# AlessioSam/LADiff

Measured on AMD Instinct MI355X. Metric: motions/sec (196-frame, 50-step DDIM, bs128), higher is better.
Workload: dtype f16x3+f32; 1 GPU; headline:ddim50_cfg7.5_b128_f196_c263_humanml3d; prompts_per_gpu=128, global_batch=128, frames=196, scheduler=ddim, denoising_steps=50, parallelism=dp1, loop=persistent pipeline kernel (16-row blocks x 86)

## Files before the change

### ladiff_amd/csrc/api.hip

```cpp
#include <algorithm>
#include <cstdlib>
#include <cstring>
#include <vector>

#include "model.h"
#include "sampler.h"
#include "../../include/ladiff_hip_debug.h"

using namespace ladiff;

namespace {

inline hipStream_t S(ladiff_stream_t s) { return reinterpret_cast<hipStream_t>(s); }

bool all_set(const float* const* w, size_t n) {
    if (w == nullptr) return false;
    for (size_t i = 0; i < n; ++i)
        if (w[i] == nullptr) return false;
    return true;
}
template <class W>
bool load_weights(W& dst, const float* const* ptrs) {
    if (!all_set(ptrs, sizeof(W) / sizeof(const float*))) return false;
    std::memcpy(&dst, ptrs, sizeof(W));
    return true;
}
const char* name_at(const std::vector<std::string>& n, int i) { return (i >= 0 && i < (int)n.size()) ? n[i].c_str() : nullptr; }

}

#ifdef LADIFF_STAMPS
static unsigned long long* g_stamps = nullptr;
#endif

extern "C" {

int ladiff_version(void) { return LADIFF_ABI_VERSION; }
int ladiff_split_format(void) {
#ifndef LADIFF_SPLIT_BF16
    return 1;
#else
    return 0;
#endif
}

const char* ladiff_error_string(int code) {
    switch (code) {
        case LADIFF_OK: return "ok";
        case LADIFF_ERR_ARG: return "invalid argument (null pointer or negative size)";
        case LADIFF_ERR_SHAPE: return "shape not supported by the gfx950 kernels";
        case LADIFF_ERR_WORKSPACE: return "workspace too small";
        case LADIFF_ERR_UNSUPPORTED: return "configuration branch not built";
        default: return code > 0 ? hipGetErrorString((hipError_t)code) : "unknown ladiff error";
    }
}

int ladiff_denoiser_num_params(void) { return DEN_NPARAMS; }
const char* ladiff_denoiser_param_name(int i) { return name_at(denoiser_param_names(), i); }
int ladiff_decoder_num_params(void) { return DEC_NPARAMS; }
const char* ladiff_decoder_param_name(int i) { return name_at(decoder_param_names(), i); }

int ladiff_gemm(const float* A, int lda, const float* A2, int lda2, int K1, const float* W, int ldw, const float* bias,
                const float* res, int ldres, const float* ln_gamma, const float* ln_beta, float* Y, int ldy, int M,
                int N, int K, int act, ladiff_stream_t stream) {
    LADIFF_CHECK_ARG(A && W && Y && M >= 0 && N > 0 && K > 0);
    GemmArgs g;
    g.A = A; g.lda = lda; g.A2 = A2; g.lda2 = lda2; g.K1 = A2 ? K1 : K; g.W = W; g.ldw = ldw; g.bias = bias;
    g.res = res; g.ldres = ldres; g.ln_g = ln_gamma; g.ln_b = ln_beta; g.Y = Y; g.ldy = ldy; g.M = M; g.N = N; g.K = K;
    g.act = act;
    return launch_gemm(g, S(stream));
}

int ladiff_gemm_resident(const float* A, int lda, const float* A2, int lda2, int K1, const float* W, int ldw,
                         const float* bias, const float* res, int ldres, float* Y, int ldy, int M, int N, int K, int act,
                         int split, float* Ys, ladiff_stream_t stream) {
    LADIFF_CHECK_ARG(A && W && (Y || Ys) && M >= 0 && N > 0 && K > 0);
    if (M == 0) return 0;
    KrArgs g;
    g.A = A; g.lda = lda; g.A2 = A2; g.lda2 = lda2; g.K1 = A2 ? K1 : K; g.W = W; g.ldw = ldw; g.bias = bias;
    g.res = res; g.ldres = ldres; g.Y = Y; g.ldy = ldy; g.M = M; g.N = N; g.K = K; g.act = act;
    g.split = split; g.Ys = Ys;
#ifdef LADIFF_STAMPS
    g.stamps = g_stamps;
#endif
    return launch_gemm_kr(g, S(stream));
}

int ladiff_gemm_split(const float* A, int lda, const float* A2, int lda2, int K1, const float* W, int ldw, const float* bias,
                      const float* res, int ldres, float* Y, float* Ys, int ldy, int M, int N, int K, int act,
                      ladiff_stream_t stream) {
    LADIFF_CHECK_ARG(A && W && (Y || Ys) && M >= 0 && N > 0 && K > 0);
    if (M == 0) return 0;
    GemmArgs g;
    g.A = A; g.lda = lda; g.A2 = A2; g.lda2 = lda2; g.K1 = A2 ? K1 : K; g.W = W; g.ldw = ldw; g.bias = bias;
    g.res = res; g.ldres = ldres; g.Y = Y; g.Ys = Ys; g.ldy = ldy; g.M = M; g.N = N; g.K = K; g.act = act; g.split = 1;
    return launch_gemm(g, S(stream));
}

#ifdef LADIFF_STAMPS
void ladiff_debug_set_stamps(unsigned long long* p) { g_stamps = p; }
void ladiff_debug_set_sys_stamps(unsigned long long* p) { ladiff::g_sys_stamps = p; }
void ladiff_debug_set_probe(int v) { ladiff::g_sys_probe = v; }
#endif

int ladiff_combine_rows(const float* partials, int n_planes, int M, const float* bias, const float* res, int mode,
                        const float* ln_gamma, const float* ln_beta, const float* table, const int32_t* counts, int Bs,
                        int T, int pad_row, float* out, ladiff_stream_t stream) {
    LADIFF_CHECK_ARG(partials && out && n_planes > 0 && M >= 0 && Bs > 0 && T > 0);
    if (mode != RED_PLAIN && mode != RED_LN && mode != RED_LN_ADD && mode != RED_LN_MOD) return LADIFF_ERR_ARG;
    if (mode != RED_PLAIN && !(ln_gamma && ln_beta)) return LADIFF_ERR_ARG;
    if ((mode == RED_LN_ADD || mode == RED_LN_MOD) && !table) return LADIFF_ERR_ARG;
    if (M == 0) return 0;
    RedArgs r;
    r.P = partials; r.S = n_planes; r.M = M; r.bias = bias; r.res = res; r.mode = mode; r.g = ln_gamma; r.b = ln_beta; r.tab = table;
    r.counts = counts; r.Bs = Bs; r.T = T; r.pad_row = pad_row; r.out = out;
    return launch_reduce_rows(r, S(stream));
}

int ladiff_layernorm(const float* x, const float* gamma, const float* beta, float* y, int M, ladiff_stream_t stream) {
    LADIFF_CHECK_ARG(x && gamma && beta && y && M >= 0);
    return launch_layernorm(x, gamma, beta, y, M, S(stream));
}

int ladiff_timestep_sinusoid(const int64_t* timesteps, int n, float* out, ladiff_stream_t stream) {
    LADIFF_CHECK_ARG(timesteps && out && n >= 0);
    if (n == 0) return 0;
    return launch_sinusoid(timesteps, n, out, S(stream));
}

int ladiff_decoder_self_attention(const float* qkv, const int32_t* lengths, const uint32_t* keybits, float* out, int B,
                                  int F, ladiff_stream_t stream) {
    LADIFF_CHECK_ARG(qkv && (lengths || keybits) && out && B >= 0);
    return launch_decoder_self_attention(qkv, lengths, keybits, out, B, F, 0, S(stream));
}

int ladiff_self_attention_split(const float* qkv, const int32_t* lengths, const uint32_t* keybits, float* out, int B, int F,
                                 int nheads, int causal, ladiff_stream_t stream) {
    LADIFF_CHECK_ARG(qkv && out && B >= 0);
    return launch_self_attention_split(qkv, lengths, keybits, out, B, F, nheads, causal, 0, S(stream));
}

int ladiff_decoder_cross_attention(const float* q, const float* kv, const int32_t* counts, float* out, int B, int F,
                                   int T, ladiff_stream_t stream) {
    LADIFF_CHECK_ARG(q && kv && out && B >= 0 && F >= 0);
    return launch_decoder_cross_attention(q, kv, counts, out, B, F, T, 0, S(stream));
}

size_t ladiff_denoiser_tables_floats(int n_steps) { return den_tables_floats(n_steps); }
size_t ladiff_denoiser_text_cache_floats(int B2, int n_steps, int n_text) { return den_text_cache_floats(B2, n_steps, n_text); }
size_t ladiff_denoiser_workspace_bytes(int B2, int T, int n_steps, int n_text) {
    return sizeof(float) * std::max({den_forward_ws_floats(B2, T), den_time_layout(nullptr, n_steps).total,
                                     den_text_ws_floats(B2, n_steps, n_text), den_text_ws_floats(B2, n_steps, 1)});
}

int ladiff_denoiser_time_tables(const float* const* w, const float* sinusoid, int n_steps, float* tables, void* ws,
                                size_t ws_bytes, ladiff_stream_t stream) {
    DenoiserW W;
    LADIFF_CHECK_ARG(load_weights(W, w) && sinusoid && tables && ws && n_steps > 0);
    if (ws_bytes < ladiff_denoiser_workspace_bytes(1, 1, n_steps, 1)) return LADIFF_ERR_WORKSPACE;
    return denoiser_time_tables(W, sinusoid, n_steps, tables, (float*)ws, ws_bytes / sizeof(float), S(stream));
}

int ladiff_denoiser_text_cache(const float* const* w, const float* text_emb, int B2, int n_text, const float* tables, int n_steps,
                               float* cache, void* ws, size_t ws_bytes, ladiff_stream_t stream) {
    DenoiserW W;
    LADIFF_CHECK_ARG(load_weights(W, w) && text_emb && tables && cache && ws && B2 > 0 && n_steps > 0 && n_text >= 1);
    if (ws_bytes < ladiff_denoiser_workspace_bytes(B2, 1, n_steps, n_text)) return LADIFF_ERR_WORKSPACE;
    return denoiser_text_cache(W, text_emb, B2, tables, n_steps, cache, (float*)ws, ws_bytes / sizeof(float), S(stream), n_text);
}

int ladiff_denoiser_forward(const float* const* w, const float* const* w_split, const float* tables, const int32_t* d_step,
                            const float* text_cache, int n_text, int n_steps, const float* sample, int Bs, int dup, int T,
                            const int32_t* counts, float* eps, void* ws, size_t ws_bytes, ladiff_stream_t stream) {
    DenoiserW W, WS;
    LADIFF_CHECK_ARG(load_weights(W, w) && tables && d_step && text_cache && sample && eps && ws && Bs > 0 && dup > 0 && n_steps > 0 &&
                     n_text >= 1);
    if (w_split != nullptr) LADIFF_CHECK_ARG(load_weights(WS, w_split));
    if (T < 1 || T > LADIFF_MAX_LATENTS) return LADIFF_ERR_SHAPE;
    if (ws_bytes < ladiff_denoiser_workspace_bytes(Bs * dup, T, n_steps, n_text)) return LADIFF_ERR_WORKSPACE;
    return denoiser_forward(W, w_split ? &WS : nullptr, tables, d_step, text_cache, n_steps, sample, Bs, dup, T, counts, eps, (float*)ws,
                            ws_bytes / sizeof(float), S(stream), 0, -1, 0, n_text);
}

size_t ladiff_linear_cross_attention_workspace_bytes(int B, int T, int n_text) {
    return linear_cross_attention_ws_floats(B, T, n_text) * sizeof(float);
}
int ladiff_linear_cross_attention(const float* const* w, int layer, const float* x, const float* xf, const float* emb,
                                  const int32_t* counts, int B, int T, int n_text, float* out, void* ws, size_t ws_bytes,
                                  ladiff_stream_t stream) {
    DenoiserW W;
    LADIFF_CHECK_ARG(load_weights(W, w) && x && xf && emb && out && ws && B > 0);
    return linear_cross_attention(W, layer, x, xf, emb, counts, B, T, n_text, out, (float*)ws, ws_bytes / sizeof(float), S(stream));
}

int ladiff_cfg_scheduler_step(const float* eps, float* latents, const float* coef, const int32_t* d_step,
                              const float* step_noise, float guidance_scale, int cfg, int B, int T,
                              ladiff_stream_t stream) {
    LADIFF_CHECK_ARG(eps && latents && coef && d_step && B > 0 && T > 0);
    return launch_cfg_step(eps, latents, coef, d_step, step_noise, guidance_scale, cfg, B, T, S(stream));
}
int ladiff_cfg_scheduler_step_multistep(const float* eps, float* latents, float* x0_prev, const float* coef, const int32_t* d_step,
                                        const float* step_noise, float guidance_scale, int cfg, int B, int T, ladiff_stream_t stream) {
    LADIFF_CHECK_ARG(eps && latents && x0_prev && coef && d_step && B > 0 && T > 0);
    if (reinterpret_cast<uintptr_t>(x0_prev) & 15) return LADIFF_ERR_SHAPE;
    return launch_cfg_step(eps, latents, coef, d_step, step_noise, guidance_scale, cfg, B, T, S(stream), nullptr, NoiseGen{0u, 0u, 0u, 0},
                           x0_prev);
}
int ladiff_advance_step(int32_t* d_step, ladiff_stream_t stream) {
    LADIFF_CHECK_ARG(d_step);
    return launch_advance(d_step, S(stream));
}
int ladiff_init_latents(const float* noise, const int32_t* counts, float sigma, float* latents, int B, int T,
                        ladiff_stream_t stream) {
    LADIFF_CHECK_ARG(noise && latents && B > 0 && T > 0);
    return launch_init_latents(noise, counts, sigma, latents, B, T, S(stream));
}
int ladiff_finalize_latents(const float* latents, const int32_t* counts, float* z, int B, int T, ladiff_stream_t stream) {
    LADIFF_CHECK_ARG(latents && z && B > 0 && T > 0);
    return launch_finalize_latents(latents, counts, z, B, T, S(stream));
}

int ladiff_sampler_create(void** sampler) {
    LADIFF_CHECK_ARG(sampler);
    *sampler = new Sampler();
    return 0;
}
int ladiff_sampler_destroy(void* sampler) {
    Sampler* sp = reinterpret_cast<Sampler*>(sampler);
    if (sp == nullptr) return 0;
    (void)hipDeviceSynchronize();
    sp->drain_retired();
    if (sp->exec) (void)hipGraphExecDestroy(sp->exec);
    if (sp->setup) (void)hipGraphExecDestroy(sp->setup);
    if (sp->ev0) (void)hipEventDestroy(sp->ev0);
    if (sp->ev1) (void)hipEventDestroy(sp->ev1);
    for (hipEvent_t e : sp->wev) (void)hipEventDestroy(e);
    sp->cap.destroy();
    delete sp;
    return 0;
}

int ladiff_reverse_plan(int B, int T, const int32_t* h_counts, int masked, int loop_mode, int f16x3, int cfg, int* rows_per_block, int* n_blocks) {
    LADIFF_CHECK_ARG(B >= 1 && T >= 1 && T <= LADIFF_MAX_LATENTS && loop_mode >= 1 && loop_mode <= 3 && rows_per_block && n_blocks);
    if (!cfg && masked && h_counts == nullptr) return LADIFF_ERR_UNSUPPORTED;
    std::vector<unsigned char> plan;
    int mr = 2, nb = 0;
    choose_plan(B, T, h_counts, masked != 0, loop_mode, f16x3 != 0, plan, &mr, &nb, cfg != 0);
    *rows_per_block = 16 * mr; *n_blocks = nb;
    return 0;
}

int ladiff_debug_set_stage_waves(int waves_per_simd) {
    LADIFF_CHECK_ARG(waves_per_simd == 1 || waves_per_simd == 2);
    g_waves16 = waves_per_simd;
    return 0;
}

int ladiff_debug_set_handoff(int tagged) {
    LADIFF_CHECK_ARG(tagged == 0 || tagged == 1);
    g_handoff = tagged;
    return 0;
}

int ladiff_debug_set_mlp_variant(int v) {
#ifdef LADIFF_STAMPS
    LADIFF_CHECK_ARG((v >= 0 && v <= 3) || (v >= 11 && v <= 17) || (v >= 21 && v <= 26));
#else
    LADIFF_CHECK_ARG(v >= 0 && v <= 3);
#endif
    g_mlp_variant = v;
    return 0;
}

int ladiff_debug_set_decoder_fusion(int on) {
    LADIFF_CHECK_ARG(on >= 0 && on <= 126 && (on & 3) != 3 && (on & 48) != 48);
    g_dec_out_cross = (on & 64) ? 0 : 1;
    g_dec_fused_mlp = on & 3;
    g_dec_small_rows_path = (on & 4) ? 0 : 1;
    g_dec_final_split = (on & 8) ? 0 : 1;
    g_dec_fused_attn = (on & 16) ? 0 : (on & 32) ? 2 : 1;
    return 0;
}

int ladiff_debug_set_stage_plan(int v) {
    LADIFF_CHECK_ARG(v >= 0 && v <= 1);
    g_stage_plan = v;
    return 0;
}

int ladiff_debug_set_poll_pause(int mask, int len) {
    LADIFF_CHECK_ARG(mask >= 0 && mask <= 255 && len >= 0 && len <= 64);
    g_poll_pause = mask | (len << 8);
    return 0;
}

int ladiff_debug_set_pacing(int eighths, int mask) {
    if (eighths == -1) { g_pace = -1; return 0; }
    LADIFF_CHECK_ARG(eighths >= 0 && eighths <= 8 && mask >= 0 && mask <= 255);
    g_pace = eighths | (mask << 8);
    return 0;
}

int ladiff_debug_set_stage_delay(int mask, int len) {
    LADIFF_CHECK_ARG(mask >= -1 && mask <= 255 && len >= 0 && len <= 64);
    g_stage_delay = mask < 0 ? -1 : (mask | (len << 8));
    return 0;
}

int ladiff_debug_set_loop_thresholds(int look_ahead_from, int small_upto) {
    LADIFF_CHECK_ARG(look_ahead_from >= -1 && small_upto >= -1);
    g_look_ahead_from = look_ahead_from;
    g_small_upto = small_upto;
    return 0;
}

int ladiff_debug_set_graph_epoch_rule(int on) {
    LADIFF_CHECK_ARG(on == 0 || on == 1);
    g_graph_epoch_rule = on;
    return 0;
}

int ladiff_debug_graph_instantiations(void) { return g_graph_instantiations.load(); }

int ladiff_debug_set_xcd_local(int on) {
    LADIFF_CHECK_ARG(on >= 0 && on <= 2);
    g_xcd_local = on;
    return 0;
}

int ladiff_sampler_set_loop(void* sampler, int mode) {
    Sampler* sp = reinterpret_cast<Sampler*>(sampler);
    LADIFF_CHECK_ARG(sp != nullptr && mode >= 0 && mode <= 3);
    sp->loop = mode != 0;
    sp->loop_mode = mode;
    return 0;
}

int ladiff_sampler_loop_ms(void* sampler, float* ms) {
    Sampler* sp = reinterpret_cast<Sampler*>(sampler);
    LADIFF_CHECK_ARG(sp != nullptr && ms != nullptr && sp->ev1 != nullptr);
    LADIFF_HIP(hipEventSynchronize(sp->ev1));
    LADIFF_HIP(hipEventElapsedTime(ms, sp->ev0, sp->ev1));
    return 0;
}

int ladiff_sampler_set_window_timing(void* sampler, int on) {
    Sampler* sp = reinterpret_cast<Sampler*>(sampler);
    LADIFF_CHECK_ARG(sp != nullptr);
    sp->time_windows = on != 0;
    return 0;
}

int ladiff_sampler_window_ms(void* sampler, float* loop_ms_sum, int* n_windows) {
    Sampler* sp = reinterpret_cast<Sampler*>(sampler);
    LADIFF_CHECK_ARG(sp != nullptr && loop_ms_sum != nullptr && n_windows != nullptr);
    float sum = 0.f;
    for (int i = 0; i < sp->n_windows; ++i) {
        float ms = 0.f;
        LADIFF_HIP(hipEventSynchronize(sp->wev[2 * i + 1]));
        LADIFF_HIP(hipEventElapsedTime(&ms, sp->wev[2 * i], sp->wev[2 * i + 1]));
        sum += ms;
    }
    *loop_ms_sum = sum; *n_windows = sp->n_windows;
    return 0;
}

int ladiff_sampler_last_loop(void* sampler, int* pipeline, int* rows_per_block, int* n_blocks) {
    Sampler* sp = reinterpret_cast<Sampler*>(sampler);
    LADIFF_CHECK_ARG(sp != nullptr && pipeline != nullptr);
    *pipeline = sp->last_pipeline;
    if (rows_per_block) *rows_per_block = sp->last_pipeline ? 16 * sp->plan_mr : 0;
    if (n_blocks) *n_blocks = sp->last_pipeline ? sp->plan_nb : 0;
    return 0;
}

int ladiff_sampler_set_noise_generator(void* sampler, uint64_t seed, uint32_t first_prompt, int enable) {
    Sampler* sp = reinterpret_cast<Sampler*>(sampler);
    LADIFF_CHECK_ARG(sp != nullptr);
    sp->gen = NoiseGen{(unsigned)(seed & 0xffffffffull), (unsigned)(seed >> 32), first_prompt, enable ? 1 : 0};
    return 0;
}

int ladiff_noise_fill(uint64_t seed, uint32_t first_prompt, int first_step, int n_steps, int B, int T, float* out, ladiff_stream_t stream) {
    LADIFF_CHECK_ARG(out != nullptr && first_step >= 0 && n_steps >= 0 && B >= 0);
    if (T < 1 || T > LADIFF_MAX_LATENTS) return LADIFF_ERR_SHAPE;
    return launch_noise_fill(NoiseGen{(unsigned)(seed & 0xffffffffull), (unsigned)(seed >> 32), first_prompt, 1}, first_step, n_steps, B, T, out,
                             S(stream));
}

int ladiff_noise_fill_prompts(const uint64_t* seeds, const uint32_t* prompt_index, int first_step, int n_steps, int B, int T, float* out,
                              ladiff_stream_t stream) {
    LADIFF_CHECK_ARG(out != nullptr && first_step >= -1 && n_steps >= 0 && B >= 0 && (seeds != nullptr || B == 0));
    if (T < 1 || T > LADIFF_MAX_LATENTS) return LADIFF_ERR_SHAPE;
    if ((reinterpret_cast<uintptr_t>(seeds) & 7) || (reinterpret_cast<uintptr_t>(prompt_index) & 3)) return LADIFF_ERR_SHAPE;
    return launch_noise_fill(NoiseGen{0u, 0u, 0u, 1, reinterpret_cast<const unsigned long long*>(seeds), prompt_index}, first_step, n_steps, B, T,
                             out, S(stream));
}

int ladiff_sampler_set_fault(void* sampler, int workgroup, int timeout_ms) {
    Sampler* sp = reinterpret_cast<Sampler*>(sampler);
    LADIFF_CHECK_ARG(sp != nullptr && workgroup >= -1 && workgroup < 256 && timeout_ms >= 0);
    sp->fault_wg = workgroup;
    sp->timeout_ticks = (unsigned long long)timeout_ms * 100000ull;
    return 0;
}

size_t ladiff_reverse_status_offset_bytes(int B, int T, int n_steps, int n_text) {
    if (B < 1 || T < 1 || T > LADIFF_MAX_LATENTS || n_steps < 1 || n_text < 1) return 0;
    const ReverseWs r = carve_reverse(nullptr, B, T, n_steps, n_text);
    return (r.sys_off + sys_status_offset_floats(B, T)) * sizeof(float);
}

int ladiff_reverse_status(void* ws, int B, int T, int n_steps, int n_text, int* code, int* info) {
    LADIFF_CHECK_ARG(ws && code && B > 0 && n_steps > 0);
    if (T < 1 || T > LADIFF_MAX_LATENTS) return LADIFF_ERR_SHAPE;
    const ReverseWs r = carve_reverse(ws, B, T, n_steps, n_text);
    unsigned st[2] = {0u, 0u};
    LADIFF_HIP(hipMemcpy(st, r.sys + sys_status_offset_floats(B, T), sizeof(st), hipMemcpyDeviceToHost));
    *code = (int)st[0];
    if (info) *info = (int)st[1];
    return 0;
}

size_t ladiff_reverse_workspace_bytes(int B, int T, int n_steps, int n_text) { return carve_reverse(nullptr, B, T, n_steps, n_text).total_bytes; }

int ladiff_mlp_ln_fused(const float* xs, const float* x, const float* w1s, const float* b1, const float* w2s, const float* b2,
                        const float* ln_gamma, const float* ln_beta, const float* ln2_gamma, const float* ln2_beta, float* y, float* ys,
                        int M, ladiff_stream_t stream) {
    LADIFF_CHECK_ARG(xs && x && w1s && b1 && w2s && b2 && ln_gamma && ln_beta && (y || ys) && M >= 0);
    if ((ln2_gamma == nullptr) != (ln2_beta == nullptr)) return LADIFF_ERR_ARG;
    return launch_dec_mlp(xs, x, w1s, b1, w2s, b2, ln_gamma, ln_beta, ln2_gamma, ln2_beta, y, ys, M, S(stream));
}

int ladiff_split_rows(const float* x, float* y, int R, int K, ladiff_stream_t stream) {
    LADIFF_CHECK_ARG(x && y && R >= 0 && K > 0);
    if (K % 64) return LADIFF_ERR_SHAPE;
    if (R == 0) return 0;
    return launch_split_rows(x, y, R, K, S(stream));
}

int ladiff_gather_rows(const float* src, const int32_t* index, int n_rows, int row_floats, float* dst, ladiff_stream_t stream) {
    LADIFF_CHECK_ARG(n_rows >= 0 && row_floats > 0);
    if (n_rows == 0) return 0;
    LADIFF_CHECK_ARG(src && index && dst);
    if (row_floats % 4 || (reinterpret_cast<uintptr_t>(src) & 15) || (reinterpret_cast<uintptr_t>(dst) & 15)) return LADIFF_ERR_SHAPE;
    if ((reinterpret_cast<uintptr_t>(index) & 3) || n_rows > (1 << 30)) return LADIFF_ERR_SHAPE;
    return launch_gather_rows(src, index, n_rows, row_floats, dst, S(stream));
}

int ladiff_split_range_stats(const float* const* tensors, const int64_t* counts, int n, int64_t max_count, uint64_t* stats,
                             ladiff_stream_t stream) {
    LADIFF_CHECK_ARG(n >= 0 && max_count >= 0);
    if (n == 0) return 0;
    LADIFF_CHECK_ARG(tensors && counts && stats);
    if (n > 65535 || max_count >= (int64_t(1) << 32)) return LADIFF_ERR_SHAPE;
    return launch_split_range_stats(tensors, counts, n, max_count, reinterpret_cast<unsigned long long*>(stats), S(stream));
}

int ladiff_diffusion_reverse(void* sampler, const float* const* w, const float* const* w_split, uint64_t weights_generation,
                             const float* text_emb, const float* init_noise, const int32_t* counts, const int32_t* final_counts,
                             const int32_t* h_counts, const float* sinusoid, const float* coef, const float* step_noise, float guidance_scale,
                             float init_noise_sigma, int cfg, int B, int T, int n_text, int n_steps, float* z, void* ws, size_t ws_bytes,
                             int reuse_time_tables, ladiff_stream_t stream) {
    return ladiff_diffusion_reverse_prompts(sampler, w, w_split, weights_generation, text_emb, init_noise, counts, final_counts, h_counts, sinusoid,
                                            coef, step_noise, guidance_scale, init_noise_sigma, cfg, B, T, n_text, n_steps, z, ws, ws_bytes,
                                            reuse_time_tables, nullptr, nullptr, nullptr, 0, stream);
}

int ladiff_diffusion_reverse_prompts(void* sampler, const float* const* w, const float* const* w_split, uint64_t weights_generation,
                                     const float* text_emb, const float* init_noise, const int32_t* counts, const int32_t* final_counts,
                                     const int32_t* h_counts, const float* sinusoid, const float* coef, const float* step_noise,
                                     float guidance_scale, float init_noise_sigma, int cfg, int B, int T, int n_text, int n_steps, float* z,
                                     void* ws, size_t ws_bytes, int reuse_time_tables, const float* guidance_scales, const uint64_t* seeds,
                                     const uint32_t* prompt_index, int draw_init_noise, ladiff_stream_t stream) {
    return ladiff_diffusion_reverse_multistep(sampler, w, w_split, weights_generation, text_emb, init_noise, counts, final_counts, h_counts,
                                              sinusoid, coef, step_noise, guidance_scale, init_noise_sigma, cfg, B, T, n_text, n_steps, z, ws,
                                              ws_bytes, reuse_time_tables, guidance_scales, seeds, prompt_index, draw_init_noise, nullptr, stream);
}

int ladiff_diffusion_reverse_multistep(void* sampler, const float* const* w, const float* const* w_split, uint64_t weights_generation,
                                       const float* text_emb, const float* init_noise, const int32_t* counts, const int32_t* final_counts,
                                       const int32_t* h_counts, const float* sinusoid, const float* coef, const float* step_noise,
                                       float guidance_scale, float init_noise_sigma, int cfg, int B, int T, int n_text, int n_steps, float* z,
                                       void* ws, size_t ws_bytes, int reuse_time_tables, const float* guidance_scales, const uint64_t* seeds,
                                       const uint32_t* prompt_index, int draw_init_noise, float* x0_prev, ladiff_stream_t stream) {
    DenoiserW W, WS;
    LADIFF_CHECK_ARG(guidance_scales == nullptr || cfg != 0);
    LADIFF_CHECK_ARG(prompt_index == nullptr || seeds != nullptr);
    LADIFF_CHECK_ARG(!draw_init_noise || seeds != nullptr);
    LADIFF_CHECK_ARG(init_noise != nullptr || draw_init_noise);
    LADIFF_CHECK_ARG(load_weights(W, w) && text_emb && sinusoid && coef && z && ws && B > 0 && n_steps > 0);
    if (w_split != nullptr) LADIFF_CHECK_ARG(load_weights(WS, w_split));
    if (T < 1 || T > LADIFF_MAX_LATENTS || n_text < 1) return LADIFF_ERR_SHAPE;
    if ((reinterpret_cast<uintptr_t>(guidance_scales) & 3) || (reinterpret_cast<uintptr_t>(seeds) & 7) ||
        (reinterpret_cast<uintptr_t>(prompt_index) & 3) || (reinterpret_cast<uintptr_t>(x0_prev) & 15))
        return LADIFF_ERR_SHAPE;
    return diffusion_reverse(reinterpret_cast<Sampler*>(sampler), W, w_split ? &WS : nullptr,
                             ReverseArgs{w, w_split, weights_generation, text_emb, init_noise, counts, final_counts, h_counts, sinusoid, coef,
                                         step_noise, guidance_scale, init_noise_sigma, cfg, B, T, n_text, n_steps, z, ws, ws_bytes,
                                         reuse_time_tables, stream, guidance_scales, seeds, prompt_index, draw_init_noise ? 1 : 0, x0_prev});
}

int ladiff_encoder_num_params(void) { return ENC_NPARAMS; }
const char* ladiff_encoder_param_name(int i) { return name_at(encoder_param_names(), i); }
size_t ladiff_encoder_workspace_bytes(int B, int F, int T, int C) { return enc_ws_floats(B, F, T, C) * sizeof(float); }

int ladiff_vae_encode(const float* const* w, const float* const* w_split, const float* features, const int32_t* lengths,
                      const int32_t* counts, const float* eps, int B, int F, int T, int C, float* mu, float* std,
                      float* latent, void* ws, size_t ws_bytes, ladiff_stream_t stream) {
    EncoderW W, WS;
    LADIFF_CHECK_ARG(load_weights(W, w) && features && lengths && counts && eps && mu && std && latent && ws && B >= 0);
    if (w_split != nullptr) LADIFF_CHECK_ARG(load_weights(WS, w_split));
    return vae_encode(W, w_split ? &WS : nullptr, features, lengths, counts, eps, B, F, T, C, mu, std, latent, (float*)ws,
                      ws_bytes / sizeof(float), S(stream));
}

int ladiff_vae_encode_dvae(const float* const* w, const float* const* w_split, const float* features, const int32_t* lengths,
                           const int32_t* counts, const float* eps, int B, int F, int T, int C, float* mu, float* std, float* latent,
                           void* ws, size_t ws_bytes, const int32_t* slot, const float* values, int n, ladiff_stream_t stream) {
    EncoderW W, WS;
    LADIFF_CHECK_ARG(load_weights(W, w) && features && lengths && counts && eps && mu && std && latent && ws && B >= 0);
    LADIFF_CHECK_ARG(slot && n >= 0 && (values || n == 0));
    if (w_split != nullptr) LADIFF_CHECK_ARG(load_weights(WS, w_split));
    if ((reinterpret_cast<uintptr_t>(slot) & 3) || (reinterpret_cast<uintptr_t>(values) & 3)) return LADIFF_ERR_SHAPE;
    return vae_encode(W, w_split ? &WS : nullptr, features, lengths, counts, eps, B, F, T, C, mu, std, latent, (float*)ws,
                      ws_bytes / sizeof(float), S(stream), slot, values, n);
}

size_t ladiff_vae_losses_workspace_bytes(int B, int F, int C, int J, int T) { return vae_losses_ws_floats(B, F, C, J, T) * sizeof(float); }

int ladiff_vae_losses(const float* m_rst, const float* m_ref, const float* joints_rst, const float* joints_ref, const float* mu,
                      const float* std, int B, int F, int C, int J, int T, double lambda_rec, double lambda_joint, double lambda_kl,
                      double* batch, double* acc, void* ws, size_t ws_bytes, ladiff_stream_t stream) {
    LADIFF_CHECK_ARG(m_rst && m_ref && joints_rst && joints_ref && mu && std && batch && acc && ws);
    if (B < 1 || F < 1 || C < 1 || J < 1 || T < 1) return LADIFF_ERR_SHAPE;
    for (const void* p : {(const void*)m_rst, (const void*)m_ref, (const void*)joints_rst, (const void*)joints_ref, (const void*)mu,
                          (const void*)std})
        if (reinterpret_cast<uintptr_t>(p) & 3) return LADIFF_ERR_SHAPE;
    for (const void* p : {(const void*)batch, (const void*)acc, (const void*)ws})
        if (reinterpret_cast<uintptr_t>(p) & 7) return LADIFF_ERR_SHAPE;
    const VaeLossWs a = vae_losses_layout((float*)ws, B, F, C, J, T);
    if (ws_bytes / sizeof(float) < a.total) return LADIFF_ERR_WORKSPACE;
    return launch_vae_losses(m_rst, m_ref, (size_t)B * F * C, joints_rst, joints_ref, (size_t)B * F * J * 3, mu, std, (size_t)T * B * D,
                             lambda_rec, lambda_joint, lambda_kl, a.part, a.blocks, batch, acc, S(stream));
}

size_t ladiff_denoiser_forward_timesteps_workspace_bytes(int B2, int T) { return den_per_sample_ws_floats(B2, T) * sizeof(float); }

int ladiff_denoiser_forward_timesteps(const float* const* w, const float* const* w_split, const float* text_emb, int n_text,
                                      const int64_t* timesteps, const float* sample, int B2, int T, const int32_t* counts, float* eps,
                                      void* ws, size_t ws_bytes, ladiff_stream_t stream) {
    DenoiserW W, WS;
    LADIFF_CHECK_ARG(load_weights(W, w) && text_emb && timesteps && sample && eps && ws);
    if (w_split != nullptr) LADIFF_CHECK_ARG(load_weights(WS, w_split));
    if (n_text != 1) return LADIFF_ERR_UNSUPPORTED;
    if (B2 < 1 || T < 1 || T > LADIFF_MAX_LATENTS) return LADIFF_ERR_SHAPE;
    for (const void* p : {(const void*)text_emb, (const void*)sample, (const void*)eps, (const void*)ws})
        if (reinterpret_cast<uintptr_t>(p) & 15) return LADIFF_ERR_SHAPE;
    if ((reinterpret_cast<uintptr_t>(timesteps) & 7) || (reinterpret_cast<uintptr_t>(counts) & 3)) return LADIFF_ERR_SHAPE;
    if (ws_bytes < ladiff_denoiser_forward_timesteps_workspace_bytes(B2, T)) return LADIFF_ERR_WORKSPACE;
    return denoiser_forward_timesteps(W, w_split ? &WS : nullptr, text_emb, timesteps, sample, B2, T, counts, eps, (float*)ws,
                                      ws_bytes / sizeof(float), S(stream));
}

int ladiff_q_sample(const float* z, const int64_t* timesteps, const float* alphas_cumprod, int n_train, const int32_t* counts, int draw,
                    uint64_t seed, uint32_t first_prompt, float* noise, float* noisy, int B, int T, ladiff_stream_t stream) {
    LADIFF_CHECK_ARG(z && timesteps && alphas_cumprod && noise && noisy && n_train > 0);
    if (B < 1 || T < 1 || T > LADIFF_MAX_LATENTS) return LADIFF_ERR_SHAPE;
    for (const void* p : {(const void*)z, (const void*)noise, (const void*)noisy})
        if (reinterpret_cast<uintptr_t>(p) & 15) return LADIFF_ERR_SHAPE;
    if ((reinterpret_cast<uintptr_t>(timesteps) & 7) || (reinterpret_cast<uintptr_t>(alphas_cumprod) & 3) ||
        (reinterpret_cast<uintptr_t>(counts) & 3))
        return LADIFF_ERR_SHAPE;
    return launch_q_sample(z, timesteps, alphas_cumprod, n_train, counts,
                           NoiseGen{(unsigned)(seed & 0xffffffffull), (unsigned)(seed >> 32), first_prompt, draw ? 1 : 0}, noise, noisy, B, T,
                           S(stream));
}

size_t ladiff_diffusion_losses_workspace_bytes(int64_t n) { return n < 1 ? 0 : diffusion_losses_layout(nullptr, (size_t)n).total * sizeof(float); }

int ladiff_diffusion_losses(const float* noise_pred, const float* noise, int64_t n, double lambda_inst, double* batch, double* acc, void* ws,
                            size_t ws_bytes, ladiff_stream_t stream) {
    LADIFF_CHECK_ARG(noise_pred && noise && batch && acc && ws);
    if (n < 1) return LADIFF_ERR_SHAPE;
    if ((reinterpret_cast<uintptr_t>(noise_pred) & 3) || (reinterpret_cast<uintptr_t>(noise) & 3)) return LADIFF_ERR_SHAPE;
    for (const void* p : {(const void*)batch, (const void*)acc, (const void*)ws})
        if (reinterpret_cast<uintptr_t>(p) & 7) return LADIFF_ERR_SHAPE;
    const DiffLossWs a = diffusion_losses_layout((float*)ws, (size_t)n);
    if (ws_bytes / sizeof(float) < a.total) return LADIFF_ERR_WORKSPACE;
    return launch_diffusion_losses(noise_pred, noise, (size_t)n, lambda_inst, a.part, a.blocks, batch, acc, S(stream));
}

int ladiff_clip_num_params(void) { return CLIP_NPARAMS; }
const char* ladiff_clip_param_name(int i) { return name_at(clip_param_names(), i); }
size_t ladiff_clip_workspace_bytes(int B, int L) { return clip_ws_floats(B, L) * sizeof(float); }

static bool load_clip(ClipW& dst, const float* const* ptrs, int n_layers) {
    if (ptrs == nullptr || n_layers < 1 || n_layers > CLIP_MAX_LAYERS) return false;
    const int n = CLIP_HEAD_NPARAMS + CLIP_LAYER_NPARAMS * n_layers;
    for (int i = 0; i < n; ++i)
        if (ptrs[i] == nullptr) return false;
    std::memset(&dst, 0, sizeof(dst));
    std::memcpy(&dst, ptrs, n * sizeof(const float*));
    return true;
}

int ladiff_clip_text_encode(const float* const* w, const float* const* w_split, int n_layers, int vocab, const int64_t* ids,
                            int B, int seq, int L, float* out, void* ws, size_t ws_bytes, ladiff_stream_t stream) {
    ClipW W, WS;
    LADIFF_CHECK_ARG(load_clip(W, w, n_layers) && ids && out && ws && B >= 0);
    if (w_split != nullptr) LADIFF_CHECK_ARG(load_clip(WS, w_split, n_layers));
    return clip_text_encode(W, w_split ? &WS : nullptr, n_layers, vocab, ids, B, seq, L, out, (float*)ws,
                            ws_bytes / sizeof(float), S(stream));
}

size_t ladiff_clip_workspace_bytes_ragged(int B, int total_rows) { return clip_ws_floats_rows(B, total_rows) * sizeof(float); }

int ladiff_clip_text_encode_ragged(const float* const* w, const float* const* w_split, int n_layers, int vocab, const int64_t* ids,
                                   int B, int seq, int L, const int32_t* seq_len, const int32_t* row_off, const int32_t* row_seq,
                                   int total_rows, float* out, void* ws, size_t ws_bytes, ladiff_stream_t stream) {
    ClipW W, WS;
    LADIFF_CHECK_ARG(load_clip(W, w, n_layers) && ids && out && ws && B >= 0 && seq_len && row_off && row_seq && total_rows >= 0);
    if (w_split != nullptr) LADIFF_CHECK_ARG(load_clip(WS, w_split, n_layers));
    return clip_text_encode(W, w_split ? &WS : nullptr, n_layers, vocab, ids, B, seq, L, out, (float*)ws,
                            ws_bytes / sizeof(float), S(stream), seq_len, row_off, row_seq, total_rows);
}

int ladiff_t2m_movement_num_params(void) { return (int)t2m_move_param_names().size(); }
const char* ladiff_t2m_movement_param_name(int i) { return name_at(t2m_move_param_names(), i); }
int ladiff_t2m_motion_num_params(void) { return (int)t2m_motion_param_names().size(); }
const char* ladiff_t2m_motion_param_name(int i) { return name_at(t2m_motion_param_names(), i); }
int ladiff_t2m_text_num_params(void) { return (int)t2m_text_param_names().size(); }
const char* ladiff_t2m_text_param_name(int i) { return name_at(t2m_text_param_names(), i); }
size_t ladiff_t2m_movement_workspace_bytes(int B, int F, int Cin) { return t2m_move_ws_floats(B, F, Cin) * sizeof(float); }
size_t ladiff_t2m_motion_workspace_bytes(int B, int T) { return t2m_motion_ws_floats(B, T) * sizeof(float); }
size_t ladiff_t2m_text_workspace_bytes(int B, int L) { return t2m_text_ws_floats(B, L) * sizeof(float); }

int ladiff_t2m_movement_encode(const float* const* w, const float* feats, int ld, int B, int F, int Cin, float* out, void* ws,
                               size_t ws_bytes, ladiff_stream_t stream) {
    LADIFF_CHECK_ARG(all_set(w, t2m_move_param_names().size()) && feats && out && ws && B >= 0);
    return t2m_movement_encode(w, feats, ld, B, F, Cin, out, (float*)ws, ws_bytes / sizeof(float), S(stream));
}
int ladiff_t2m_motion_encode(const float* const* w, const float* movements, const int32_t* m_lens, int B, int T, float* out,
                             void* ws, size_t ws_bytes, ladiff_stream_t stream) {
    LADIFF_CHECK_ARG(all_set(w, t2m_motion_param_names().size()) && movements && m_lens && out && ws && B >= 0);
    return t2m_motion_encode(w, movements, m_lens, B, T, out, (float*)ws, ws_bytes / sizeof(float), S(stream));
}
int ladiff_t2m_text_encode(const float* const* w, const float* word_embs, const float* pos_onehot, const int32_t* cap_lens,
                           int B, int L, float* out, void* ws, size_t ws_bytes, ladiff_stream_t stream) {
    LADIFF_CHECK_ARG(all_set(w, t2m_text_param_names().size()) && word_embs && pos_onehot && cap_lens && out && ws && B >= 0);
    return t2m_text_encode(w, word_embs, pos_onehot, cap_lens, B, L, out, (float*)ws, ws_bytes / sizeof(float), S(stream));
}

int ladiff_feats2joints(const float* feats, const float* mean, const float* std, int B, int F, int C, int njoints,
                        float* joints, ladiff_stream_t stream) {
    LADIFF_CHECK_ARG(feats && mean && std && joints && B >= 0);
    return launch_feats2joints(feats, mean, std, B, F, C, njoints, joints, S(stream));
}

namespace {
int joint_metrics_check(const void* rst, const void* ref, const int32_t* h_lengths, int B, int F, int J, const void* seq_rows, const void* acc) {
    if (J != 21 && J != 22) return LADIFF_ERR_SHAPE;
    if (F < 1 || F > LADIFF_MAX_FRAMES) return LADIFF_ERR_SHAPE;
    for (int b = 0; b < B; ++b)
        if (h_lengths[b] < 1 || h_lengths[b] > F) return LADIFF_ERR_SHAPE;
    if ((reinterpret_cast<uintptr_t>(rst) & 3) || (reinterpret_cast<uintptr_t>(ref) & 3) || (reinterpret_cast<uintptr_t>(seq_rows) & 3) ||
        (reinterpret_cast<uintptr_t>(acc) & 7))
        return LADIFF_ERR_SHAPE;
    return 0;
}
}

int ladiff_joint_ape_ave(const float* joints_rst, const float* joints_ref, const int32_t* lengths, const int32_t* h_lengths, int B, int F,
                         int J, const int32_t* h_part_idx, float factor, float* seq_rows, double* acc, ladiff_stream_t stream) {
    LADIFF_CHECK_ARG(B >= 0);
    if (B == 0) return 0;
    LADIFF_CHECK_ARG(joints_rst && joints_ref && lengths && h_lengths && h_part_idx && seq_rows && acc && factor > 0.f);
    LADIFF_TRY(joint_metrics_check(joints_rst, joints_ref, h_lengths, B, F, J, seq_rows, acc));
    if (reinterpret_cast<uintptr_t>(lengths) & 3) return LADIFF_ERR_SHAPE;
    for (int i = 0; i < 8; ++i)
        if (h_part_idx[i] < 0 || h_part_idx[i] >= (i < 4 ? J - 1 : J)) return LADIFF_ERR_SHAPE;
    return launch_joint_ape_ave(joints_rst, joints_ref, lengths, B, F, J, h_part_idx, factor, seq_rows, acc, S(stream));
}

int ladiff_joint_mr(const float* joints_rst, const float* joints_ref, const int32_t* h_lengths, int B, int F, int J, float* seq_rows,
                    double* acc, ladiff_stream_t stream) {
    LADIFF_CHECK_ARG(B >= 0);
    if (B == 0) return 0;
    LADIFF_CHECK_ARG(joints_rst && joints_ref && h_lengths && seq_rows && acc);
    LADIFF_TRY(joint_metrics_check(joints_rst, joints_ref, h_lengths, B, F, J, seq_rows, acc));
    return launch_joint_mr(joints_rst, joints_ref, B, F, J, seq_rows, acc, S(stream));
}

size_t ladiff_decoder_workspace_bytes(int B, int F, int T, int C) {
    (void)C;
    return dec_ws_floats(B, (size_t)B * F, T) * sizeof(float);
}

int ladiff_vae_decode(const float* const* w, const float* const* w_split, const float* z, const int32_t* lengths,
                      const int32_t* counts, int B, int F, int T, int C, float* feats, void* ws, size_t ws_bytes,
                      ladiff_stream_t stream) {
    DecoderW W, WS;
    LADIFF_CHECK_ARG(load_weights(W, w) && z && lengths && feats && ws && B >= 0);
    if (w_split != nullptr) LADIFF_CHECK_ARG(load_weights(WS, w_split));
    return vae_decode(W, w_split ? &WS : nullptr, z, lengths, counts, nullptr, 0, B, F, T, C, feats, (float*)ws, ws_bytes / sizeof(float),
                      S(stream));
}

namespace {
struct DecodeGraph {
    hipGraphExec_t exec = nullptr;
    GraphSlot slot;
    CaptureStream cap;
};
}

int ladiff_decoder_graph_create(void** graph) {
    LADIFF_CHECK_ARG(graph);
    *graph = new DecodeGraph();
    return 0;
}
int ladiff_decoder_graph_destroy(void* graph) {
    DecodeGraph* g = reinterpret_cast<DecodeGraph*>(graph);
    if (g == nullptr) return 0;
    (void)hipDeviceSynchronize();
    if (g->exec) (void)hipGraphExecDestroy(g->exec);
    g->cap.destroy();
    delete g;
    return 0;
}

int ladiff_vae_decode_graphed(void* graph, const float* const* w, const float* const* w_split, uint64_t weights_generation, const float* z,
                              const int32_t* lengths, const int32_t* counts, const int32_t* row_off, int total_rows, int B, int F, int T,
                              int C, float* feats, void* ws, size_t ws_bytes, ladiff_stream_t stream) {
    DecodeGraph* dg = reinterpret_cast<DecodeGraph*>(graph);
    DecoderW W, WS;
    LADIFF_CHECK_ARG(dg && load_weights(W, w) && z && lengths && feats && ws && B >= 0 && stream != nullptr);
    if (w_split != nullptr) LADIFF_CHECK_ARG(load_weights(WS, w_split));
    if (F < 1 || F > LADIFF_MAX_FRAMES || T < 1 || T > LADIFF_MAX_LATENTS || C < 1) return LADIFF_ERR_SHAPE;
    if (ws_bytes < ladiff_decoder_workspace_bytes(B, F, T, C)) return LADIFF_ERR_WORKSPACE;
    hipStream_t s = S(stream);
    const GraphKey key = decode_key(w, w_split, DEC_NPARAMS, weights_generation, z, lengths, counts, row_off, total_rows, B, F, T, C, feats, ws,
                                    stream, g_dec_fused_mlp, g_dec_small_rows_path, g_dec_final_split, g_mlp_variant, g_dec_fused_attn);
    if (!(dg->exec && dg->slot.key == key && dg->slot.newest())) {
        if (dg->exec) { LADIFF_HIP(hipStreamSynchronize(s)); (void)hipGraphExecDestroy(dg->exec); dg->exec = nullptr; }
        LADIFF_TRY(dec_mlp_prepare());
        LADIFF_TRY(dec_qkv_attn_prepare());
        LADIFF_TRY(dec_cross_prepare());
        LADIFF_TRY(dg->cap.ensure());
        LADIFF_TRY(capture_graph(dg->cap.s, [&](hipStream_t cs) {
            if (row_off != nullptr) LADIFF_TRY(launch_zero_fill(feats, (size_t)B * F * C, cs));
            return vae_decode(W, w_split ? &WS : nullptr, z, lengths, counts, row_off, total_rows, B, F, T, C, feats, (float*)ws,
                              ws_bytes / sizeof(float), cs);
        }, &dg->exec));
        dg->slot.stamp(key);
    }
    LADIFF_HIP(hipGraphLaunch(dg->exec, s));
    return 0;
}

int ladiff_vae_decode_ragged(const float* const* w, const float* const* w_split, const float* z, const int32_t* lengths,
                             const int32_t* counts, const int32_t* row_off, int total_rows, int B, int F, int T, int C, float* feats,
                             void* ws, size_t ws_bytes, ladiff_stream_t stream) {
    DecoderW W, WS;
    LADIFF_CHECK_ARG(load_weights(W, w) && z && lengths && row_off && feats && ws && B >= 0 && total_rows >= 0);
    if (w_split != nullptr) LADIFF_CHECK_ARG(load_weights(WS, w_split));
    if (F < 1 || F > LADIFF_MAX_FRAMES || T < 1 || T > LADIFF_MAX_LATENTS || C < 1) return LADIFF_ERR_SHAPE;
    if (ws_bytes < ladiff_decoder_workspace_bytes(B, F, T, C)) return LADIFF_ERR_WORKSPACE;
    LADIFF_HIP(hipMemsetAsync(feats, 0, (size_t)B * F * C * sizeof(float), S(stream)));
    return vae_decode(W, w_split ? &WS : nullptr, z, lengths, counts, row_off, total_rows, B, F, T, C, feats, (float*)ws,
                      ws_bytes / sizeof(float), S(stream));
}

}
```

### ladiff_amd/csrc/attention.hip

```cpp
#include "kernels.h"

namespace ladiff {

constexpr int SA_FMAX = LADIFF_MAX_FRAMES;
constexpr int SA_NKT = SA_FMAX / 32;

struct AttnGeom { int nheads, ld, koff, voff, out_ld, causal; };

__global__ __launch_bounds__(256) void dec_self_attn_kernel(const float* __restrict__ qkv, const int32_t* __restrict__ lengths,
                                                            const uint32_t* __restrict__ keybits, float* __restrict__ out,
                                                            int B, int F, int split_out, const AttnGeom g,
                                                            const int32_t* __restrict__ row_off, int shared_qkv) {
    __shared__ __attribute__((aligned(16))) float Ks[SA_FMAX * DH];
    __shared__ __attribute__((aligned(16))) float Vs[SA_FMAX * DH];
    const int tid = threadIdx.x, lane = tid & 63, wave = tid >> 6;
    const int b = blockIdx.y / g.nheads, h = blockIdx.y % g.nheads;
    int len = F;
    uint32_t kb[SA_NKT + 1];
    if (keybits != nullptr) {
        len = 1;
#pragma unroll
        for (int i = 0; i < SA_NKT; ++i) {
            kb[i] = keybits[(size_t)b * 8 + i];
            if (kb[i]) len = 32 * i + 32 - __builtin_clz(kb[i]);
        }
        len = len > F ? F : len;
    } else {
        len = lengths != nullptr ? lengths[b] : F;
        len = len < 1 ? 1 : (len > F ? F : len);
#pragma unroll
        for (int i = 0; i < SA_NKT; ++i) kb[i] = len >= 32 * i + 32 ? 0xFFFFFFFFu : (len > 32 * i ? (1u << (len - 32 * i)) - 1u : 0u);
    }
    const int nkt = (len + 31) >> 5;
    size_t row0 = (size_t)b * F;
    if (row_off != nullptr) { row0 = row_off[b]; F = row_off[b + 1] - row_off[b]; }
    const size_t base = (shared_qkv ? (size_t)0 : row0) * g.ld + h * DH;

    for (int id = tid; id < nkt * 32 * 16; id += 256) {
        const int r = id >> 4, c = id & 15;
        f32x4 kk = {0.f, 0.f, 0.f, 0.f}, vv = {0.f, 0.f, 0.f, 0.f};
        if (r < F) {
            const float* src = qkv + base + (size_t)r * g.ld + c * 4;
            kk = ld4(src + g.koff);
            vv = ld4(src + g.voff);
        }
        st4(Ks + r * DH + ((c ^ (r & 15)) << 2), kk);
        st4(Vs + r * DH + c * 4, vv);
    }
    __syncthreads();

    const int qt = blockIdx.x * 4 + wave;
    if (qt * 32 >= F) return;
    const int q = lane & 31, h2 = lane >> 5;
    const int qrow = qt * 32 + q;

    f32x4 qf[8];
#pragma unroll
    for (int g8 = 0; g8 < 8; ++g8) {
        f32x4 v = {0.f, 0.f, 0.f, 0.f};
        if (qrow < F) v = ld4(qkv + base + (size_t)qrow * g.ld + g8 * 8 + h2 * 4);
#pragma unroll
        for (int e = 0; e < 4; ++e) v[e] *= 0.125f;
        qf[g8] = v;
    }

    f32x16 sT[SA_NKT];
    float m = -INFINITY;
#pragma unroll
    for (int kt = 0; kt < SA_NKT; ++kt) {
        if (kt < nkt) {
            f32x16 acc;
#pragma unroll
            for (int i = 0; i < 16; ++i) acc[i] = 0.f;
            const int r = kt * 32 + q;
#pragma unroll
            for (int g8 = 0; g8 < 8; ++g8) {
                const f32x4 a = ld4(Ks + r * DH + ((((g8 << 1) + h2) ^ (r & 15)) << 2));
#pragma unroll
                for (int e = 0; e < 4; ++e) acc = __builtin_amdgcn_mfma_f32_32x32x2f32(a[e], qf[g8][e], acc, 0, 0, 0);
            }
#pragma unroll
            for (int i = 0; i < 16; ++i) {
                const int kin = (i & 3) + 8 * (i >> 2) + 4 * h2;
                const bool ok = ((kb[kt] >> kin) & 1u) && (!g.causal || kt * 32 + kin <= qrow);
                const float s = ok ? acc[i] : -INFINITY;
                acc[i] = s;
                m = fmaxf(m, s);
            }
            sT[kt] = acc;
        }
    }
    m = fmaxf(m, __shfl_xor(m, 32, 64));

    float l = 0.f;
#pragma unroll
    for (int kt = 0; kt < SA_NKT; ++kt) {
        if (kt < nkt) {
#pragma unroll
            for (int i = 0; i < 16; ++i) {
                const float pv = expf(sT[kt][i] - m);
                sT[kt][i] = pv;
                l += pv;
            }
        }
    }
    l += __shfl_xor(l, 32, 64);

    f32x16 o0, o1;
#pragma unroll
    for (int i = 0; i < 16; ++i) { o0[i] = 0.f; o1[i] = 0.f; }
#pragma unroll
    for (int kt = 0; kt < SA_NKT; ++kt) {
        if (kt < nkt) {
#pragma unroll
            for (int i = 0; i < 16; ++i) {
                const int key = kt * 32 + (i & 3) + 8 * (i >> 2) + 4 * h2;
                const float a0 = Vs[key * DH + q];
                const float a1 = Vs[key * DH + 32 + q];
                o0 = __builtin_amdgcn_mfma_f32_32x32x2f32(a0, sT[kt][i], o0, 0, 0, 0);
                o1 = __builtin_amdgcn_mfma_f32_32x32x2f32(a1, sT[kt][i], o1, 0, 0, 0);
            }
        }
    }

    if (qrow < F) {
        const float inv = 1.f / l;
        float* rowp = out + (row0 + qrow) * g.out_ld;
        const int c0 = h * DH + 4 * h2;
#pragma unroll
        for (int rg = 0; rg < 4; ++rg) {
            f32x4 v0, v1;
#pragma unroll
            for (int e = 0; e < 4; ++e) { v0[e] = o0[4 * rg + e] * inv; v1[e] = o1[4 * rg + e] * inv; }
            if (split_out) {
                store_split4(rowp, c0 + 8 * rg, v0);
                store_split4(rowp, c0 + 32 + 8 * rg, v1);
            } else {
                st4(rowp + c0 + 8 * rg, v0);
                st4(rowp + c0 + 32 + 8 * rg, v1);
            }
        }
    }
}


__device__ __forceinline__ void split8(const float (&v)[8], s16x8& hi, s16x8& lo) {
    split8(f32x4{v[0], v[1], v[2], v[3]}, f32x4{v[4], v[5], v[6], v[7]}, hi, lo);
}

template <int FM, int NT>
__global__ __launch_bounds__(NT, NT == 64 ? 2 : 1) void self_attn_split_kernel(const float* __restrict__ qkv, const int32_t* __restrict__ lengths,
                                                               const uint32_t* __restrict__ keybits, float* __restrict__ out,
                                                               int B, int F, int split_out, const AttnGeom g,
                                                               const int32_t* __restrict__ row_off, int shared_qkv) {
    constexpr int NKT = FM / 32, IT = FM * 16 / NT, VLD = FM + 8;
    static_assert(FM % 32 == 0 && (FM * 16) % NT == 0 && NT % 64 == 0 && (FM / 4) % (NT / 64) == 0 && NT / 64 >= FM / 32, "a wave per query tile");
    __shared__ __attribute__((aligned(16))) s16 Kp[2 * FM * DH];
    __shared__ __attribute__((aligned(16))) s16 Vt[2 * DH * VLD];
    s16* const Kh = Kp; s16* const Kl = Kp + FM * DH;
    s16* const Vth = Vt; s16* const Vtl = Vt + DH * VLD;
    float* const Vtmp = reinterpret_cast<float*>(Kp);
    const int tid = threadIdx.x, lane = tid & 63, wave = tid >> 6;
    const int b = blockIdx.x / g.nheads, h = blockIdx.x % g.nheads;
    int len = F;
    uint32_t kb[NKT + 1];
    if (keybits != nullptr) {
        len = 1;
#pragma unroll
        for (int i = 0; i < NKT; ++i) {
            kb[i] = keybits[(size_t)b * 8 + i];
            if (kb[i]) len = 32 * i + 32 - __builtin_clz(kb[i]);
        }
        len = len > F ? F : len;
    } else {
        len = lengths != nullptr ? lengths[b] : F;
        len = len < 1 ? 1 : (len > F ? F : len);
#pragma unroll
        for (int i = 0; i < NKT; ++i) kb[i] = len >= 32 * i + 32 ? 0xFFFFFFFFu : (len > 32 * i ? (1u << (len - 32 * i)) - 1u : 0u);
    }
    const int nkt = (len + 31) >> 5;
    size_t row0 = (size_t)b * F;
    if (row_off != nullptr) { row0 = row_off[b]; F = row_off[b + 1] - row_off[b]; }
    const size_t base = (shared_qkv ? (size_t)0 : row0) * g.ld + h * DH;

    const int qt = wave;
    const int q = lane & 31, h2 = lane >> 5;
    const int qrow = qt * 32 + q;

    s16x8 qh[4], ql[4];
#pragma unroll
    for (int ks = 0; ks < 4; ++ks) {
        float v[8] = {0.f, 0.f, 0.f, 0.f, 0.f, 0.f, 0.f, 0.f};
        if (qrow < F) {
            const f32x4 a = ld4(qkv + base + (size_t)qrow * g.ld + 16 * ks + 8 * h2);
            const f32x4 c = ld4(qkv + base + (size_t)qrow * g.ld + 16 * ks + 8 * h2 + 4);
#pragma unroll
            for (int e = 0; e < 4; ++e) { v[e] = a[e] * (0.125f * 1.4426950408889634f); v[4 + e] = c[e] * (0.125f * 1.4426950408889634f); }
        }
        split8(v, qh[ks], ql[ks]);
    }


    f32x4 kk[IT], vv[IT];
#pragma unroll
    for (int it = 0; it < IT; ++it) {
        const int id = tid + it * NT, r = id >> 4, c = id & 15;
        kk[it] = f32x4{0.f, 0.f, 0.f, 0.f}; vv[it] = kk[it];
        if (r < nkt * 32 && r < F) {
            const float* src = qkv + base + (size_t)r * g.ld + c * 4;
            kk[it] = ld4(src + g.koff);
            vv[it] = ld4(src + g.voff);
        }
    }
#pragma unroll
    for (int it = 0; it < IT; ++it) {
        const int id = tid + it * NT, r = id >> 4, c = id & 15;
        if (r < nkt * 32) st4(Vtmp + r * DH + c * 4, vv[it]);
    }
    __syncthreads();
    {
        const int d = tid & 63, kg = tid >> 6;
        for (int p = 0; p < FM / 4 / (NT / 64); ++p) {
            const int k0 = (p * (NT / 64) + kg) * 4;
            if (k0 < nkt * 32) {
                s16x4 hi, lo;
                split4(Vtmp[k0 * DH + d], Vtmp[(k0 + 1) * DH + d], Vtmp[(k0 + 2) * DH + d], Vtmp[(k0 + 3) * DH + d], hi, lo);
                *reinterpret_cast<s16x4*>(Vth + d * VLD + k0) = hi;
                *reinterpret_cast<s16x4*>(Vtl + d * VLD + k0) = lo;
            }
        }
    }
    __syncthreads();
#pragma unroll
    for (int it = 0; it < IT; ++it) {
        const int id = tid + it * NT, r = id >> 4, c = id & 15;
        if (r < nkt * 32) {
            s16x4 hi, lo;
            split4(kk[it], hi, lo);
            const int off = r * DH + ((((c >> 1) ^ ((r >> 1) & 7)) << 3) | ((c & 1) << 2));
            *reinterpret_cast<s16x4*>(Kh + off) = hi;
            *reinterpret_cast<s16x4*>(Kl + off) = lo;
        }
    }
    __syncthreads();

    if (qt * 32 >= F) return;

    f32x16 sT[NKT];
    float m = -INFINITY;
#pragma unroll
    for (int kt = 0; kt < NKT; ++kt) {
        if (kt < nkt) {
            f32x16 acc;
#pragma unroll
            for (int i = 0; i < 16; ++i) acc[i] = 0.f;
            const int r = kt * 32 + q;
#pragma unroll
            for (int ks = 0; ks < 4; ++ks) {
                const int off = r * DH + (((2 * ks + h2) ^ ((r >> 1) & 7)) << 3);
                const s16x8 kh = *reinterpret_cast<const s16x8*>(Kh + off);
                const s16x8 kl = *reinterpret_cast<const s16x8*>(Kl + off);
                acc = MFMA32_S16(kl, qh[ks], acc, 0, 0, 0);
                acc = MFMA32_S16(kh, ql[ks], acc, 0, 0, 0);
                acc = MFMA32_S16(kh, qh[ks], acc, 0, 0, 0);
            }
            if (kb[kt] == 0xFFFFFFFFu && !g.causal) {
#pragma unroll
                for (int i = 0; i < 16; ++i) m = fmaxf(m, acc[i]);
            } else {
#pragma unroll
                for (int i = 0; i < 16; ++i) {
                    const int kin = (i & 3) + 8 * (i >> 2) + 4 * h2;
                    const bool ok = ((kb[kt] >> kin) & 1u) && (!g.causal || kt * 32 + kin <= qrow);
                    const float s = ok ? acc[i] : -INFINITY;
                    acc[i] = s;
                    m = fmaxf(m, s);
                }
            }
            sT[kt] = acc;
        }
    }
    m = fmaxf(m, __shfl_xor(m, 32, 64));

    float l = 0.f;
#pragma unroll
    for (int kt = 0; kt < NKT; ++kt) {
        if (kt < nkt) {
#pragma unroll
            for (int i = 0; i < 16; ++i) {
                const float pv = __builtin_amdgcn_exp2f(sT[kt][i] - m);
                sT[kt][i] = pv;
                l += pv;
            }
        }
    }
    l += __shfl_xor(l, 32, 64);

    f32x16 o0, o1;
#pragma unroll
    for (int i = 0; i < 16; ++i) { o0[i] = 0.f; o1[i] = 0.f; }
#pragma unroll
    for (int kt = 0; kt < NKT; ++kt) {
        if (kt < nkt) {
#pragma unroll
            for (int mm = 0; mm < 2; ++mm) {
                float pv[8];
#pragma unroll
                for (int j = 0; j < 8; ++j) pv[j] = sT[kt][8 * mm + j];
                s16x8 ph, pl;
                split8(pv, ph, pl);
                const int k1 = 32 * kt + 16 * mm + 4 * h2;
#pragma unroll
                for (int t = 0; t < 2; ++t) {
                    const int voff = (32 * t + q) * VLD + k1;
                    const s16x4 h_a = *reinterpret_cast<const s16x4*>(Vth + voff), h_b = *reinterpret_cast<const s16x4*>(Vth + voff + 8);
                    const s16x4 l_a = *reinterpret_cast<const s16x4*>(Vtl + voff), l_b = *reinterpret_cast<const s16x4*>(Vtl + voff + 8);
                    const s16x8 vh = {h_a[0], h_a[1], h_a[2], h_a[3], h_b[0], h_b[1], h_b[2], h_b[3]};
                    const s16x8 vl = {l_a[0], l_a[1], l_a[2], l_a[3], l_b[0], l_b[1], l_b[2], l_b[3]};
                    f32x16& o = t == 0 ? o0 : o1;
                    o = MFMA32_S16(vl, ph, o, 0, 0, 0);
                    o = MFMA32_S16(vh, pl, o, 0, 0, 0);
                    o = MFMA32_S16(vh, ph, o, 0, 0, 0);
                }
            }
        }
    }

    if (qrow < F) {
        const float inv = 1.f / l;
        float* rowp = out + (row0 + qrow) * g.out_ld;
        const int c0 = h * DH + 4 * h2;
#pragma unroll
        for (int rg = 0; rg < 4; ++rg) {
            f32x4 v0, v1;
#pragma unroll
            for (int e = 0; e < 4; ++e) { v0[e] = o0[4 * rg + e] * inv; v1[e] = o1[4 * rg + e] * inv; }
            if (split_out) {
                store_split4(rowp, c0 + 8 * rg, v0);
                store_split4(rowp, c0 + 32 + 8 * rg, v1);
            } else {
                st4(rowp + c0 + 8 * rg, v0);
                st4(rowp + c0 + 32 + 8 * rg, v1);
            }
        }
    }
}

int launch_self_attention_split(const float* qkv, const int32_t* lengths, const uint32_t* keybits, float* out, int B, int F,
                                 int nheads, int causal, int split_out, hipStream_t s, const int32_t* row_off, int shared_qkv) {
    if (F > SA_FMAX || F < 1 || nheads < 1) return LADIFF_ERR_SHAPE;
    if (B == 0) return 0;
    const int W = nheads * DH;
    const AttnGeom g{nheads, 3 * W, W, 2 * W, W, causal};
    if (F <= 32) hipLaunchKernelGGL((self_attn_split_kernel<32, 64>), dim3(B * nheads), dim3(64), 0, s, qkv, lengths, keybits, out, B, F, split_out, g, row_off, shared_qkv);
    else hipLaunchKernelGGL((self_attn_split_kernel<SA_FMAX, 512>), dim3(B * nheads), dim3(512), 0, s, qkv, lengths, keybits, out, B, F, split_out, g, row_off, shared_qkv);
    LADIFF_LAUNCH_CHECK();
    return 0;
}

int launch_self_attention(const float* qkv, const int32_t* lengths, const uint32_t* keybits, float* out, int B, int F, int nheads,
                          int causal, int split_out, hipStream_t s, const int32_t* row_off) {
    if (F > SA_FMAX || F < 1 || nheads < 1) return LADIFF_ERR_SHAPE;
    if (B == 0) return 0;
    const int W = nheads * DH;
    const AttnGeom g{nheads, 3 * W, W, 2 * W, W, causal};
    const int nqt = (F + 31) / 32;
    hipLaunchKernelGGL(dec_self_attn_kernel, dim3((nqt + 3) / 4, B * nheads), dim3(256), 0, s, qkv, lengths, keybits, out, B, F,
                       split_out, g, row_off, 0);
    LADIFF_LAUNCH_CHECK();
    return 0;
}

int launch_decoder_self_attention(const float* qkv, const int32_t* lengths, const uint32_t* keybits, float* out, int B, int F,
                                  int split_out, hipStream_t s, const int32_t* row_off, int shared_qkv) {
    if (F > SA_FMAX || F < 1) return LADIFF_ERR_SHAPE;
    if (lengths == nullptr && keybits == nullptr) return LADIFF_ERR_ARG;
    if (B == 0) return 0;
    const AttnGeom g{H, 3 * D, D, 2 * D, D, 0};
    const int nqt = (F + 31) / 32;
    hipLaunchKernelGGL(dec_self_attn_kernel, dim3((nqt + 3) / 4, B * H), dim3(256), 0, s, qkv, lengths, keybits, out, B, F,
                       split_out, g, row_off, shared_qkv);
    LADIFF_LAUNCH_CHECK();
    return 0;
}

template <int T>
__global__ __launch_bounds__(256) void dec_cross_attn_kernel(const float* __restrict__ q, const float* __restrict__ kv,
                                                             const int32_t* __restrict__ counts, float* __restrict__ out,
                                                             int B, int F, int M, int split_out) {
    const int row = blockIdx.x * 4 + (threadIdx.x >> 6);
    if (row >= M) return;
    const int c = (threadIdx.x & 63) * 4;
    const int b = row / F;
    int nv = counts ? counts[b] : T;
    nv = nv < 1 ? 1 : (nv > T ? T : nv);
    f32x4 qv = ld4(q + (size_t)row * D + c);
    float s[T];
    float m = -INFINITY;
#pragma unroll
    for (int j = 0; j < T; ++j) {
        const f32x4 kk = ld4(kv + ((size_t)j * B + b) * 512 + c);
        float d = (qv[0] * 0.125f) * kk[0] + (qv[1] * 0.125f) * kk[1] + (qv[2] * 0.125f) * kk[2] + (qv[3] * 0.125f) * kk[3];
        d = row16_sum(d);
        s[j] = j < nv ? d : -INFINITY;
        m = fmaxf(m, s[j]);
    }
    float l = 0.f;
    f32x4 o = {0.f, 0.f, 0.f, 0.f};
#pragma unroll
    for (int j = 0; j < T; ++j) {
        const float pv = expf(s[j] - m);
        l += pv;
        const f32x4 vv = ld4(kv + ((size_t)j * B + b) * 512 + 256 + c);
#pragma unroll
        for (int e = 0; e < 4; ++e) o[e] += pv * vv[e];
    }
    const float inv = 1.f / l;
#pragma unroll
    for (int e = 0; e < 4; ++e) o[e] *= inv;
    if (split_out) store_split4(out + (size_t)row * D, c, o);
    else st4(out + (size_t)row * D + c, o);
}

int launch_decoder_cross_attention(const float* q, const float* kv, const int32_t* counts, float* out, int B, int F,
                                   int T, int split_out, hipStream_t s) {
    const int M = B * F;
    if (M == 0) return 0;
    const dim3 grid((M + 3) / 4), block(256);
#define LADIFF_CA_CASE(TT) \
    case TT: hipLaunchKernelGGL(dec_cross_attn_kernel<TT>, grid, block, 0, s, q, kv, counts, out, B, F, M, split_out); break;
    switch (T) {
        LADIFF_CA_CASE(1) LADIFF_CA_CASE(2) LADIFF_CA_CASE(3) LADIFF_CA_CASE(4)
        LADIFF_CA_CASE(5) LADIFF_CA_CASE(6) LADIFF_CA_CASE(7) LADIFF_CA_CASE(8)
        default: return LADIFF_ERR_SHAPE;
    }
#undef LADIFF_CA_CASE
    LADIFF_LAUNCH_CHECK();
    return 0;
}

template <int T, bool PER_SAMPLE>
__global__ __launch_bounds__(256) void den_self_attn_kernel(const float* __restrict__ qkv, const float* __restrict__ text_kv,
                                                            const float* __restrict__ tables, int kv_off, int step_stride,
                                                            const int32_t* __restrict__ d_step,
                                                            const int32_t* __restrict__ counts, int Bs, int b_off,
                                                            float* __restrict__ out, int split_out) {
    const int b2 = blockIdx.x;
    const int bg = b_off + b2;
    const int col = threadIdx.x;
    float qv[T], kk[T + 2], vv[T + 2];
#pragma unroll
    for (int i = 0; i < T; ++i) {
        const float* r = qkv + ((size_t)b2 * T + i) * 768 + col;
        qv[i] = r[0] * 0.125f;
        kk[i] = r[256];
        vv[i] = r[512];
    }
    kk[T] = text_kv[(size_t)bg * 512 + col];
    vv[T] = text_kv[(size_t)bg * 512 + 256 + col];
    const float* tk = tables + (size_t)(PER_SAMPLE ? bg : *d_step) * step_stride + kv_off;
    kk[T + 1] = tk[col];
    vv[T + 1] = tk[256 + col];
    int nv = counts ? counts[bg % Bs] : T;
    nv = nv > T ? T : nv;
    __shared__ __attribute__((aligned(16))) float so[T * D];
#pragma unroll
    for (int i = 0; i < T; ++i) {
        float s[T + 2];
        float m = -INFINITY;
#pragma unroll
        for (int j = 0; j < T + 2; ++j) {
            const float d = wave_sum(qv[i] * kk[j]);
            s[j] = (j < T && j >= nv) ? -INFINITY : d;
            m = fmaxf(m, s[j]);
        }
        float l = 0.f, o = 0.f;
#pragma unroll
        for (int j = 0; j < T + 2; ++j) {
            const float pv = expf(s[j] - m);
            l += pv;
            o += pv * vv[j];
        }
        if (split_out) so[i * D + col] = o / l;
        else out[((size_t)b2 * T + i) * D + col] = o / l;
    }
    if (split_out) {
        __syncthreads();
        for (int u = threadIdx.x; u < T * (D / 4); u += 256) {
            const int r = u / (D / 4), c4 = (u % (D / 4)) * 4;
            store_split4(out + ((size_t)b2 * T + r) * D, c4, ld4(so + r * D + c4));
        }
    }
}

int launch_denoiser_self_attention(const float* qkv, const float* text_kv, const float* tables, int kv_off,
                                   int step_stride, const int32_t* d_step, const int32_t* counts, int Bs, int b_off,
                                   int b_n, int T, float* out, int split_out, hipStream_t s) {
    if (b_n == 0) return 0;
    const dim3 grid(b_n), block(256);
#define LADIFF_SA_CASE(TT)                                                                                          \
    case TT:                                                                                                        \
        if (d_step == nullptr)                                                                                      \
            hipLaunchKernelGGL((den_self_attn_kernel<TT, true>), grid, block, 0, s, qkv, text_kv, tables, kv_off,    \
                               step_stride, d_step, counts, Bs, b_off, out, split_out);                               \
        else                                                                                                        \
            hipLaunchKernelGGL((den_self_attn_kernel<TT, false>), grid, block, 0, s, qkv, text_kv, tables, kv_off,   \
                               step_stride, d_step, counts, Bs, b_off, out, split_out);                               \
        break;
    switch (T) {
        LADIFF_SA_CASE(1) LADIFF_SA_CASE(2) LADIFF_SA_CASE(3) LADIFF_SA_CASE(4)
        LADIFF_SA_CASE(5) LADIFF_SA_CASE(6) LADIFF_SA_CASE(7) LADIFF_SA_CASE(8)
        default: return LADIFF_ERR_SHAPE;
    }
#undef LADIFF_SA_CASE
    LADIFF_LAUNCH_CHECK();
    return 0;
}

}
```

### ladiff_amd/csrc/dec_cross.hip

```cpp
#include <mutex>
#include "kernels.h"
#include "tile_mma.h"

namespace ladiff { extern unsigned long long* g_sys_stamps; }

namespace ladiff {

namespace {
constexpr int TM = LADIFF_MAX_LATENTS;
}

__global__ __launch_bounds__(256) void dec_cross_prep_kernel(const DecCrossPrepBatch pb, int B, int T, int tiles_per_wg) {
    const int h = blockIdx.y, layer = blockIdx.z, tid = threadIdx.x, lane = tid & 63, c16 = lane & 15, kq = lane >> 4;
    const int wave = __builtin_amdgcn_readfirstlane(tid >> 6);
    const float* __restrict__ kv = pb.kv[layer]; const float* __restrict__ wq = pb.wq[layer]; const float* __restrict__ bq = pb.bq[layer];
    const float* __restrict__ wo = pb.wo[layer]; float* __restrict__ gu = pb.gu[layer];
    float* __restrict__ cc = gu + (size_t)B * H * T * 2 * D;
    const int M = T * B, ntiles = (M + 15) / 16;
    float gq[4][16], uo[4][16], bqv[16];
#pragma unroll
    for (int t = 0; t < 4; ++t) {
        const int n = 64 * wave + 16 * t + c16;
#pragma unroll
        for (int s = 0; s < 16; ++s) gq[t][s] = wq[(size_t)(h * DH + 16 * kq + s) * D + n];
#pragma unroll
        for (int s4 = 0; s4 < 16; s4 += 4) {
            const f32x4 w4 = ld4(wo + (size_t)n * D + h * DH + 16 * kq + s4);
#pragma unroll
            for (int e = 0; e < 4; ++e) uo[t][s4 + e] = w4[e];
        }
    }
#pragma unroll
    for (int s4 = 0; s4 < 16; s4 += 4) {
        const f32x4 b4 = ld4(bq + h * DH + 16 * kq + s4);
#pragma unroll
        for (int e = 0; e < 4; ++e) bqv[s4 + e] = b4[e];
    }
    const int tile1 = (blockIdx.x + 1) * tiles_per_wg < ntiles ? (blockIdx.x + 1) * tiles_per_wg : ntiles;
    for (int tile = blockIdx.x * tiles_per_wg; tile < tile1; ++tile) {
        const int arow = 16 * tile + c16 < M ? 16 * tile + c16 : M - 1;
        const float* kr = kv + (size_t)arow * 2 * D + h * DH + 16 * kq;
        float ak[16], av[16];
#pragma unroll
        for (int s4 = 0; s4 < 16; s4 += 4) {
            const f32x4 k4 = ld4(kr + s4), v4 = ld4(kr + D + s4);
#pragma unroll
            for (int e = 0; e < 4; ++e) { ak[s4 + e] = k4[e]; av[s4 + e] = v4[e]; }
        }
        f32x4 ag[4], au[4];
#pragma unroll
        for (int t = 0; t < 4; ++t) { ag[t] = f32x4{0.f, 0.f, 0.f, 0.f}; au[t] = ag[t]; }
#pragma unroll
        for (int s = 0; s < 16; ++s)
#pragma unroll
            for (int t = 0; t < 4; ++t) {
                ag[t] = __builtin_amdgcn_mfma_f32_16x16x4f32(ak[s], gq[t][s], ag[t], 0, 0, 0);
                au[t] = __builtin_amdgcn_mfma_f32_16x16x4f32(av[s], uo[t][s], au[t], 0, 0, 0);
            }
#pragma unroll
        for (int i = 0; i < 4; ++i) {
            const int bt = 16 * tile + 4 * kq + i;
            if (bt < M) {
                const int j = bt / B, b = bt - j * B;
                float* o = gu + ((((size_t)b * H + h) * T + j) * 2) * D + 64 * wave + c16;
#pragma unroll
                for (int t = 0; t < 4; ++t) { o[16 * t] = ag[t][i] * 0.125f; o[D + 16 * t] = au[t][i]; }
            }
        }
        if (wave == 0) {
            float c = 0.f;
#pragma unroll
            for (int s = 0; s < 16; ++s) c = fmaf(bqv[s], ak[s], c);
            c += __shfl_xor(c, 16, 64); c += __shfl_xor(c, 32, 64);
            const int bt = 16 * tile + c16;
            if (kq == 0 && bt < M) { const int j = bt / B, b = bt - j * B; cc[((size_t)b * H + h) * T + j] = c * 0.125f; }
        }
    }
}

template <int T>
__device__ __forceinline__ void cross_row(const f32x4 (&xv)[4], f32x4 (&acc)[4], const float* sm, const float* cs, int nv, int c0) {
#pragma unroll 1
    for (int h = 0; h < H; ++h) {
        float sc[T];
#pragma unroll
        for (int j = 0; j < T; ++j) {
            const float* gp = sm + ((size_t)(h * T + j) * 2) * D + c0;
            float d = 0.f;
#pragma unroll
            for (int k = 0; k < 4; ++k) {
                const f32x4 g4 = ld4(gp + 64 * k);
                d = fmaf(xv[k][0], g4[0], fmaf(xv[k][1], g4[1], fmaf(xv[k][2], g4[2], fmaf(xv[k][3], g4[3], d))));
            }
            sc[j] = d;
        }
#pragma unroll
        for (int j = 0; j < T; ++j) sc[j] = row16_sum(sc[j]) + cs[h * T + j];
        float m = -INFINITY;
#pragma unroll
        for (int j = 0; j < T; ++j) { sc[j] = j < nv ? sc[j] : -INFINITY; m = fmaxf(m, sc[j]); }
        float l = 0.f;
#pragma unroll
        for (int j = 0; j < T; ++j) { sc[j] = __builtin_amdgcn_exp2f((sc[j] - m) * 1.4426950408889634f); l += sc[j]; }
        const float inv = 1.f / l;
#pragma unroll
        for (int j = 0; j < T; ++j) {
            const float pj = sc[j] * inv;
            const float* up = sm + ((size_t)(h * T + j) * 2 + 1) * D + c0;
#pragma unroll
            for (int k = 0; k < 4; ++k) {
                const f32x4 u4 = ld4(up + 64 * k);
                acc[k][0] = fmaf(pj, u4[0], acc[k][0]); acc[k][1] = fmaf(pj, u4[1], acc[k][1]);
                acc[k][2] = fmaf(pj, u4[2], acc[k][2]); acc[k][3] = fmaf(pj, u4[3], acc[k][3]);
            }
        }
    }
}

template <int TT>
__global__ __launch_bounds__(256) void dec_cross_apply_kernel(const float* __restrict__ x, const float* __restrict__ gu,
                                                              const float* __restrict__ cc, const int32_t* __restrict__ counts,
                                                              const float* __restrict__ bo, const float* __restrict__ g2,
                                                              const float* __restrict__ b2, int F, int rows_per_wg,
                                                              float* __restrict__ y, float* __restrict__ ys,
                                                              const int32_t* __restrict__ row_off, const float* __restrict__ g1,
                                                              const float* __restrict__ b1) {
    extern __shared__ __attribute__((aligned(16))) float sm[];
    constexpr int T = TT, HT = H * TT;
    const int b = blockIdx.x, tid = threadIdx.x, lane = tid & 63, wave = tid >> 6;
    const float* src = gu + (size_t)b * HT * 2 * D;
    for (int u = tid; u < HT * 2 * D / 4; u += 256) st4(sm + 4 * u, ld4(src + 4 * u));
    float* cs = sm + (size_t)HT * 2 * D;
    if (tid < HT) cs[tid] = cc[(size_t)b * HT + tid];
    int nv = counts != nullptr ? counts[b] : T;
    nv = nv > T ? T : nv;
    __syncthreads();
    const int l16 = lane & 15, grp = lane >> 4, c0 = 4 * l16;
    f32x4 bo4[4], gg[4], bb[4];
#pragma unroll
    for (int k = 0; k < 4; ++k) { bo4[k] = ld4(bo + c0 + 64 * k); gg[k] = ld4(g2 + c0 + 64 * k); bb[k] = ld4(b2 + c0 + 64 * k); }
    size_t row0 = (size_t)b * F;
    if (row_off != nullptr) { row0 = row_off[b]; F = row_off[b + 1] - row_off[b]; }
    const int f0 = blockIdx.y * rows_per_wg;
    const int f1 = f0 + rows_per_wg < F ? f0 + rows_per_wg : F;
    for (int fb = f0; fb < f1; fb += 16) {
        const int f = fb + 4 * wave + grp;
        const bool live = f < f1;
        const size_t row = row0 + (live ? f : f1 - 1);
        f32x4 xv[4], acc[4];
#pragma unroll
        for (int k = 0; k < 4; ++k) xv[k] = ld4(x + row * D + c0 + 64 * k);
        if (g1 != nullptr) {
            float s1 = 0.f;
#pragma unroll
            for (int k = 0; k < 4; ++k) s1 += (xv[k][0] + xv[k][1]) + (xv[k][2] + xv[k][3]);
            const float mean1 = row16_sum(s1) * (1.f / 256.f);
            float q1 = 0.f;
#pragma unroll
            for (int k = 0; k < 4; ++k)
#pragma unroll
                for (int i = 0; i < 4; ++i) { const float dlt = xv[k][i] - mean1; q1 += dlt * dlt; }
            const float rstd1 = rsqrtf(row16_sum(q1) * (1.f / 256.f) + LN_EPS);
#pragma unroll
            for (int k = 0; k < 4; ++k) {
                const f32x4 ga = ld4(g1 + c0 + 64 * k), be = ld4(b1 + c0 + 64 * k);
#pragma unroll
                for (int i = 0; i < 4; ++i) xv[k][i] = (xv[k][i] - mean1) * rstd1 * ga[i] + be[i];
            }
        }
#pragma unroll
        for (int k = 0; k < 4; ++k)
#pragma unroll
            for (int i = 0; i < 4; ++i) acc[k][i] = bo4[k][i] + xv[k][i];
        cross_row<T>(xv, acc, sm, cs, nv, c0);
        float sum = 0.f;
#pragma unroll
        for (int k = 0; k < 4; ++k) sum += (acc[k][0] + acc[k][1]) + (acc[k][2] + acc[k][3]);
        const float mean = row16_sum(sum) * (1.f / 256.f);
        float q = 0.f;
#pragma unroll
        for (int k = 0; k < 4; ++k)
#pragma unroll
            for (int i = 0; i < 4; ++i) { const float dlt = acc[k][i] - mean; q += dlt * dlt; }
        const float rstd = rsqrtf(row16_sum(q) * (1.f / 256.f) + LN_EPS);
        if (live) {
#pragma unroll
            for (int k = 0; k < 4; ++k) {
                f32x4 o;
#pragma unroll
                for (int i = 0; i < 4; ++i) o[i] = (acc[k][i] - mean) * rstd * gg[k][i] + bb[k][i];
                st4(y + row * D + c0 + 64 * k, o);
                if (ys != nullptr) store_split4(ys + row * D, c0 + 64 * k, o);
            }
        }
    }
}


constexpr int OC_ROWS = 32;
constexpr int OC_TILE = OC_ROWS * 1024;
constexpr int OC_CT = OC_ROWS * CLD * 4;
constexpr int OC_XN = OC_ROWS * CLD * 4;
constexpr int OC_SLD = 36;
constexpr int OC_PS = 8 * OC_ROWS * OC_SLD * 4;
constexpr int OC_PT = OC_ROWS * 256;

struct OutCrossArgs {
    const float* att;
    const float* x0;
    const float* wo;
    const float* bo; const float* g1; const float* b1;
    const float* gu; const float* cc;
    const float* bo_c; const float* g2; const float* b2;
    const int32_t* counts; const int32_t* row_off;
    float* y; float* ys;
    int F, rows_per_wg;
    unsigned long long* stamps;
};

#ifdef LADIFF_STAMPS
#define OC_STAMP(i) do { if (p.stamps != nullptr && blockIdx.x == 3 && blockIdx.y == 0 && threadIdx.x == 0 && npass < 6) p.stamps[npass * 16 + (i)] = __builtin_amdgcn_s_memrealtime(); } while (0)
#else
#define OC_STAMP(i) do { } while (0)
#endif

__device__ __forceinline__ void oc_barrier() { asm volatile("s_waitcnt lgkmcnt(0)\n\ts_barrier" ::: "memory"); }

template <int TT>
__global__ __launch_bounds__(512, 1) void dec_out_cross_kernel(const OutCrossArgs p) {
    __shared__ __attribute__((aligned(1024))) char tile[OC_TILE];
    __shared__ __attribute__((aligned(1024))) char ps_b[OC_PS];
    __shared__ __attribute__((aligned(1024))) char ct_b[OC_CT];
    __shared__ __attribute__((aligned(1024))) char xn_b[OC_XN];
    __shared__ __attribute__((aligned(16))) float sc[OC_ROWS * OC_SLD];
    __shared__ __attribute__((aligned(256))) char ptile[OC_PT];
    __shared__ __attribute__((aligned(16))) float vec[6 * D];
    __shared__ float cs[32];
    constexpr int T = TT, HT = H * TT;
    static_assert(HT <= 32, "the (head, token) columns fit one k-step");
    float* ct = reinterpret_cast<float*>(ct_b);
    float* xn = reinterpret_cast<float*>(xn_b);
    float* ps = reinterpret_cast<float*>(ps_b);
    const int b = blockIdx.x, tid = threadIdx.x, lane = tid & 63, frow = lane & 15, fk = lane >> 4;
    const int wave = __builtin_amdgcn_readfirstlane(tid >> 6);
    int npass = 0;
    OC_STAMP(15);
    WFrag<0, 2, 1> gf, uf;
    {
        const float* gub = p.gu + (size_t)b * HT * 2 * D;
#pragma unroll
        for (int j = 0; j < 2; ++j) {
            const int hj = 16 * j + frow;
            f32x4 a = {0.f, 0.f, 0.f, 0.f}, c = a;
            if (hj < HT) { const float* g = gub + (size_t)hj * 2 * D + 32 * wave + 8 * fk; a = ld4(g); c = ld4(g + 4); }
            split8(a, c, gf.hi[j][0], gf.lo[j][0]);
            const int col = 32 * wave + 16 * j + frow;
            f32x4 u0 = {0.f, 0.f, 0.f, 0.f}, u1 = u0;
#pragma unroll
            for (int e = 0; e < 4; ++e) {
                if (8 * fk + e < HT) u0[e] = gub[((size_t)(8 * fk + e) * 2 + 1) * D + col];
                if (8 * fk + 4 + e < HT) u1[e] = gub[((size_t)(8 * fk + 4 + e) * 2 + 1) * D + col];
            }
            split8(u0, u1, uf.hi[j][0], uf.lo[j][0]);
        }
        if (tid < 32) cs[tid] = tid < HT ? p.cc[(size_t)b * HT + tid] : 0.f;
        const float* vs[6] = {p.bo, p.g1, p.b1, p.bo_c, p.g2, p.b2};
        if (tid < 6 * (D / 4)) st4(vec + 4 * tid, ld4(vs[tid / (D / 4)] + 4 * (tid % (D / 4))));
    }
    WFrag<0, 2, 8> wf;
    {
#pragma unroll 1
        for (int half = 0; half < 2; ++half) {
            if (half == 1) __syncthreads();
#pragma unroll
            for (int qq = 0; qq < 4; ++qq) {
                const int q = (qq + b) & 3;
                char* dst = q == 0 ? tile : q == 1 ? ps_b : q == 2 ? ct_b : xn_b;
#pragma unroll
                for (int kk = 0; kk < 4; ++kk) {
                    const int lr32 = wave + 8 * kk, r = 32 * q + lr32;
                    const char* src = reinterpret_cast<const char*>(p.wo) + ((size_t)(128 * half + r) << 10) + ((lane & 48) << 4) + ((((lane & 15) ^ r) & 15) << 4);
                    __builtin_amdgcn_global_load_lds(reinterpret_cast<const float*>(src), (__attribute__((address_space(3))) void*)(dst + lr32 * 1024), 16, 0, 0);
                }
            }
            __builtin_amdgcn_s_waitcnt(0xF70);
            __syncthreads();
            if ((wave >> 2) == half) {
                const int q = wave & 3;
                const char* srcb = q == 0 ? tile : q == 1 ? ps_b : q == 2 ? ct_b : xn_b;
#pragma unroll
                for (int j = 0; j < 2; ++j)
#pragma unroll
                    for (int st = 0; st < 8; ++st) {
                        const int r = 16 * j + frow;
                        wf.hi[j][st] = *reinterpret_cast<const s16x8*>(a_slot<4>(const_cast<char*>(srcb), r, st >> 1, 4 * (st & 1) + fk));
                        wf.lo[j][st] = *reinterpret_cast<const s16x8*>(a_slot<4>(const_cast<char*>(srcb), r, st >> 1, 8 + 4 * (st & 1) + fk));
                    }
            }
        }
        __syncthreads();
    }
    int nv = p.counts != nullptr ? p.counts[b] : T;
    nv = nv > T ? T : nv;
    int F = p.F;
    size_t row0 = (size_t)b * F;
    if (p.row_off != nullptr) { row0 = p.row_off[b]; F = p.row_off[b + 1] - p.row_off[b]; }
    const int f0 = blockIdx.y * p.rows_per_wg;
    const int f1 = f0 + p.rows_per_wg < F ? f0 + p.rows_per_wg : F;
    if (f0 >= f1) return;
    const int l16 = lane & 15, grp = lane >> 4, c0 = 4 * l16, lr = 4 * wave + grp;
    typedef unsigned u32x4_o __attribute__((ext_vector_type(4)));
    const float* x0s = ps;
    auto dma_att = [&](int fb) {
#pragma unroll
        for (int i = 0; i < 4; ++i) {
            const int r = wave + 8 * i, f = fb + r < f1 ? fb + r : f1 - 1;
            unsigned vo = ((lane & 48) << 4) + ((((lane & 15) ^ r) & 15) << 4);
            asm volatile("" : "+v"(vo));
            const char* src = reinterpret_cast<const char*>(p.att) + ((row0 + f) << 10) + vo;
            __builtin_amdgcn_global_load_lds(reinterpret_cast<const float*>(src), (__attribute__((address_space(3))) void*)(tile + r * 1024), 16, 0, 0);
        }
    };
    auto dma_x0 = [&](int fb) {
#pragma unroll
        for (int i = 0; i < 4; ++i) {
            const int r = wave + 8 * i, f = fb + r < f1 ? fb + r : f1 - 1;
            unsigned vo = lane << 4;
            asm volatile("" : "+v"(vo));
            const char* src = reinterpret_cast<const char*>(p.x0) + ((row0 + f) << 10) + vo;
            __builtin_amdgcn_global_load_lds(reinterpret_cast<const float*>(src), (__attribute__((address_space(3))) void*)(ps_b + r * 1024), 16, 0, 0);
        }
    };
    dma_att(f0);
    dma_x0(f0);
    __builtin_amdgcn_s_waitcnt(0xF70);
    __syncthreads();
    for (int fb = f0; fb < f1; fb += OC_ROWS, ++npass) {
        OC_STAMP(0);
        OC_STAMP(1);
        f32x4 acc2[2][2];
        zero_acc(acc2);
        mma<0, 4, 2, 8, 2>(tile, wf, acc2);
        OC_STAMP(2);
        const int f = fb + lr;
        const bool live = f < f1;
        const size_t row = row0 + (live ? f : f1 - 1);
        f32x4 xv[4];
        stage_c(ct, acc2, [&](int j) { return 32 * wave + 16 * j; });
        __builtin_amdgcn_s_waitcnt(0xF70);
        __syncthreads();
        OC_STAMP(3);
        {
            const float* cr = ct + lr * CLD + c0;
#pragma unroll
            for (int k = 0; k < 4; ++k) {
                const f32x4 o = ld4(cr + 64 * k), bo = ld4(vec + c0 + 64 * k), r0 = ld4(x0s + lr * D + c0 + 64 * k);
#pragma unroll
                for (int i = 0; i < 4; ++i) xv[k][i] = (o[i] + bo[i]) + r0[i];
            }
            float s1 = 0.f;
#pragma unroll
            for (int k = 0; k < 4; ++k) s1 += (xv[k][0] + xv[k][1]) + (xv[k][2] + xv[k][3]);
            const float mean1 = row16_sum(s1) * (1.f / 256.f);
            float q1 = 0.f;
#pragma unroll
            for (int k = 0; k < 4; ++k)
#pragma unroll
                for (int i = 0; i < 4; ++i) { const float dlt = xv[k][i] - mean1; q1 += dlt * dlt; }
            const float rstd1 = rsqrtf(row16_sum(q1) * (1.f / 256.f) + LN_EPS);
#pragma unroll
            for (int k = 0; k < 4; ++k) {
                const f32x4 ga = ld4(vec + D + c0 + 64 * k), be = ld4(vec + 2 * D + c0 + 64 * k);
#pragma unroll
                for (int i = 0; i < 4; ++i) xv[k][i] = (xv[k][i] - mean1) * rstd1 * ga[i] + be[i];
                st4(xn + lr * CLD + c0 + 64 * k, xv[k]);
                tile_put4<0, 4>(tile, lr, c0 + 64 * k, xv[k]);
            }
        }
        OC_STAMP(4);
        __syncthreads();
        OC_STAMP(5);
        {
            u32x4_o ah[2], al[2];
#pragma unroll
            for (int i = 0; i < 2; ++i) {
                ah[i] = *reinterpret_cast<const u32x4_o*>(a_slot<4>(tile, 16 * i + frow, wave >> 1, 4 * (wave & 1) + fk));
                al[i] = *reinterpret_cast<const u32x4_o*>(a_slot<4>(tile, 16 * i + frow, wave >> 1, 8 + 4 * (wave & 1) + fk));
            }
            f32x4 as[2][2];
            zero_acc(as);
#pragma unroll
            for (int i = 0; i < 2; ++i)
#pragma unroll
                for (int j = 0; j < 2; ++j) as[i][j] = MFMA16_S16(__builtin_bit_cast(s16x8, al[i]), gf.hi[j][0], as[i][j], 0, 0, 0);
#pragma unroll
            for (int i = 0; i < 2; ++i)
#pragma unroll
                for (int j = 0; j < 2; ++j) as[i][j] = MFMA16_S16(__builtin_bit_cast(s16x8, ah[i]), gf.lo[j][0], as[i][j], 0, 0, 0);
#pragma unroll
            for (int i = 0; i < 2; ++i)
#pragma unroll
                for (int j = 0; j < 2; ++j) as[i][j] = MFMA16_S16(__builtin_bit_cast(s16x8, ah[i]), gf.hi[j][0], as[i][j], 0, 0, 0);
            float* pw = ps + wave * (OC_ROWS * OC_SLD);
#pragma unroll
            for (int i = 0; i < 2; ++i)
#pragma unroll
                for (int j = 0; j < 2; ++j)
#pragma unroll
                    for (int r = 0; r < 4; ++r) pw[(16 * i + 4 * fk + r) * OC_SLD + 16 * j + frow] = as[i][j][r];
        }
        __syncthreads();
        OC_STAMP(6);
        if (fb + OC_ROWS < f1) dma_att(fb + OC_ROWS);
        {
            float tot[2];
#pragma unroll
            for (int u = 0; u < 2; ++u) {
                const int hj = 16 * u + l16;
                float a = 0.f;
#pragma unroll
                for (int w = 0; w < 8; ++w) a += ps[w * (OC_ROWS * OC_SLD) + lr * OC_SLD + hj];
                tot[u] = a + cs[hj];
                sc[lr * OC_SLD + hj] = tot[u];
            }
            asm volatile("s_waitcnt lgkmcnt(0)" ::: "memory");
            __builtin_amdgcn_wave_barrier();
            float hs[2][T];
            int hh[2], jj[2];
#pragma unroll
            for (int u = 0; u < 2; ++u) {
                const int hj = 16 * u + l16;
                hh[u] = hj < HT ? hj / T : 0; jj[u] = hj - hh[u] * T;
#pragma unroll
                for (int t = 0; t < T; ++t) hs[u][t] = sc[lr * OC_SLD + hh[u] * T + t];
            }
#pragma unroll
            for (int u = 0; u < 2; ++u) {
                const int hj = 16 * u + l16;
                float m = -INFINITY, l = 0.f;
#pragma unroll
                for (int t = 0; t < T; ++t) m = t < nv ? fmaxf(m, hs[u][t]) : m;
#pragma unroll
                for (int t = 0; t < T; ++t) l += t < nv ? __builtin_amdgcn_exp2f((hs[u][t] - m) * 1.4426950408889634f) : 0.f;
                float pr = __builtin_amdgcn_exp2f((tot[u] - m) * 1.4426950408889634f) / l;
                if (!(hj < HT && jj[u] < nv)) pr = 0.f;
                tile_put1<0, 1>(ptile, lr, hj, pr);
            }
        }
        oc_barrier();
        OC_STAMP(7);
        f32x4 ao[2][2];
        zero_acc(ao);
        mma<0, 1, 2, 1, 2>(ptile, uf, ao);
        stage_c(ct, ao, [&](int j) { return 32 * wave + 16 * j; });
        __builtin_amdgcn_s_waitcnt(0xF70);
        oc_barrier();
        OC_STAMP(8);
        {
            const float* cr = ct + lr * CLD + c0;
            f32x4 acc[4];
#pragma unroll
            for (int k = 0; k < 4; ++k) {
                const f32x4 o = ld4(cr + 64 * k), bc = ld4(vec + 3 * D + c0 + 64 * k), x1 = ld4(xn + lr * CLD + c0 + 64 * k);
#pragma unroll
                for (int i = 0; i < 4; ++i) acc[k][i] = (bc[i] + x1[i]) + o[i];
            }
            if (fb + OC_ROWS < f1) dma_x0(fb + OC_ROWS);
            float sum = 0.f;
#pragma unroll
            for (int k = 0; k < 4; ++k) sum += (acc[k][0] + acc[k][1]) + (acc[k][2] + acc[k][3]);
            const float mean = row16_sum(sum) * (1.f / 256.f);
            float q = 0.f;
#pragma unroll
            for (int k = 0; k < 4; ++k)
#pragma unroll
                for (int i = 0; i < 4; ++i) { const float dlt = acc[k][i] - mean; q += dlt * dlt; }
            const float rstd = rsqrtf(row16_sum(q) * (1.f / 256.f) + LN_EPS);
            if (live) {
#pragma unroll
                for (int k = 0; k < 4; ++k) {
                    const f32x4 ga = ld4(vec + 4 * D + c0 + 64 * k), be = ld4(vec + 5 * D + c0 + 64 * k);
                    f32x4 o;
#pragma unroll
                    for (int i = 0; i < 4; ++i) o[i] = (acc[k][i] - mean) * rstd * ga[i] + be[i];
                    st4(p.y + row * D + c0 + 64 * k, o);
                    if (p.ys != nullptr) store_split4(p.ys + row * D, c0 + 64 * k, o);
                }
            }
        }
        OC_STAMP(9);
    }
}

int dec_cross_prepare() {
    static std::mutex mu;
    static bool attr_set[64] = {};
    int dev = 0;
    LADIFF_HIP(hipGetDevice(&dev));
    if (dev < 0 || dev >= 64) return LADIFF_ERR_ARG;
    std::lock_guard<std::mutex> lock(mu);
    if (!attr_set[dev]) {
        LADIFF_HIP(hipFuncSetAttribute(reinterpret_cast<const void*>(dec_cross_apply_kernel<8>), hipFuncAttributeMaxDynamicSharedMemorySize,
                                       (int)(((size_t)H * TM * 2 * D + H * TM) * sizeof(float))));
        const void* oc[8] = {reinterpret_cast<const void*>(dec_out_cross_kernel<1>), reinterpret_cast<const void*>(dec_out_cross_kernel<2>),
                             reinterpret_cast<const void*>(dec_out_cross_kernel<3>), reinterpret_cast<const void*>(dec_out_cross_kernel<4>),
                             reinterpret_cast<const void*>(dec_out_cross_kernel<5>), reinterpret_cast<const void*>(dec_out_cross_kernel<6>),
                             reinterpret_cast<const void*>(dec_out_cross_kernel<7>), reinterpret_cast<const void*>(dec_out_cross_kernel<8>)};
        for (int t = 1; t <= 8; ++t)
            (void)oc[t - 1];
        attr_set[dev] = true;
    }
    return 0;
}

int launch_decoder_cross_prep(const DecCrossPrepBatch& pb, int n, int B, int T, hipStream_t s) {
    if (B == 0 || n == 0) return 0;
    if (T < 1 || T > TM || n > DEC_PREP_MAX) return LADIFF_ERR_SHAPE;
    const int ntiles = (T * B + 15) / 16;
    int tpw = 1;
    while (tpw < 8 && (ntiles + 2 * tpw - 1) / (2 * tpw) * H * n >= 160) tpw *= 2;
    hipLaunchKernelGGL(dec_cross_prep_kernel, dim3((ntiles + tpw - 1) / tpw, H, n), dim3(256), 0, s, pb, B, T, tpw);
    LADIFF_LAUNCH_CHECK();
    return 0;
}

int launch_decoder_cross_apply(const float* x, const float* bo, const float* g2, const float* b2, const int32_t* counts, int B, int F,
                               int T, const float* gu_ws, float* y, float* ys, hipStream_t s, const int32_t* row_off, const float* g1,
                               const float* b1) {
    if (B == 0 || F == 0) return 0;
    if (T < 1 || T > TM) return LADIFF_ERR_SHAPE;
    const float* gu = gu_ws;
    const float* cc = gu_ws + (size_t)B * H * T * 2 * D;
    int chunks = (512 + B - 1) / B;
    if (chunks < 1) chunks = 1;
    if (chunks > (F + 3) / 4) chunks = (F + 3) / 4;
    const int rows_per_wg = ((F + chunks - 1) / chunks + 15) / 16 * 16;
    chunks = (F + rows_per_wg - 1) / rows_per_wg;
    const size_t lds = ((size_t)H * T * 2 * D + H * T) * sizeof(float);
    LADIFF_TRY(dec_cross_prepare());
#define LADIFF_DC_CASE(TT)                                                                                                   \
    case TT:                                                                                                                 \
        hipLaunchKernelGGL(dec_cross_apply_kernel<TT>, dim3(B, chunks), dim3(256), lds, s, x, gu, cc, counts, bo, g2, b2, F, \
                           rows_per_wg, y, ys, row_off, g1, b1);                                                                              \
        break;
    switch (T) {
        LADIFF_DC_CASE(1) LADIFF_DC_CASE(2) LADIFF_DC_CASE(3) LADIFF_DC_CASE(4)
        LADIFF_DC_CASE(5) LADIFF_DC_CASE(6) LADIFF_DC_CASE(7) LADIFF_DC_CASE(8)
        default: return LADIFF_ERR_SHAPE;
    }
#undef LADIFF_DC_CASE
    LADIFF_LAUNCH_CHECK();
    return 0;
}

int launch_decoder_out_cross(const float* att_s, const float* x0, const float* wo_s, const float* bo, const float* g1, const float* b1,
                             const float* bo_c, const float* g2, const float* b2, const int32_t* counts, int B, int F, int T,
                             const float* gu_ws, float* y, float* ys, hipStream_t s, const int32_t* row_off) {
    if (B == 0 || F == 0) return 0;
    if (T < 1 || T > TM) return LADIFF_ERR_SHAPE;
    int chunks = (256 + B - 1) / B;
    if (chunks > (F + OC_ROWS - 1) / OC_ROWS) chunks = (F + OC_ROWS - 1) / OC_ROWS;
    if (chunks < 1) chunks = 1;
    const int rows_per_wg = ((F + chunks - 1) / chunks + OC_ROWS - 1) / OC_ROWS * OC_ROWS;
    chunks = (F + rows_per_wg - 1) / rows_per_wg;
    LADIFF_TRY(dec_cross_prepare());
    OutCrossArgs a{att_s, x0, wo_s, bo, g1, b1, gu_ws, gu_ws + (size_t)B * H * T * 2 * D, bo_c, g2, b2, counts, row_off, y, ys, F, rows_per_wg, nullptr};
#ifdef LADIFF_STAMPS
    a.stamps = g_sys_stamps;
#endif
#define LADIFF_OC_CASE(TT) \
    case TT: hipLaunchKernelGGL(dec_out_cross_kernel<TT>, dim3(B, chunks), dim3(512), 0, s, a); break;
    switch (T) {
        LADIFF_OC_CASE(1) LADIFF_OC_CASE(2) LADIFF_OC_CASE(3) LADIFF_OC_CASE(4)
        LADIFF_OC_CASE(5) LADIFF_OC_CASE(6) LADIFF_OC_CASE(7) LADIFF_OC_CASE(8)
        default: return LADIFF_ERR_SHAPE;
    }
#undef LADIFF_OC_CASE
    LADIFF_LAUNCH_CHECK();
    return 0;
}

}
```

### ladiff_amd/csrc/decoder.hip

```cpp
#include "model.h"
#ifdef LADIFF_STAMPS
#include <cstdlib>
#endif

namespace ladiff {

#ifdef LADIFF_STAMPS
#define DEC_CUT() do { if (dec_cut >= 0 && ++dec_launched >= dec_cut) return 0; } while (0)
#else
#define DEC_CUT() do { } while (0)
#endif

constexpr int DEC_SMALL_ROWS = 4096;
std::atomic<int> g_dec_out_cross{1};
std::atomic<int> g_dec_fused_attn{1};
std::atomic<int> g_dec_final_split{1};
std::atomic<int> g_dec_small_rows_path{1};
std::atomic<int> g_dec_fused_mlp{1};

static GemmArgs lin(const float* A, int lda, const float* W, const float* bias, float* Y, int ldy, int M, int N, int K,
                    int act = ACT_NONE) {
    GemmArgs g;
    g.A = A; g.lda = lda; g.W = W; g.ldw = K; g.bias = bias; g.Y = Y; g.ldy = ldy; g.M = M; g.N = N; g.K = K; g.act = act;
    return g;
}

int vae_decode(const DecoderW& w, const DecoderW* wsp, const float* z, const int32_t* lengths, const int32_t* counts,
               const int32_t* row_off, int R, int B, int F, int T, int C, float* feats, float* ws, size_t ws_floats, hipStream_t s) {
    if (F < 1 || F > LADIFF_MAX_FRAMES || T < 1 || T > LADIFF_MAX_LATENTS || C < 1) return LADIFF_ERR_SHAPE;
    const bool ragged = row_off != nullptr;
    if (ragged && (R < 0 || (size_t)R > (size_t)B * F)) return LADIFF_ERR_SHAPE;
    const int M = ragged ? R : B * F;
    DecWs a = dec_layout(ws, B, (size_t)M, T);
    if (ws_floats < a.total) return LADIFF_ERR_WORKSPACE;
    if (M == 0) return 0;
#ifdef LADIFF_STAMPS
    const char* dec_cut_env = getenv("LADIFF_DEC_CUT");
    const int dec_cut = dec_cut_env ? atoi(dec_cut_env) : -1;
    int dec_launched = 0;
    if (dec_cut == 0) return 0;
#endif
    const bool sp = wsp != nullptr;
    if (!sp) { for (float*& t : a.Ps) t = nullptr; for (float*& t : a.SKs) t = nullptr; }
    float *const *P = a.P, *const *SK = a.SK, *const *Ps = a.Ps, *const *SKs = a.SKs;
    float *qkv = a.qkv, *att = a.att, *hid = a.hid, *kv = a.kv, *guws = a.guws, *pex = a.pex, *pexs = a.pexs, *qkv0 = a.qkv0;
    int32_t* row_out = a.row_out;
    const size_t kv_l = a.kv_layer, gu_l = a.gu_layer;

    {
        GemmArgs g[NL];
        DecCrossPrepBatch pb;
        for (int l = 0; l < NL; ++l) {
            const DecLayerW& L = w.layer[l];
            g[l] = lin(z, D, L.cross_attn.in_w + (size_t)D * D, L.cross_attn.in_b + D, kv + l * kv_l, 2 * D, T * B, 2 * D, D);
            pb.kv[l] = kv + l * kv_l; pb.wq[l] = L.cross_attn.in_w; pb.bq[l] = L.cross_attn.in_b; pb.wo[l] = L.cross_attn.out_w;
            pb.gu[l] = guws + l * gu_l;
        }
        LADIFF_TRY(launch_gemm_batch(g, NL, s)); DEC_CUT();
        LADIFF_TRY(launch_decoder_cross_prep(pb, NL, B, T, s)); DEC_CUT();
    }

    const bool small = sp && M < DEC_SMALL_ROWS && g_dec_small_rows_path;
    const bool fused_attn = sp && g_dec_fused_attn && (M >= DEC_SMALL_ROWS || g_dec_fused_attn == 2);
    auto krs = [&](const float* A, int K, const float* W, const float* bias, float* Y, float* Ys, int ldy, int N, int act,
                   const float* res, int rows) -> int {
        KrArgs g;
        g.A = A; g.lda = K; g.W = W; g.ldw = K; g.bias = bias; g.Y = Y; g.Ys = Ys; g.ldy = ldy; g.M = rows; g.N = N; g.K = K; g.act = act;
        g.res = res; g.ldres = D; g.split = 1;
        return launch_gemm_kr(g, s);
    };

    auto gemm_ln = [&](const float* A, int K, const float* W, const float* Wsp, const float* bias, const float* res,
                       const NormW& n1, const NormW* n2, float* dst, float* dsts) -> int {
        GemmArgs g = lin(A, K, sp ? Wsp : W, bias, dst, D, M, D, K);
        g.res = res; g.ldres = D;
        if (!sp) {
            g.ln_g = n1.g; g.ln_b = n1.b;
            if (n2) { g.ln2_g = n2->g; g.ln2_b = n2->b; }
            return launch_gemm(g, s);
        }
        g.split = 1;
        LADIFF_TRY(launch_gemm(g, s));
        RedArgs r;
        r.P = dst; r.M = M; r.mode = RED_LN; r.g = n1.g; r.b = n1.b; r.out = dst; r.outs = dsts;
        if (n2) { r.g2 = n2->g; r.b2 = n2->b; }
        return launch_reduce_rows(r, s);
    };

    if (ragged) { LADIFF_TRY(launch_broadcast_pe_ragged(w.query_pe, row_off, B, F, F, P[0], Ps[0], row_out, s)); DEC_CUT(); }
    else { LADIFF_TRY(launch_broadcast_pe(w.query_pe, B, F, P[0], Ps[0], s)); DEC_CUT(); }
    const float* cur = P[0]; const float* curs = Ps[0];
    for (int l = 0; l < NL; ++l) {
        const DecLayerW& L = w.layer[l];
        const DecLayerW& Ls = sp ? wsp->layer[l] : w.layer[l];
        const bool is_in = l < NSKIP, is_out = l > NSKIP, last = l == NL - 1;
        if (is_out) {
            const LinearW& sk = w.skip[l - NSKIP - 1];
            if (small) {
                RowLnArgs g;
                g.A = curs; g.lda = D; g.A2 = SKs[NL - 1 - l]; g.lda2 = D; g.K1 = D; g.W = wsp->skip[l - NSKIP - 1].w; g.ldw = 2 * D; g.bias = sk.b;
                g.Y = P[3]; g.Ys = Ps[3]; g.ldy = D; g.M = M; g.K = 2 * D;
                LADIFF_TRY(launch_gemm_rowln(g, s)); DEC_CUT();
            } else {
            GemmArgs g = lin(sp ? curs : cur, D, sp ? wsp->skip[l - NSKIP - 1].w : sk.w, sk.b, P[3], D, M, D, 2 * D);
            g.A2 = sp ? SKs[NL - 1 - l] : SK[NL - 1 - l]; g.lda2 = D; g.K1 = D;
            g.split = sp ? 1 : 0; g.Ys = Ps[3];
            LADIFF_TRY(launch_gemm(g, s)); DEC_CUT();
            }
            cur = P[3]; curs = Ps[3];
        }
        const bool shared = l == 0;
        if (shared) {
            LADIFF_TRY(launch_broadcast_pe(w.query_pe, 1, F, pex, sp ? pexs : nullptr, s)); DEC_CUT();
            if (small) { LADIFF_TRY(krs(pexs, D, Ls.self_attn.in_w, L.self_attn.in_b, qkv0, nullptr, 3 * D, 3 * D, ACT_NONE, nullptr, F)); DEC_CUT(); }
            else {
            GemmArgs g = lin(sp ? pexs : pex, D, Ls.self_attn.in_w, L.self_attn.in_b, qkv0, 3 * D, F, 3 * D, D);
            g.split = sp ? 1 : 0;
            LADIFF_TRY(launch_gemm(g, s)); DEC_CUT();
            }
        } else if (fused_attn) {
        } else if (small) {
            LADIFF_TRY(krs(curs, D, Ls.self_attn.in_w, L.self_attn.in_b, qkv, nullptr, 3 * D, 3 * D, ACT_NONE, nullptr, M)); DEC_CUT();
        } else {
            GemmArgs g = lin(sp ? curs : cur, D, Ls.self_attn.in_w, L.self_attn.in_b, qkv, 3 * D, M, 3 * D, D);
            g.split = sp ? 1 : 0;
            LADIFF_TRY(launch_gemm(g, s)); DEC_CUT();
        }
        const float* qkv_l = shared ? qkv0 : qkv;
        if (fused_attn && !shared) { LADIFF_TRY(launch_dec_qkv_attn(curs, Ls.self_attn.in_w, L.self_attn.in_b, lengths, row_off, att, B, F, 1, s)); DEC_CUT(); }
        else if (sp) { LADIFF_TRY(launch_self_attention_split(qkv_l, lengths, nullptr, att, B, F, H, 0, 1, s, row_off, shared)); DEC_CUT(); }
        else { LADIFF_TRY(launch_decoder_self_attention(qkv_l, lengths, nullptr, att, B, F, 0, s, row_off, shared)); DEC_CUT(); }
        const NormW* n1_late = nullptr;
        if (sp && !small && g_dec_out_cross) {
            LADIFF_TRY(launch_decoder_out_cross(att, cur, Ls.self_attn.out_w, L.self_attn.out_b, L.norm1.g, L.norm1.b, L.cross_attn.out_b,
                                                L.norm2.g, L.norm2.b, counts, B, F, T, guws + l * gu_l, P[2], Ps[2], s, row_off)); DEC_CUT();
        } else {
        if (sp) {
            if (small) { LADIFF_TRY(krs(att, D, Ls.self_attn.out_w, L.self_attn.out_b, P[1], nullptr, D, D, ACT_NONE, cur, M)); DEC_CUT(); }
            else {
            GemmArgs g = lin(att, D, Ls.self_attn.out_w, L.self_attn.out_b, P[1], D, M, D, D);
            g.res = cur; g.ldres = D; g.split = 1;
            LADIFF_TRY(launch_gemm(g, s)); DEC_CUT();
            }
            n1_late = &L.norm1;
        } else {
            LADIFF_TRY(gemm_ln(att, D, L.self_attn.out_w, Ls.self_attn.out_w, L.self_attn.out_b, cur, L.norm1, nullptr, P[1], nullptr)); DEC_CUT();
        }
        LADIFF_TRY(launch_decoder_cross_apply(P[1], L.cross_attn.out_b, L.norm2.g, L.norm2.b, counts, B, F, T, guws + l * gu_l, P[2],
                                              Ps[2], s, row_off, n1_late ? n1_late->g : nullptr, n1_late ? n1_late->b : nullptr)); DEC_CUT();
        }
        float* dst = is_in ? SK[l] : P[0];
        float* dsts = is_in ? SKs[l] : Ps[0];
        if (sp && g_dec_fused_mlp && (M >= dec_mlp_min_rows() || g_dec_fused_mlp == 2)) {
            LADIFF_TRY(launch_dec_mlp(Ps[2], P[2], Ls.lin1.w, L.lin1.b, Ls.lin2.w, L.lin2.b, L.norm3.g, L.norm3.b,
                                      last ? w.norm.g : nullptr, last ? w.norm.b : nullptr, dst, dsts, M, s)); DEC_CUT();
        } else if (small) {
            LADIFF_TRY(krs(Ps[2], D, Ls.lin1.w, L.lin1.b, nullptr, hid, FF, FF, ACT_GELU, nullptr, M)); DEC_CUT();
            LADIFF_TRY(krs(hid, FF, Ls.lin2.w, nullptr, qkv, nullptr, D, D, ACT_NONE, nullptr, M)); DEC_CUT();
            RedArgs r;
            r.P = qkv; r.S = 4; r.M = M; r.bias = L.lin2.b; r.res = P[2]; r.mode = RED_LN; r.g = L.norm3.g; r.b = L.norm3.b;
            r.out = dst; r.outs = dsts;
            if (last) { r.g2 = w.norm.g; r.b2 = w.norm.b; }
            LADIFF_TRY(launch_reduce_rows(r, s));
        } else {
            GemmArgs g = lin(sp ? Ps[2] : P[2], D, Ls.lin1.w, L.lin1.b, sp ? nullptr : hid, FF, M, FF, D, ACT_GELU);
            g.split = sp ? 1 : 0; if (sp) g.Ys = hid;
            LADIFF_TRY(launch_gemm(g, s)); DEC_CUT();
            LADIFF_TRY(gemm_ln(hid, FF, L.lin2.w, Ls.lin2.w, L.lin2.b, P[2], L.norm3, last ? &w.norm : nullptr, dst, dsts)); DEC_CUT();
        }
        cur = dst; curs = dsts;
    }
    if (sp && M >= DEC_SMALL_ROWS && g_dec_final_split) {
        const int Np = (C + 127) / 128 * 128;
        if ((size_t)M * Np > a.hid_floats || (size_t)Np * (D + 1) > a.qkv_floats) return LADIFF_ERR_SHAPE;
        float* wpad = qkv; float* bpad = qkv + (size_t)Np * D;
        LADIFF_TRY(launch_pad_rows(wsp->final_layer.w, w.final_layer.b, wpad, bpad, C, Np, s)); DEC_CUT();
        GemmArgs g = lin(curs, D, wpad, bpad, hid, Np, M, Np, D);
        g.split = 1;
        LADIFF_TRY(launch_gemm(g, s)); DEC_CUT();
        return launch_scatter_feats(hid, Np, C, M, F, ragged ? nullptr : lengths, ragged ? row_out : nullptr, feats, s);
    }
    GemmArgs g = lin(cur, D, w.final_layer.w, w.final_layer.b, feats, C, M, C, D);
    if (ragged) g.row_map = row_out;
    else { g.row_len = lengths; g.rows_per_item = F; }
    return launch_gemm(g, s);
}

}
```

### ladiff_amd/csrc/denoiser.hip

```cpp
#include "model.h"

namespace ladiff {

static std::vector<std::string> block_prefixes(const char* root) {
    std::vector<std::string> v;
    for (int i = 0; i < NSKIP; ++i) v.push_back(std::string(root) + ".input_blocks." + std::to_string(i));
    v.push_back(std::string(root) + ".middle_block");
    for (int i = 0; i < NSKIP; ++i) v.push_back(std::string(root) + ".output_blocks." + std::to_string(i));
    return v;
}
static void wb(std::vector<std::string>& v, const std::string& p) { v.push_back(p + ".weight"); v.push_back(p + ".bias"); }
static void mha_names(std::vector<std::string>& v, const std::string& p) {
    v.push_back(p + ".in_proj_weight"); v.push_back(p + ".in_proj_bias"); wb(v, p + ".out_proj");
}
static void styl_names(std::vector<std::string>& v, const std::string& p) {
    wb(v, p + ".emb_layers.1"); wb(v, p + ".norm"); wb(v, p + ".out_layers.2");
}

const std::vector<std::string>& denoiser_param_names() {
    static const std::vector<std::string> names = [] {
        std::vector<std::string> v;
        wb(v, "time_embedding.linear_1"); wb(v, "time_embedding.linear_2"); wb(v, "emb_proj.1");
        v.push_back("query_pos.pe"); v.push_back("mem_pos.pe");
        wb(v, "encoder.norm");
        for (const auto& p : block_prefixes("encoder")) {
            wb(v, p + ".ca_block.norm"); wb(v, p + ".ca_block.text_norm");
            wb(v, p + ".ca_block.query"); wb(v, p + ".ca_block.key"); wb(v, p + ".ca_block.value");
            styl_names(v, p + ".ca_block.proj_out");
            wb(v, p + ".ffn.linear1"); wb(v, p + ".ffn.linear2");
            styl_names(v, p + ".ffn.proj_out");
            mha_names(v, p + ".sa_block.self_attn");
            wb(v, p + ".sa_block.linear1"); wb(v, p + ".sa_block.linear2");
            wb(v, p + ".sa_block.norm1"); wb(v, p + ".sa_block.norm2");
        }
        for (int i = 0; i < NSKIP; ++i) wb(v, "encoder.linear_blocks." + std::to_string(i));
        return v;
    }();
    return names;
}

const std::vector<std::string>& decoder_param_names() {
    static const std::vector<std::string> names = [] {
        std::vector<std::string> v;
        v.push_back("query_pos_decoder.pe");
        for (const auto& p : block_prefixes("decoder")) {
            mha_names(v, p + ".self_attn"); mha_names(v, p + ".multihead_attn");
            wb(v, p + ".linear1"); wb(v, p + ".linear2");
            wb(v, p + ".norm1"); wb(v, p + ".norm2"); wb(v, p + ".norm3");
        }
        for (int i = 0; i < NSKIP; ++i) wb(v, "decoder.linear_blocks." + std::to_string(i));
        wb(v, "decoder.norm"); wb(v, "final_layer");
        return v;
    }();
    return names;
}

const std::vector<std::string>& encoder_param_names() {
    static const std::vector<std::string> names = [] {
        std::vector<std::string> v;
        v.push_back("global_motion_token"); v.push_back("query_pos_encoder.pe");
        for (const auto& p : block_prefixes("encoder")) {
            mha_names(v, p + ".self_attn");
            wb(v, p + ".linear1"); wb(v, p + ".linear2");
            wb(v, p + ".norm1"); wb(v, p + ".norm2");
        }
        for (int i = 0; i < NSKIP; ++i) wb(v, "encoder.linear_blocks." + std::to_string(i));
        wb(v, "encoder.norm"); wb(v, "skel_embedding");
        return v;
    }();
    return names;
}

int denoiser_time_tables(const DenoiserW& w, const float* sinus, int n, float* tables, float* ws, size_t ws_floats,
                         hipStream_t s) {
    const DenTimeWs t = den_time_layout(ws, n);
    if (ws_floats < t.total) return LADIFF_ERR_WORKSPACE;
    float *h1 = t.h1, *temb = t.temb, *semb = t.semb;
    LADIFF_TRY(launch_gemm(lin(sinus, TEXT_DIM, w.time1, h1, D, n, D, TEXT_DIM, ACT_SILU), s));
    LADIFF_TRY(launch_gemm(lin(h1, D, w.time2, temb, D, n, D, D), s));
    LADIFF_TRY(launch_silu(temb, semb, (size_t)n * D, s));
    for (int l = 0; l < NL; ++l) {
        const DenLayerW& L = w.layer[l];
        float* base = tables + (size_t)l * DEN_LAYER_STRIDE;
        LADIFF_TRY(launch_gemm(lin(semb, D, L.ca_proj.emb, base + DEN_OFF_CA_MOD, DEN_STEP_STRIDE, n, 2 * D, D), s));
        LADIFF_TRY(launch_gemm(lin(semb, D, L.ffn_proj.emb, base + DEN_OFF_FFN_MOD, DEN_STEP_STRIDE, n, 2 * D, D), s));
        LinearW kvw{L.sa_attn.in_w + (size_t)D * D, L.sa_attn.in_b + D};
        LADIFF_TRY(launch_gemm(lin(temb, D, kvw, base + DEN_OFF_TIME_KV, DEN_STEP_STRIDE, n, 2 * D, D), s));
    }
    return 0;
}

static int denoiser_text_cache_general(const DenoiserW& w, const float* text, int B2, int N, float* cache, float* ws, size_t ws_floats,
                                       hipStream_t s) {
    const int R = B2 * N;
    const DenTextWs t = den_text_layout(ws, B2, 1, N);
    if (ws_floats < t.total) return LADIFF_ERR_WORKSPACE;
    const DenTextCache c = den_text_cache_layout(cache, B2, 1, N);
    float *rl = t.rl, *tn = t.tn, *key = t.key, *val = t.val, *tproj = c.tproj, *tkv = c.tkv, *catt = c.catt;
    LADIFF_TRY(launch_relu(text, rl, (size_t)R * TEXT_DIM, s));
    LADIFF_TRY(launch_gemm(lin(rl, TEXT_DIM, w.emb_proj, tproj, D, R, D, TEXT_DIM), s));
    for (int l = 0; l < NL; ++l) {
        const DenLayerW& L = w.layer[l];
        LinearW kvw{L.sa_attn.in_w + (size_t)D * D, L.sa_attn.in_b + D};
        LADIFF_TRY(launch_gemm(lin(tproj, D, kvw, tkv + (size_t)l * R * 2 * D, 2 * D, R, 2 * D, D), s));
        LADIFF_TRY(launch_layernorm(tproj, L.ca_text_norm.g, L.ca_text_norm.b, tn, R, s));
        LADIFF_TRY(launch_gemm(lin(tn, D, L.ca_key, key, D, R, D, D), s));
        LADIFF_TRY(launch_gemm(lin(tn, D, L.ca_value, val, D, R, D, D), s));
        LADIFF_TRY(launch_lca_kv(key, val, B2, N, catt + (size_t)l * B2 * H * DH * DH, s));
    }
    return 0;
}

int denoiser_text_static(const DenoiserW& w, const float* text, int B2, float* cache, float* ws, size_t ws_floats, hipStream_t s) {
    const DenTextWs t = den_text_layout(ws, B2, 0, 1);
    if (ws_floats < t.total) return LADIFF_ERR_WORKSPACE;
    const DenTextCache c = den_text_cache_layout(cache, B2, 0, 1);
    float *rl = t.rl, *tn = t.tn, *tproj = c.tproj, *tkv = c.tkv, *nval = c.nval;
    LADIFF_TRY(launch_relu(text, rl, (size_t)B2 * TEXT_DIM, s));
    LADIFF_TRY(launch_gemm(lin(rl, TEXT_DIM, w.emb_proj, tproj, D, B2, D, TEXT_DIM), s));
    GemmArgs kv[NL], val[NL];
    RowBatch ln;
    for (int l = 0; l < NL; ++l) {
        const DenLayerW& L = w.layer[l];
        LinearW kvw{L.sa_attn.in_w + (size_t)D * D, L.sa_attn.in_b + D};
        kv[l] = lin(tproj, D, kvw, tkv + (size_t)l * B2 * 2 * D, 2 * D, B2, 2 * D, D);
        ln.a[l] = tproj; ln.g[l] = L.ca_text_norm.g; ln.b[l] = L.ca_text_norm.b; ln.y[l] = tn + (size_t)l * B2 * D;
        val[l] = lin(tn + (size_t)l * B2 * D, D, L.ca_value, nval + (size_t)l * B2 * D, D, B2, D, D);
        val[l].ln_g = L.ca_proj.norm.g; val[l].ln_b = L.ca_proj.norm.b;
    }
    LADIFF_TRY(launch_gemm_batch(kv, NL, s));
    LADIFF_TRY(launch_layernorm_batch(ln, NL, B2, s));
    return launch_gemm_batch(val, NL, s);
}

int denoiser_ctab(const DenoiserW& w, const float* tables_lo, int n, float* cache, int B2, float* u, size_t u_floats, hipStream_t s,
                  const DenoiserW* wsp) {
    const int R = B2 + 1;
    const size_t u_all = den_text_layout(nullptr, B2, n, 1).u_floats;
    if (u_floats < u_all / NL) return LADIFF_ERR_WORKSPACE;
    const DenTextCache c = den_text_cache_layout(cache, B2, n, 1);
    const float* nval = c.nval;
    float* ctab = c.ctab;
    if (u_floats >= u_all) {
        RowBatch rb;
        GemmArgs g[NL];
        for (int l = 0; l < NL; ++l) {
            const DenLayerW& L = w.layer[l];
            float* ul = u + (size_t)l * n * R * D;
            rb.a[l] = nval + (size_t)l * B2 * D; rb.g[l] = L.ca_proj.norm.b;
            rb.b[l] = tables_lo + (size_t)l * DEN_LAYER_STRIDE + DEN_OFF_CA_MOD; rb.y[l] = ul;
            g[l] = lin(ul, D, L.ca_proj.out, ctab + (size_t)l * n * R * D, D, n * R, D, D);
            if (wsp != nullptr) { g[l].W = wsp->layer[l].ca_proj.out.w; g[l].split = 1; }
        }
        LADIFF_TRY(launch_ca_table_input_batch(rb, NL, DEN_STEP_STRIDE, n, B2, s, wsp != nullptr ? 1 : 0));
        return launch_gemm_batch(g, NL, s);
    }
    for (int l = 0; l < NL; ++l) {
        const DenLayerW& L = w.layer[l];
        LADIFF_TRY(launch_ca_table_input(nval + (size_t)l * B2 * D, L.ca_proj.norm.b, tables_lo + (size_t)l * DEN_LAYER_STRIDE + DEN_OFF_CA_MOD,
                                         DEN_STEP_STRIDE, n, B2, u, s));
        LADIFF_TRY(launch_gemm(lin(u, D, L.ca_proj.out, ctab + (size_t)l * n * R * D, D, n * R, D, D), s));
    }
    return 0;
}

int denoiser_text_cache(const DenoiserW& w, const float* text, int B2, const float* tables, int n, float* cache,
                        float* ws, size_t ws_floats, hipStream_t s, int ntxt) {
    if (ntxt > 1) return denoiser_text_cache_general(w, text, B2, ntxt, cache, ws, ws_floats, s);
    const DenTextWs t = den_text_layout(ws, B2, n, 1);
    if (ws_floats < t.total) return LADIFF_ERR_WORKSPACE;
    LADIFF_TRY(denoiser_text_static(w, text, B2, cache, ws, ws_floats, s));
    return denoiser_ctab(w, tables, n, cache, B2, t.u, t.u_floats, s, nullptr);
}

int linear_cross_attention(const DenoiserW& w, int layer, const float* x, const float* xf, const float* emb, const int32_t* counts,
                           int B, int T, int N, float* out, float* ws, size_t ws_floats, hipStream_t s) {
    if (layer < 0 || layer >= NL || T < 1 || T > LADIFF_MAX_LATENTS || N < 1) return LADIFF_ERR_SHAPE;
    const LcaWs a = lca_layout(ws, B, T, N);
    if (ws_floats < a.total) return LADIFF_ERR_WORKSPACE;
    const DenLayerW& L = w.layer[layer];
    const int R = B * N, M = B * T;
    float *tn = a.tn, *key = a.key, *val = a.val, *catt = a.catt, *xn = a.xn, *q = a.q, *semb = a.semb, *mod = a.mod;
    LADIFF_TRY(launch_layernorm(xf, L.ca_text_norm.g, L.ca_text_norm.b, tn, R, s));
    LADIFF_TRY(launch_gemm(lin(tn, D, L.ca_key, key, D, R, D, D), s));
    LADIFF_TRY(launch_gemm(lin(tn, D, L.ca_value, val, D, R, D, D), s));
    LADIFF_TRY(launch_lca_kv(key, val, B, N, catt, s));
    LADIFF_TRY(launch_layernorm(x, L.ca_norm.g, L.ca_norm.b, xn, M, s));
    LADIFF_TRY(launch_gemm(lin(xn, D, L.ca_query, q, D, M, D, D), s));
    LADIFF_TRY(launch_silu(emb, semb, (size_t)B * D, s));
    LADIFF_TRY(launch_gemm(lin(semb, D, L.ca_proj.emb, mod, 2 * D, B, 2 * D, D), s));
    LADIFF_TRY(launch_lca_apply(q, catt, counts, B, 0, B, T, mod, 0, 2 * D, nullptr, L.ca_proj.norm.g, L.ca_proj.norm.b, xn, s));
    GemmArgs g = lin(xn, D, L.ca_proj.out, out, D, M, D, D);
    g.res = x; g.ldres = D;
    return launch_gemm(g, s);
}


int denoiser_forward(const DenoiserW& w, const DenoiserW* wsp, const float* tables, const int32_t* d_step, const float* cache,
                     int n_steps, const float* sample, int Bs, int dup, int T, const int32_t* counts, float* eps, float* ws,
                     size_t ws_floats, hipStream_t s, int b_lo, int b_n, int loop_mode, int ntxt, const int32_t* d_base,
                     const float* dctab) {
    const int B2 = Bs * dup;
    const bool per_sample = d_step == nullptr;
    if (per_sample && (dctab == nullptr || ntxt != 1 || loop_mode)) return LADIFF_ERR_ARG;
    if (b_n < 0) { b_lo = 0; b_n = B2; }
    const int M = b_n * T;
    if (T < 1 || T > LADIFF_MAX_LATENTS || b_lo < 0 || b_lo + b_n > B2) return LADIFF_ERR_SHAPE;
    if (M == 0) return 0;
    DenForwardWs a = den_forward_layout(ws, (size_t)M);
    if (ws_floats < a.total) return LADIFF_ERR_WORKSPACE;
    eps += (size_t)b_lo * T * D;
    const bool sp = wsp != nullptr;
    const size_t MD = (size_t)M * D;
    if (!sp) { for (float*& t : a.Ps) t = nullptr; for (float*& t : a.SKs) t = nullptr; }
    float *const *P = a.P, *const *SK = a.SK, *const *Ps = a.Ps, *const *SKs = a.SKs;
    float *qkv = a.qkv, *att = a.att, *hid = a.hid, *part = a.part;
    const float* tkv = den_cache_tkv(cache, B2, ntxt);
    const float* ctab = den_cache_ctab(cache, B2, ntxt);
    const int R = B2 + 1;
    auto gemm = [&](KrArgs g) { g.split = sp ? 1 : 0; return launch_gemm_kr(g, s); };
    auto red = [&](const float* src, int S, const float* bias, const float* res, const NormW* n, float* out, float* outs) {
        RedArgs r;
        r.P = src; r.S = S; r.M = M; r.bias = bias; r.res = res; r.out = out; r.outs = outs;
        if (n != nullptr) { r.mode = RED_LN; r.g = n->g; r.b = n->b; }
        return r;
    };

    if (!loop_mode) LADIFF_TRY(launch_add_pe(sample, w.query_pe, Bs, b_lo, b_n, T, P[0], Ps[0], s));
    const float* cur = P[0]; const float* curs = Ps[0];
    for (int l = 0; l < NL; ++l) {
        const DenLayerW& L = w.layer[l];
        const DenLayerW& Ls = sp ? wsp->layer[l] : w.layer[l];
        const float* tl = tables + (size_t)l * DEN_LAYER_STRIDE;
        const bool is_in = l < NSKIP, is_out = l > NSKIP;
        if (is_out) {
            const LinearW& sk = w.skip[l - NSKIP - 1];
            const LinearW& sks = sp ? wsp->skip[l - NSKIP - 1] : sk;
            if (sp) {
                RowLnArgs g;
                g.A = curs; g.lda = D; g.A2 = SKs[NL - 1 - l]; g.lda2 = D; g.K1 = D; g.W = sks.w; g.ldw = 2 * D; g.bias = sk.b;
                g.Y = P[3]; g.Ys = Ps[3]; g.ldy = D; g.M = M; g.K = 2 * D;
                LADIFF_TRY(launch_gemm_rowln(g, s));
            } else {
                KrArgs g = kr(cur, D, sks.w, nullptr, part, D, M, D, 2 * D);
                g.A2 = SK[NL - 1 - l]; g.lda2 = D; g.K1 = D;
                LADIFF_TRY(gemm(g));
                LADIFF_TRY(launch_reduce_rows(red(part, 2, sk.b, nullptr, nullptr, P[3], Ps[3]), s));
            }
            cur = P[3]; curs = Ps[3];
        }
        const float* att_op = att;
        if (sp && ntxt == 1 && !per_sample) {
            LADIFF_TRY(launch_qkv_attention(curs, Ls.sa_attn.in_w, L.sa_attn.in_b, tkv + (size_t)l * B2 * 2 * D, tl,
                                            DEN_OFF_TIME_KV, DEN_STEP_STRIDE, d_step, counts, Bs, b_lo, b_n, T, att, s));
        } else {
            LADIFF_TRY(gemm(kr(sp ? curs : cur, D, Ls.sa_attn.in_w, L.sa_attn.in_b, qkv, 3 * D, M, 3 * D, D)));
            if (ntxt > 1) {
                LADIFF_TRY(launch_denoiser_self_attention_general(qkv, tkv + (size_t)l * B2 * ntxt * 2 * D, ntxt, tl, DEN_OFF_TIME_KV,
                                                                  DEN_STEP_STRIDE, d_step, counts, Bs, b_lo, b_n, T, att, s));
                if (sp) { LADIFF_TRY(launch_split_rows(att, hid, M, D, s)); att_op = hid; }
            } else
                LADIFF_TRY(launch_denoiser_self_attention(qkv, tkv + (size_t)l * B2 * 2 * D, tl, DEN_OFF_TIME_KV, DEN_STEP_STRIDE,
                                                          d_step, counts, Bs, b_lo, b_n, T, att, sp ? 1 : 0, s));
        }
        if (sp) {
            RowLnArgs g;
            g.A = att_op; g.lda = D; g.W = Ls.sa_attn.out_w; g.ldw = D; g.bias = L.sa_attn.out_b; g.res = cur; g.ldres = D;
            g.ln_g = L.sa_norm1.g; g.ln_b = L.sa_norm1.b; g.Y = P[2]; g.Ys = Ps[2]; g.ldy = D; g.M = M; g.K = D;
            LADIFF_TRY(launch_gemm_rowln(g, s));
        } else {
            KrArgs g = kr(att, D, Ls.sa_attn.out_w, L.sa_attn.out_b, P[1], D, M, D, D);
            g.res = cur; g.ldres = D;
            LADIFF_TRY(gemm(g));
            LADIFF_TRY(launch_reduce_rows(red(P[1], 1, nullptr, nullptr, &L.sa_norm1, P[2], Ps[2]), s));
        }
        {
            KrArgs g = kr(sp ? Ps[2] : P[2], D, Ls.sa_lin1.w, L.sa_lin1.b, sp ? nullptr : hid, FF, M, FF, D, ACT_RELU);
            if (sp) g.Ys = hid;
            LADIFF_TRY(gemm(g));
        }
        LADIFF_TRY(gemm(kr(hid, FF, Ls.sa_lin2.w, nullptr, part, D, M, D, FF)));
        const float* x3 = P[1];
        if (ntxt > 1) {
            LADIFF_TRY(launch_reduce_rows(red(part, 4, L.sa_lin2.b, P[2], &L.sa_norm2, P[1], nullptr), s));
            if (sp) LADIFF_TRY(launch_reduce_rows(red(P[1], 1, nullptr, nullptr, &L.ca_norm, P[2], Ps[2]), s));
            else LADIFF_TRY(launch_layernorm(P[1], L.ca_norm.g, L.ca_norm.b, P[2], M, s));
            LADIFF_TRY(gemm(kr(sp ? Ps[2] : P[2], D, Ls.ca_query.w, L.ca_query.b, att, D, M, D, D)));
            LADIFF_TRY(launch_lca_apply(att, ctab + (size_t)l * B2 * H * DH * DH, counts, Bs, b_lo, b_n, T, tl + DEN_OFF_CA_MOD,
                                        DEN_STEP_STRIDE, 0, d_step, L.ca_proj.norm.g, L.ca_proj.norm.b, P[2], s));
            if (sp) LADIFF_TRY(launch_split_rows(P[2], Ps[2], M, D, s));
            KrArgs g = kr(sp ? Ps[2] : P[2], D, Ls.ca_proj.out.w, L.ca_proj.out.b, qkv, D, M, D, D);
            g.res = P[1]; g.ldres = D; g.Ys = sp ? Ps[1] : nullptr;
            LADIFF_TRY(gemm(g));
            x3 = qkv;
        } else {
            RedArgs r = red(part, 4, L.sa_lin2.b, P[2], &L.sa_norm2, P[1], Ps[1]);
            r.mode = RED_LN_ADD; r.counts = counts; r.Bs = Bs; r.T = T; r.b_off = b_lo;
            if (per_sample) { r.tab = dctab + (size_t)l * B2 * 2 * D; r.tab_step_stride = 2 * D; r.pad_row = 1; }
            else { r.tab = ctab + (size_t)l * n_steps * R * D; r.tab_step_stride = R * D; r.pad_row = B2; r.d_step = d_step; r.d_base = d_base; }
            LADIFF_TRY(launch_reduce_rows(r, s, per_sample));
        }
        {
            KrArgs g = kr(sp ? Ps[1] : x3, D, Ls.ffn1.w, L.ffn1.b, sp ? nullptr : hid, FF, M, FF, D, ACT_GELU);
            if (sp) g.Ys = hid;
            LADIFF_TRY(gemm(g));
        }
        LADIFF_TRY(gemm(kr(hid, FF, Ls.ffn2.w, nullptr, part, D, M, D, FF)));
        float* dst = is_in ? SK[l] : P[0];
        float* dsts = is_in ? SKs[l] : Ps[0];
        if (sp && !per_sample) {
            CombineGemmArgs g;
            g.P = part; g.plane = MD; g.S = 4; g.bias2 = L.ffn2.b; g.ln_g = L.ffn_proj.norm.g; g.ln_b = L.ffn_proj.norm.b;
            g.tab = tl + DEN_OFF_FFN_MOD; g.tab_step_stride = DEN_STEP_STRIDE; g.d_step = d_step;
            g.W = Ls.ffn_proj.out.w; g.ldw = D; g.bias = L.ffn_proj.out.b; g.res = x3; g.ldres = D;
            g.Y = dst; g.Ys = dsts; g.ldy = D; g.M = M;
            LADIFF_TRY(launch_combine_gemm(g, s));
        } else {
            RedArgs r = red(part, 4, L.ffn2.b, nullptr, &L.ffn_proj.norm, P[2], Ps[2]);
            r.mode = RED_LN_MOD; r.tab = tl + DEN_OFF_FFN_MOD; r.tab_step_stride = DEN_STEP_STRIDE; r.d_step = d_step;
            if (per_sample) { r.T = T; r.b_off = b_lo; }
            LADIFF_TRY(launch_reduce_rows(r, s, per_sample));
            KrArgs g = kr(sp ? Ps[2] : P[2], D, Ls.ffn_proj.out.w, L.ffn_proj.out.b, dst, D, M, D, D);
            g.res = x3; g.ldres = D; g.Ys = dsts;
            LADIFF_TRY(gemm(g));
        }
        cur = dst; curs = dsts;
    }
    if (loop_mode) return 0;
    return launch_layernorm(cur, w.norm.g, w.norm.b, eps, M, s);
}

}
```

### ladiff_amd/csrc/gemm.h

```cpp
#pragma once
#include "common.h"

namespace ladiff {

struct GemmArgs {
    const float* A = nullptr;  int lda = 0;
    const float* A2 = nullptr; int lda2 = 0;
    int K1 = 0;
    const float* W = nullptr;  int ldw = 0;
    const float* bias = nullptr;
    float* Y = nullptr;        int ldy = 0;
    float* Ys = nullptr;
    int split = 0;
    int M = 0, N = 0, K = 0;
    int act = ACT_NONE;
    const float* res = nullptr; int ldres = 0;
    const float* ln_g = nullptr; const float* ln_b = nullptr;
    const float* ln2_g = nullptr; const float* ln2_b = nullptr;
    const float* mod = nullptr;
    const int32_t* d_step = nullptr; int mod_stride = 0;
    int post_act = ACT_NONE;
    const int32_t* row_len = nullptr; int rows_per_item = 0;
    const int32_t* row_map = nullptr;
    int ksplit = 1; size_t plane = 0;
};

int launch_gemm(const GemmArgs& a, hipStream_t stream);
constexpr int GEMM_BATCH_MAX = 9;
struct GemmBatch { GemmArgs a[GEMM_BATCH_MAX]; };
int launch_gemm_batch(const GemmArgs* list, int n, hipStream_t stream);
int launch_gemm_big_batch(const GemmBatch& b, int n, hipStream_t stream);
bool gemm_big_supported(const GemmArgs& a);
int launch_gemm_big(const GemmArgs& a, hipStream_t stream);

}
```

### ladiff_amd/csrc/gemm_big.hip

```cpp
#include "gemm.h"

namespace ladiff {

namespace {
constexpr int BKB = 32;
template <int N> __device__ __forceinline__ void wait_vm() { asm volatile("s_waitcnt vmcnt(%0)" ::"n"(N) : "memory"); }
__device__ __forceinline__ void dma16(const float* g, float* l) {
    __builtin_amdgcn_global_load_lds(g, (__attribute__((address_space(3))) void*)l, 16, 0, 0);
}
}

template <int BM, int BN, int WM, int WN, bool LN>
__device__ __forceinline__ void gemm_big_body(const GemmArgs& p) {
    constexpr int NW = 4;
    static_assert(WM * WN == NW, "four waves");
    constexpr int TMW = BM / WM, TNW = BN / WN, RM = TMW / 32, RN = TNW / 32;
    constexpr int ROWS = BM + BN;
    constexpr int STAGE = ROWS * BKB;
    constexpr int GRP = 8 * NW;
    constexpr int GA = BM / GRP, GT = ROWS / GRP;
    static_assert(BM % GRP == 0 && BN % GRP == 0, "tiles are multiples of 32 rows");
    constexpr int CLD = BN + 4;
    constexpr int LDSF = (2 * STAGE > BM * CLD) ? 2 * STAGE : BM * CLD;
    constexpr int LPR = BN / 4;
    constexpr int RPI = 64 / LPR;
    constexpr int EI = BM / NW / RPI;
    static_assert(!LN || BN == 256, "LayerNorm needs whole rows");

    __shared__ __attribute__((aligned(1024))) float lds[LDSF];

    const int tid = threadIdx.x, lane = tid & 63;
    const int wave = __builtin_amdgcn_readfirstlane(tid >> 6);
    const int wm = wave / WN, wn = wave % WN;
    const int nbn = p.N / BN;
    const int nbm = (p.M + BM - 1) / BM;
    const int xcd = blockIdx.x & 7, local = blockIdx.x >> 3;
    const int bm = (local / nbn) * 8 + xcd, bn = local % nbn;
    if (bm >= nbm) return;
    const int row0 = bm * BM, col0 = bn * BN;
    const int nk = p.K / BKB;

    const int rl = 8 * wave + (lane >> 3);
    const int kl = (((lane & 7) ^ ((rl >> 1) & 7)) << 2);
    float* const lbase = lds + 8 * wave * BKB;
    auto issue = [&](int kt, int buf) __attribute__((always_inline)) {
        const int k0 = kt * BKB;
        const float* abase; int ald;
        if (k0 < p.K1) { abase = p.A + k0; ald = p.lda; } else { abase = p.A2 + (k0 - p.K1); ald = p.lda2; }
#pragma unroll
        for (int g = 0; g < GT; ++g) {
            const float* src;
            if (g < GA) {
                int gr = row0 + GRP * g + rl; gr = gr < p.M ? gr : p.M - 1;
                src = abase + (size_t)gr * ald + kl;
            } else {
                src = p.W + (size_t)(col0 + GRP * (g - GA) + rl) * p.ldw + k0 + kl;
            }
            dma16(src, lbase + buf * STAGE + GRP * g * BKB);
        }
    };

    f32x16 acc[RM][RN];
#pragma unroll
    for (int i = 0; i < RM; ++i)
#pragma unroll
        for (int j = 0; j < RN; ++j)
#pragma unroll
            for (int r = 0; r < 16; ++r) acc[i][j][r] = 0.f;

    const int frow = lane & 31, fk = lane >> 5;
    auto compute = [&](int buf) __attribute__((always_inline)) {
        const float* sa = lds + buf * STAGE + (wm * TMW) * BKB;
        const float* sb = lds + buf * STAGE + (BM + wn * TNW) * BKB;
#pragma unroll
        for (int g = 0; g < BKB / 8; ++g) {
            const int c = 2 * g + fk;
            f32x4 fa[RM], fb[RN];
#pragma unroll
            for (int i = 0; i < RM; ++i) { const int r = i * 32 + frow; fa[i] = ld4(sa + r * BKB + ((c ^ ((r >> 1) & 7)) << 2)); }
#pragma unroll
            for (int j = 0; j < RN; ++j) { const int r = j * 32 + frow; fb[j] = ld4(sb + r * BKB + ((c ^ ((r >> 1) & 7)) << 2)); }
#pragma unroll
            for (int e = 0; e < 4; ++e)
#pragma unroll
                for (int i = 0; i < RM; ++i)
#pragma unroll
                    for (int j = 0; j < RN; ++j)
                        acc[i][j] = __builtin_amdgcn_mfma_f32_32x32x2f32(fa[i][e], fb[j][e], acc[i][j], 0, 0, 0);
        }
    };

    const int er = wave * (BM / NW) + lane / LPR;
    const int ec = 4 * (lane % LPR);
    f32x4 rv[EI];
#pragma unroll
    for (int e = 0; e < EI; ++e) rv[e] = f32x4{0.f, 0.f, 0.f, 0.f};

    issue(0, 0);
    for (int kt = 0; kt < nk; ++kt) {
        const int buf = kt & 1;
        wait_vm<0>();
        __builtin_amdgcn_s_barrier();
        if (kt + 1 < nk) issue(kt + 1, buf ^ 1);
        if (kt == nk - 1 && p.res != nullptr) {
#pragma unroll
            for (int e = 0; e < EI; ++e) {
                const int gr = row0 + er + e * RPI;
                if (gr < p.M) rv[e] = ld4(p.res + (size_t)gr * p.ldres + col0 + ec);
            }
        }
        compute(buf);
    }
    __builtin_amdgcn_s_barrier();

    float* ct = lds;
#pragma unroll
    for (int i = 0; i < RM; ++i)
#pragma unroll
        for (int j = 0; j < RN; ++j)
#pragma unroll
            for (int r = 0; r < 16; ++r)
                ct[(wm * TMW + i * 32 + (r & 3) + 8 * (r >> 2) + 4 * (lane >> 5)) * CLD + wn * TNW + j * 32 + (lane & 31)] = acc[i][j][r];
    asm volatile("s_waitcnt vmcnt(0) lgkmcnt(0)" ::: "memory");
    __builtin_amdgcn_s_barrier();
#pragma unroll
    for (int e = 0; e < EI; ++e) reg_touch(rv[e]);

    f32x4 bv = {0.f, 0.f, 0.f, 0.f};
    if (p.bias != nullptr) bv = ld4(p.bias + col0 + ec);
    f32x4 g1 = bv, b1 = bv, g2 = bv, b2 = bv;
    if constexpr (LN) {
        g1 = ld4(p.ln_g + ec); b1 = ld4(p.ln_b + ec);
        if (p.ln2_g != nullptr) { g2 = ld4(p.ln2_g + ec); b2 = ld4(p.ln2_b + ec); }
    }
    act_dispatch(p.act, [&](auto ACT) __attribute__((always_inline)) {
#pragma unroll
    for (int e = 0; e < EI; ++e) {
        const int lr = er + e * RPI;
        const int gr = row0 + lr;
        f32x4 v = ld4(ct + lr * CLD + ec);
#pragma unroll
        for (int q = 0; q < 4; ++q) v[q] = act_c<decltype(ACT)::value>(v[q] + bv[q]) + rv[e][q];
        if constexpr (LN) {
#pragma unroll
            for (int pass = 0; pass < 2; ++pass) {
                if (pass == 1 && p.ln2_g == nullptr) break;
                const float mean = wave_sum((v[0] + v[1]) + (v[2] + v[3])) * (1.f / 256.f);
                float sq = 0.f;
#pragma unroll
                for (int q = 0; q < 4; ++q) { const float d = v[q] - mean; sq += d * d; }
                const float rstd = rsqrtf(wave_sum(sq) * (1.f / 256.f) + LN_EPS);
#pragma unroll
                for (int q = 0; q < 4; ++q) v[q] = (v[q] - mean) * rstd * (pass ? g2[q] : g1[q]) + (pass ? b2[q] : b1[q]);
            }
        }
        if (gr < p.M) st4(p.Y + (size_t)gr * p.ldy + col0 + ec, v);
    }
    });
}

template <int BM, int BN>
__device__ __forceinline__ void gemm_big_split_body(const GemmArgs& p) {
    constexpr int NW = 4, WM = 2, WN = 2;
    constexpr int TMW = BM / WM, TNW = BN / WN, RM = TMW / 16, RN = TNW / 16;
    constexpr int ROWS = BM + BN;
    constexpr int STAGE = ROWS * 32;
    constexpr int GRP = 8 * NW;
    constexpr int GA = BM / GRP, GT = ROWS / GRP;
    constexpr int CLD = BN + 4;
    constexpr int LPR = BN / 4, RPI = 64 / LPR, EI = BM / NW / RPI;
    constexpr int LDSF = (2 * STAGE > BM * CLD) ? 2 * STAGE : BM * CLD;

    __shared__ __attribute__((aligned(1024))) float lds[LDSF];

    const int tid = threadIdx.x, lane = tid & 63;
    const int wave = __builtin_amdgcn_readfirstlane(tid >> 6);
    const int wm = wave / WN, wn = wave % WN;
    const int argM = pin_s(p.M), argK1 = pin_s(p.K1), ldy = pin_s(p.ldy), act = pin_s(p.act);
    float* const argY = pin_s(p.Y); float* const argYs = pin_s(p.Ys);
    const int nbn = p.N / BN;
    const int nbm = (argM + BM - 1) / BM;
    const int xcd = blockIdx.x & 7, local = blockIdx.x >> 3;
    const int bm = (local / nbn) * 8 + xcd, bn = local % nbn;
    if (bm >= nbm) return;
    const int row0 = bm * BM, col0 = bn * BN;
    const int ksplit = pin_s(p.ksplit), kz = ksplit > 1 ? (int)blockIdx.y : 0;
    const int nk_all = p.K / 32, nk = nk_all / ksplit, kt0 = kz * nk;

    const int rl = 8 * wave + (lane >> 3);
    const int cs = (lane & 7) ^ ((rl >> 1) & 7);
    const int kl = (cs < 4 ? cs * 4 : 32 + (cs - 4) * 4);
    float* const lbase = lds + 8 * wave * 32;
    auto issue = [&](int ktl, int buf) __attribute__((always_inline)) {
        const int kt = kt0 + ktl;
        const int k0 = (kt >> 1) * 64, hf = (kt & 1) * 16;
        const float* abase; int ald;
        if (k0 < argK1) { abase = p.A + k0; ald = p.lda; } else { abase = p.A2 + (k0 - argK1); ald = p.lda2; }
#pragma unroll
        for (int g = 0; g < GT; ++g) {
            const float* src;
            if (g < GA) {
                int gr = row0 + GRP * g + rl; gr = gr < argM ? gr : argM - 1;
                src = abase + (size_t)gr * ald + hf + kl;
            } else {
                src = p.W + (size_t)(col0 + GRP * (g - GA) + rl) * p.ldw + k0 + hf + kl;
            }
            dma16(src, lbase + buf * STAGE + GRP * g * 32);
        }
    };

    f32x4 acc[RM][RN];
#pragma unroll
    for (int i = 0; i < RM; ++i)
#pragma unroll
        for (int j = 0; j < RN; ++j) acc[i][j] = f32x4{0.f, 0.f, 0.f, 0.f};

    const int frow = lane & 15, fk = lane >> 4;
    const int sw = (frow >> 1) & 7;
    auto compute = [&](int buf) __attribute__((always_inline)) {
        const float* sa = lds + buf * STAGE + (wm * TMW) * 32;
        const float* sb = lds + buf * STAGE + (BM + wn * TNW) * 32;
        s16x8 ah[RM], al[RM], bh[RN], bl[RN];
#pragma unroll
        for (int i = 0; i < RM; ++i) {
            const int r = i * 16 + frow;
            ah[i] = __builtin_bit_cast(s16x8, ld4(sa + r * 32 + ((fk ^ sw) << 2)));
            al[i] = __builtin_bit_cast(s16x8, ld4(sa + r * 32 + (((4 + fk) ^ sw) << 2)));
        }
#pragma unroll
        for (int j = 0; j < RN; ++j) {
            const int r = j * 16 + frow;
            bh[j] = __builtin_bit_cast(s16x8, ld4(sb + r * 32 + ((fk ^ sw) << 2)));
            bl[j] = __builtin_bit_cast(s16x8, ld4(sb + r * 32 + (((4 + fk) ^ sw) << 2)));
        }
#pragma unroll
        for (int i = 0; i < RM; ++i)
#pragma unroll
            for (int j = 0; j < RN; ++j) acc[i][j] = MFMA16_S16(al[i], bh[j], acc[i][j], 0, 0, 0);
#pragma unroll
        for (int i = 0; i < RM; ++i)
#pragma unroll
            for (int j = 0; j < RN; ++j) acc[i][j] = MFMA16_S16(ah[i], bl[j], acc[i][j], 0, 0, 0);
#pragma unroll
        for (int i = 0; i < RM; ++i)
#pragma unroll
            for (int j = 0; j < RN; ++j) acc[i][j] = MFMA16_S16(ah[i], bh[j], acc[i][j], 0, 0, 0);
    };

    const int er = wave * (BM / NW) + lane / LPR;
    const int ec = 4 * (lane % LPR);
    f32x4 rv[EI];
#pragma unroll
    for (int e = 0; e < EI; ++e) rv[e] = f32x4{0.f, 0.f, 0.f, 0.f};
    f32x4 bv = {0.f, 0.f, 0.f, 0.f};

    issue(0, 0);
    for (int kt = 0; kt < nk; ++kt) {
        const int buf = kt & 1;
        wait_vm<0>();
        __builtin_amdgcn_s_barrier();
        if (kt + 1 < nk) issue(kt + 1, buf ^ 1);
        if (kt == nk - 1 && ksplit == 1) {
            if (p.bias != nullptr) bv = ld4(p.bias + col0 + ec);
            if (p.res != nullptr) {
#pragma unroll
                for (int e = 0; e < EI; ++e) {
                    const int gr = row0 + er + e * RPI;
                    if (gr < argM) rv[e] = ld4(p.res + (size_t)gr * p.ldres + col0 + ec);
                }
            }
        }
        compute(buf);
    }
    __builtin_amdgcn_s_barrier();

    float* ct = lds;
#pragma unroll
    for (int i = 0; i < RM; ++i)
#pragma unroll
        for (int j = 0; j < RN; ++j)
#pragma unroll
            for (int r = 0; r < 4; ++r)
                ct[(wm * TMW + i * 16 + 4 * (lane >> 4) + r) * CLD + wn * TNW + j * 16 + (lane & 15)] = acc[i][j][r];
    asm volatile("s_waitcnt vmcnt(0) lgkmcnt(0)" ::: "memory");
    __builtin_amdgcn_s_barrier();
    reg_touch(bv);
#pragma unroll
    for (int e = 0; e < EI; ++e) reg_touch(rv[e]);

    if (ksplit > 1) {
        float* const Yz = argY + (size_t)kz * p.plane;
#pragma unroll
        for (int e = 0; e < EI; ++e) {
            const int lr = er + e * RPI;
            const int gr = row0 + lr;
            if (gr < argM) st4g(Yz + (size_t)gr * ldy + col0 + ec, ld4(ct + lr * CLD + ec));
        }
        return;
    }
    act_dispatch(act, [&](auto ACT) __attribute__((always_inline)) {
#pragma unroll
        for (int e = 0; e < EI; ++e) {
            const int lr = er + e * RPI;
            const int gr = row0 + lr;
            f32x4 v = ld4(ct + lr * CLD + ec);
#pragma unroll
            for (int q = 0; q < 4; ++q) v[q] = act_c<decltype(ACT)::value>(v[q] + bv[q]) + rv[e][q];
            if (gr < argM) {
                if (argY != nullptr) st4g(argY + (size_t)gr * ldy + col0 + ec, v);
                if (argYs != nullptr) store_split4g(argYs + (size_t)gr * ldy, col0 + ec, v);
            }
        }
    });
}

template <int BM, int BN>
__global__ __launch_bounds__(256, 2) void gemm_big_split_kernel(const GemmArgs p) { gemm_big_split_body<BM, BN>(p); }
template <int BM, int BN>
__global__ __launch_bounds__(256, 2) void gemm_big_split_batch_kernel(const GemmBatch b) { gemm_big_split_body<BM, BN>(b.a[blockIdx.y]); }

template <int BM, int BN, int WM, int WN, bool LN>
__global__ __launch_bounds__(256) void gemm_big_kernel(const GemmArgs p) { gemm_big_body<BM, BN, WM, WN, LN>(p); }
template <int BM, int BN, int WM, int WN, bool LN>
__global__ __launch_bounds__(256) void gemm_big_batch_kernel(const GemmBatch b) { gemm_big_body<BM, BN, WM, WN, LN>(b.a[blockIdx.y]); }

template <int BM, int BN, int WM, int WN, bool LN>
static int launch_big_batch(const GemmBatch& b, int n, hipStream_t s) {
    const GemmArgs& a = b.a[0];
    const int nbm = (a.M + BM - 1) / BM, nbn = a.N / BN;
    const int grid = ((nbm + 7) / 8) * 8 * nbn;
    hipLaunchKernelGGL((gemm_big_batch_kernel<BM, BN, WM, WN, LN>), dim3(grid, n), dim3(256), 0, s, b);
    LADIFF_LAUNCH_CHECK();
    return 0;
}

template <int BM, int BN, int WM, int WN, bool LN>
static int launch_big(const GemmArgs& a, hipStream_t s) {
    const int nbm = (a.M + BM - 1) / BM, nbn = a.N / BN;
    const int grid = ((nbm + 7) / 8) * 8 * nbn;
    hipLaunchKernelGGL((gemm_big_kernel<BM, BN, WM, WN, LN>), dim3(grid), dim3(256), 0, s, a);
    LADIFF_LAUNCH_CHECK();
    return 0;
}

bool gemm_big_supported(const GemmArgs& a) {
    if (a.split) return a.M > 0 && a.K % 64 == 0 && a.K1 % 64 == 0 && a.N % 128 == 0 && a.lda % 4 == 0 && a.ldw % 4 == 0 && (!a.A2 || a.lda2 % 4 == 0) &&
                        a.ldy % 64 == 0 && !a.ln_g && !a.mod && !a.row_len && !a.row_map && a.post_act == ACT_NONE && (a.Y || a.Ys);
    if (a.M < 4096 || a.K % BKB || a.K1 % BKB || (a.lda % 4) || (a.ldw % 4) || (a.A2 && (a.lda2 % 4))) return false;
    if ((a.ldy % 4) || (a.res && (a.ldres % 4)) || a.mod || a.row_len || a.row_map || a.post_act != ACT_NONE) return false;
    if (a.ln_g != nullptr) return a.N == 256;
    return a.N % 128 == 0;
}

int launch_gemm_big(const GemmArgs& a, hipStream_t s) {
    if (a.split) {
        const int nbm = (a.M + 127) / 128, nbn = a.N / 128;
        const int ks = a.ksplit > 1 ? a.ksplit : 1;
        if (ks > 1 && ((a.K / 32) % ks != 0 || a.Y == nullptr || a.Ys != nullptr || a.plane == 0)) return LADIFF_ERR_ARG;
        if (nbm * nbn <= 256 && a.M > 64) {
            const int nbm64 = (a.M + 63) / 64;
            hipLaunchKernelGGL((gemm_big_split_kernel<64, 128>), dim3(((nbm64 + 7) / 8) * 8 * nbn, ks), dim3(256), 0, s, a);
        } else {
            hipLaunchKernelGGL((gemm_big_split_kernel<128, 128>), dim3(((nbm + 7) / 8) * 8 * nbn, ks), dim3(256), 0, s, a);
        }
        LADIFF_LAUNCH_CHECK();
        return 0;
    }
    if (a.ksplit > 1) return LADIFF_ERR_ARG;
    if (a.ln_g != nullptr) return launch_big<64, 256, 2, 2, true>(a, s);
    return launch_big<128, 128, 2, 2, false>(a, s);
}

int launch_gemm_big_batch(const GemmBatch& b, int n, hipStream_t s) {
    for (int i = 0; i < n; ++i) if (b.a[i].ksplit > 1) return LADIFF_ERR_ARG;
    if (b.a[0].split) {
        const GemmArgs& a = b.a[0];
        const int nbm = (a.M + 127) / 128, nbn = a.N / 128;
        hipLaunchKernelGGL((gemm_big_split_batch_kernel<128, 128>), dim3(((nbm + 7) / 8) * 8 * nbn, n), dim3(256), 0, s, b);
        LADIFF_LAUNCH_CHECK();
        return 0;
    }
    if (b.a[0].ln_g != nullptr) return launch_big_batch<64, 256, 2, 2, true>(b, n, s);
    return launch_big_batch<128, 128, 2, 2, false>(b, n, s);
}

}
```

### ladiff_amd/csrc/kernels.h

```cpp
#pragma once
#include "common.h"
#include "noise_gen.h"

namespace ladiff {

enum RedMode : int { RED_PLAIN = 0, RED_LN = 1, RED_LN_ADD = 2, RED_LN_MOD = 3 };
struct RedArgs {
    const float* P = nullptr;
    const float* bias = nullptr; const float* res = nullptr;
    const float* g = nullptr; const float* b = nullptr;
    const float* tab = nullptr;
    const int32_t* d_step = nullptr;
    const int32_t* counts = nullptr;
    float* out = nullptr; float* outs = nullptr;
    const int32_t* d_base = nullptr;
    const float* g2 = nullptr; const float* b2 = nullptr;
    size_t plane = 0;
    int S = 1, mode = RED_PLAIN, tab_step_stride = 0, Bs = 1, T = 1, pad_row = 0, b_off = 0, M = 0;
};
int launch_reduce_rows(const RedArgs& a, hipStream_t s, bool per_sample = false);
int launch_split_rows(const float* x, float* y, int R, int K, hipStream_t s);
int launch_gather_rows(const float* src, const int32_t* index, int n_rows, int row_floats, float* dst, hipStream_t s);
int launch_split_range_stats(const float* const* xs, const int64_t* counts, int n, int64_t max_count, unsigned long long* stats,
                             hipStream_t s);
int launch_layernorm(const float* x, const float* g, const float* b, float* y, int M, hipStream_t s);
constexpr int DEC_PREP_MAX = 9;
struct DecCrossPrepBatch { const float* kv[DEC_PREP_MAX]; const float* wq[DEC_PREP_MAX]; const float* bq[DEC_PREP_MAX];
                           const float* wo[DEC_PREP_MAX]; float* gu[DEC_PREP_MAX]; };
constexpr int ROW_BATCH_MAX = 9;
struct RowBatch { const float* a[ROW_BATCH_MAX]; const float* g[ROW_BATCH_MAX]; const float* b[ROW_BATCH_MAX]; float* y[ROW_BATCH_MAX]; };
int launch_layernorm_batch(const RowBatch& rb, int n, int M, hipStream_t s);
int launch_ca_table_input_batch(const RowBatch& rb, int n_layers, int step_stride, int n, int B2, hipStream_t s, int split_out = 0);
int launch_ca_table_input(const float* nval, const float* beta, const float* mod, int step_stride, int n, int B2, float* u,
                          hipStream_t s);
int launch_add_pe(const float* sample, const float* pe, int Bs, int b_off, int b_n, int T, float* x, float* xs, hipStream_t s);
int launch_broadcast_pe(const float* pe, int B, int F, float* x, float* xs, hipStream_t s);
int launch_broadcast_pe_ragged(const float* pe, const int32_t* row_off, int B, int F, int F_out, float* x, float* xs, int32_t* row_out,
                               hipStream_t s);
int launch_relu(const float* x, float* y, size_t n, hipStream_t s);
int launch_pad_rows(const float* src, const float* srcb, float* dst, float* dstb, int C, int Np, hipStream_t s);
int launch_zero_fill(float* x, size_t n, hipStream_t s);
int launch_silu(const float* x, float* y, size_t n, hipStream_t s);
int launch_sinusoid(const int64_t* t, int n, float* out, hipStream_t s);
int launch_cfg_step(const float* eps, float* lat, const float* coef, const int32_t* d_step, const float* noise,
                    float g, int cfg, int B, int T, hipStream_t s, const float* gs = nullptr, const NoiseGen& gen = NoiseGen{0u, 0u, 0u, 0},
                    float* x0_prev = nullptr);
int launch_advance(int32_t* d_step, hipStream_t s);
int launch_step_tail(float* x, float* xs, const float* ng, const float* nb, float* lat, const float* coef, int32_t* d_step,
                     const float* noise, const float* pe, float g, int cfg, int B, int T, hipStream_t s, const NoiseGen& gen = NoiseGen{0u, 0u, 0u, 0},
                     const float* gs = nullptr,
                     float* x0_prev = nullptr);
int launch_noise_fill(const NoiseGen& gen, int step0, int n, int B, int T, float* out, hipStream_t s);
int launch_init_latents(const float* noise, const int32_t* counts, float sigma, float* lat, int B, int T, hipStream_t s);
int launch_init_latents_gen(const NoiseGen& gen, const int32_t* counts, float sigma, float* lat, int B, int T, hipStream_t s);
int launch_finalize_latents(const float* lat, const int32_t* counts, float* z, int B, int T, hipStream_t s, const unsigned* status = nullptr);

int launch_dec_qkv_attn(const float* xs, const float* w, const float* bias, const int32_t* lengths, const int32_t* row_off, float* out,
                        int B, int F, int split_out, hipStream_t s);
int launch_scatter_feats(const float* tmp, int ldt, int C, int M, int F, const int32_t* row_len, const int32_t* row_map, float* feats,
                         hipStream_t s);
int launch_pad_cols(const float* x, float* y, int R, int C, int Cp, hipStream_t s);
int launch_dvae_pad_cols(const float* x, const int32_t* slot, const float* values, int n, float* y, int B, int F, int C, int Cp,
                         hipStream_t s);
int launch_encoder_assemble(const float* token, const float* emb, const float* pe, const int32_t* lengths,
                            const int32_t* counts, int B, int F, int T, float* x, float* xs, uint32_t* keybits, hipStream_t s);
int launch_encoder_finalize(const float* out, const float* eps, const int32_t* counts, int B, int T, int S, float* mu, float* sd,
                            float* latent, hipStream_t s);

int launch_lca_kv(const float* key, const float* value, int B, int N, float* att, hipStream_t s);
int launch_lca_apply(const float* q, const float* att, const int32_t* counts, int Bs, int b_off, int b_n, int T, const float* mod,
                     int step_stride, int sample_stride, const int32_t* d_step, const float* g, const float* be, float* u,
                     hipStream_t s);
int launch_denoiser_self_attention_general(const float* qkv, const float* text_kv, int N, const float* tables, int kv_off,
                                           int step_stride, const int32_t* d_step, const int32_t* counts, int Bs, int b_off,
                                           int b_n, int T, float* out, hipStream_t s);

int launch_decoder_cross_prep(const DecCrossPrepBatch& pb, int n, int B, int T, hipStream_t s);
int launch_decoder_out_cross(const float* att_s, const float* x0, const float* wo_s, const float* bo, const float* g1, const float* b1,
                             const float* bo_c, const float* g2, const float* b2, const int32_t* counts, int B, int F, int T,
                             const float* gu_ws, float* y, float* ys, hipStream_t s, const int32_t* row_off);
int launch_decoder_cross_apply(const float* x, const float* bo, const float* g2, const float* b2, const int32_t* counts, int B, int F,
                               int T, const float* gu_ws, float* y, float* ys, hipStream_t s, const int32_t* row_off = nullptr,
                               const float* g1 = nullptr, const float* b1 = nullptr);

int launch_feats2joints(const float* feats, const float* mean, const float* stdv, int B, int F, int C, int J, float* joints,
                        hipStream_t s);

int launch_joint_ape_ave(const float* rst, const float* ref, const int32_t* lengths, int B, int F, int J, const int32_t* part_idx,
                         float factor, float* seq_rows, double* acc, hipStream_t s);
int launch_joint_mr(const float* rst, const float* ref, int B, int F, int J, float* seq_rows, double* acc, hipStream_t s);

int launch_vae_losses(const float* m_rst, const float* m_ref, size_t n_feat, const float* j_rst, const float* j_ref, size_t n_joint,
                      const float* mu, const float* sd, size_t n_lat, double l_rec, double l_joint, double l_kl, double* part, int blocks,
                      double* batch, double* acc, hipStream_t s);

int launch_denoiser_self_attention(const float* qkv, const float* text_kv, const float* tables, int kv_off,
                                   int step_stride, const int32_t* d_step, const int32_t* counts, int Bs, int b_off,
                                   int b_n, int T, float* out, int split_out, hipStream_t s);
int launch_decoder_self_attention(const float* qkv, const int32_t* lengths, const uint32_t* keybits, float* out, int B, int F,
                                  int split_out, hipStream_t s, const int32_t* row_off = nullptr, int shared_qkv = 0);
int launch_self_attention(const float* qkv, const int32_t* lengths, const uint32_t* keybits, float* out, int B, int F, int nheads,
                          int causal, int split_out, hipStream_t s, const int32_t* row_off = nullptr);
int launch_self_attention_split(const float* qkv, const int32_t* lengths, const uint32_t* keybits, float* out, int B, int F,
                                 int nheads, int causal, int split_out, hipStream_t s, const int32_t* row_off = nullptr, int shared_qkv = 0);
int launch_decoder_cross_attention(const float* q, const float* kv, const int32_t* counts, float* out, int B, int F,
                                   int T, int split_out, hipStream_t s);

}
```

### ladiff_amd/csrc/model.h

```cpp
#pragma once
#include <atomic>
#include "gemm.h"
#include "gemm_kr.h"
#include "graph_key.h"
#include "kernels.h"
#include "systolic_plan.h"
#include "weights.h"
#include "workspace.h"

namespace ladiff {

inline GemmArgs lin(const float* A, int lda, const LinearW& l, float* Y, int ldy, int M, int N, int K, int act = ACT_NONE) {
    GemmArgs g;
    g.A = A; g.lda = lda; g.W = l.w; g.ldw = K; g.bias = l.b; g.Y = Y; g.ldy = ldy; g.M = M; g.N = N; g.K = K; g.act = act;
    return g;
}
inline KrArgs kr(const float* A, int lda, const float* W, const float* b, float* Y, int ldy, int M, int N, int K, int act = ACT_NONE) {
    KrArgs g;
    g.A = A; g.lda = lda; g.W = W; g.ldw = K; g.bias = b; g.Y = Y; g.ldy = ldy; g.M = M; g.N = N; g.K = K; g.act = act;
    return g;
}

int denoiser_time_tables(const DenoiserW& w, const float* sinus, int n, float* tables, float* ws, size_t ws_floats, hipStream_t s);
int denoiser_text_cache(const DenoiserW& w, const float* text, int B2, const float* tables, int n_steps, float* cache,
                        float* ws, size_t ws_floats, hipStream_t s, int ntxt = 1);
int denoiser_forward(const DenoiserW& w, const DenoiserW* w_split, const float* tables, const int32_t* d_step,
                     const float* cache, int n_steps, const float* sample, int Bs, int dup, int T, const int32_t* counts, float* eps, float* ws,
                     size_t ws_floats, hipStream_t s, int b_lo = 0, int b_n = -1, int loop_mode = 0, int ntxt = 1,
                     const int32_t* d_base = nullptr, const float* dctab = nullptr);
int denoiser_text_static(const DenoiserW& w, const float* text, int B2, float* cache, float* ws, size_t ws_floats, hipStream_t s);
int denoiser_ctab(const DenoiserW& w, const float* tables_lo, int n, float* cache, int B2, float* u, size_t u_floats, hipStream_t s,
                  const DenoiserW* w_split = nullptr);
int linear_cross_attention(const DenoiserW& w, int layer, const float* x, const float* xf, const float* emb, const int32_t* counts,
                           int B, int T, int N, float* out, float* ws, size_t ws_floats, hipStream_t s);

int denoiser_forward_timesteps(const DenoiserW& w, const DenoiserW* w_split, const float* text, const int64_t* timesteps, const float* sample,
                               int B2, int T, const int32_t* counts, float* eps, float* ws, size_t ws_floats, hipStream_t s);
int launch_q_sample(const float* z, const int64_t* ts, const float* acp, int n_train, const int32_t* counts, const NoiseGen& gen, float* noise,
                    float* noisy, int B, int T, hipStream_t s);
int launch_diffusion_losses(const float* pred, const float* noise, size_t n, double lambda_inst, double* part, int blocks, double* batch,
                            double* acc, hipStream_t s);

struct Sampler;
int diffusion_reverse(Sampler* sp, const DenoiserW& w, const DenoiserW* w_split, const ReverseArgs& a);

extern std::atomic<int> g_dec_fused_mlp;
extern std::atomic<int> g_dec_small_rows_path;
extern std::atomic<int> g_dec_final_split;
extern std::atomic<int> g_dec_out_cross;
extern std::atomic<int> g_stage_plan;
extern std::atomic<int> g_poll_pause;
extern std::atomic<int> g_stage_delay;
extern std::atomic<int> g_pace;
extern std::atomic<int> g_look_ahead_from, g_small_upto;
extern std::atomic<int> g_dec_fused_attn;
extern std::atomic<int> g_mlp_variant;
int dec_mlp_prepare();
int dec_qkv_attn_prepare();
int dec_cross_prepare();
int dec_mlp_min_rows();
int vae_decode(const DecoderW& w, const DecoderW* w_split, const float* z, const int32_t* lengths, const int32_t* counts,
               const int32_t* row_off, int R, int B, int F, int T, int C, float* feats, float* ws, size_t ws_floats, hipStream_t s);

int launch_dec_mlp(const float* xs, const float* x, const float* w1, const float* b1, const float* w2, const float* b2, const float* g3,
                   const float* be3, const float* g4, const float* be4, float* y, float* ys, int M, hipStream_t s);

int vae_encode(const EncoderW& w, const EncoderW* w_split, const float* features, const int32_t* lengths,
               const int32_t* counts, const float* eps, int B, int F, int T, int C, float* mu, float* sd, float* latent, float* ws,
               size_t ws_floats, hipStream_t s, const int32_t* slot = nullptr, const float* values = nullptr, int n_values = 0);

#ifdef LADIFF_STAMPS
extern unsigned long long* g_sys_stamps;
extern int g_sys_probe;
#endif
bool sys_supported(int B, int T, int cfg, bool split);
extern std::atomic<int> g_waves16;
extern std::atomic<int> g_handoff;
int sys_reset_status(float* ws, hipStream_t s);
extern std::atomic<int> g_xcd_local;
int sys_build_stages(const DenoiserW& W, const DenoiserW& WS, float* ws, int MR, int NB, std::vector<unsigned char>& host);
int launch_systolic_loop(const DenoiserW& W, float* ws, const float* tables, const float* tkv, const float* ctab, int n_ctab,
                         const float* coef, const float* noise, float* lat, const int32_t* counts, float gscale, int B, int T,
                         int step_lo, int n, int fp32, int MR, int NB, hipStream_t s, int cfg = 1, int fault_wg = -1,
                         unsigned long long timeout_ticks = 0, const NoiseGen& gen = NoiseGen{0u, 0u, 0u, 0},
                         const float* gscales = nullptr,
                         float* x0_prev = nullptr);

int launch_qkv_attention(const float* x, const float* w, const float* bias, const float* text_kv, const float* tables,
                         int kv_off, int step_stride, const int32_t* d_step, const int32_t* counts, int Bs, int b_off,
                         int b_n, int T, float* out, hipStream_t s);

int clip_text_encode(const ClipW& w, const ClipW* w_split, int n_layers, int vocab, const int64_t* ids, int B, int S, int L,
                     float* out, float* ws, size_t ws_floats, hipStream_t s, const int32_t* seq_len = nullptr,
                     const int32_t* row_off = nullptr, const int32_t* row_seq = nullptr, int total_rows = 0);

const std::vector<std::string>& t2m_move_param_names();
const std::vector<std::string>& t2m_motion_param_names();
const std::vector<std::string>& t2m_text_param_names();
int t2m_movement_encode(const float* const* w, const float* feats, int ld, int B, int F, int Cin, float* out, float* ws,
                        size_t ws_floats, hipStream_t s);
int t2m_motion_encode(const float* const* w, const float* mov, const int32_t* m_lens, int B, int T, float* out, float* ws,
                      size_t ws_floats, hipStream_t s);
int t2m_text_encode(const float* const* w, const float* word_embs, const float* pos_onehot, const int32_t* cap_lens, int B, int L,
                    float* out, float* ws, size_t ws_floats, hipStream_t s);

}
```

### ladiff_amd/csrc/workspace.h

```cpp
#pragma once
#include <cstddef>
#include <cstdint>

#include "systolic_plan.h"
#include "weights.h"

namespace ladiff {

struct Carver {
    float* base;
    size_t align, off = 0;
    explicit Carver(float* b, size_t a = 1) : base(b), align(a) {}
    float* take(size_t floats) {
        float* p = base ? base + off : nullptr;
        off += (floats + align - 1) / align * align;
        return p;
    }
};
inline int pad32(int c) { return (c + 31) / 32 * 32; }

struct XfmrWs {
    float *P[4], *SK[NSKIP], *Ps[4], *SKs[NSKIP], *qkv, *att, *hid;
    size_t qkv_floats, hid_floats;
};
inline void carve_xfmr(Carver& c, size_t M, XfmrWs& x) {
    const size_t MD = M * D;
    for (float*& p : x.P) p = c.take(MD);
    for (float*& p : x.SK) p = c.take(MD);
    for (float*& p : x.Ps) p = c.take(MD);
    for (float*& p : x.SKs) p = c.take(MD);
    x.qkv_floats = 3 * MD; x.hid_floats = M * FF;
    x.qkv = c.take(x.qkv_floats);
    x.att = c.take(MD);
    x.hid = c.take(x.hid_floats);
}

constexpr int DEN_OFF_CA_MOD = 0;
constexpr int DEN_OFF_FFN_MOD = 2 * D;
constexpr int DEN_OFF_TIME_KV = 4 * D;
constexpr int DEN_LAYER_STRIDE = 6 * D;
constexpr int DEN_STEP_STRIDE = NL * DEN_LAYER_STRIDE;
inline size_t den_tables_floats(int n_steps) { return (size_t)n_steps * DEN_STEP_STRIDE; }

struct DenForwardWs : XfmrWs { float* part; size_t total; };
inline DenForwardWs den_forward_layout(float* ws, size_t M) {
    DenForwardWs L;
    Carver c(ws);
    carve_xfmr(c, M, L);
    L.part = c.take(4 * M * D);
    L.total = c.off;
    return L;
}
inline size_t den_forward_ws_floats(int B2, int T) { return den_forward_layout(nullptr, (size_t)B2 * T).total; }

struct DenTimeWs { float *h1, *temb, *semb; size_t total; };
inline DenTimeWs den_time_layout(float* ws, int n) {
    DenTimeWs L;
    Carver c(ws);
    L.h1 = c.take((size_t)n * D); L.temb = c.take((size_t)n * D); L.semb = c.take((size_t)n * D);
    L.total = c.off;
    return L;
}

struct DenTextWs { float *rl, *tn, *u, *key, *val; size_t u_floats, total; };
inline DenTextWs den_text_layout(float* ws, int B2, int n, int ntxt) {
    DenTextWs L{};
    Carver c(ws);
    const size_t R = (size_t)B2 * ntxt;
    L.rl = c.take(R * TEXT_DIM);
    if (ntxt > 1) {
        L.tn = c.take(R * D); L.key = c.take(R * D); L.val = c.take(R * D);
    } else {
        L.tn = c.take((size_t)NL * B2 * D);
        L.u_floats = (size_t)NL * n * (B2 + 1) * D;
        L.u = c.take(L.u_floats);
    }
    L.total = c.off;
    return L;
}
inline size_t den_text_ws_floats(int B2, int n_steps, int ntxt = 1) { return den_text_layout(nullptr, B2, n_steps, ntxt).total; }

struct DenTextCache { float *tproj, *tkv, *nval, *ctab, *catt; size_t total; };
inline DenTextCache den_text_cache_layout(float* cache, int B2, int n, int ntxt) {
    DenTextCache L{};
    Carver c(cache);
    const size_t R = (size_t)B2 * ntxt;
    L.tproj = c.take(R * D);
    L.tkv = c.take((size_t)NL * R * 2 * D);
    if (ntxt > 1) {
        L.catt = c.take((size_t)NL * B2 * H * DH * DH);
    } else {
        L.nval = c.take((size_t)NL * B2 * D);
        L.ctab = c.take((size_t)NL * n * (B2 + 1) * D);
    }
    L.total = c.off;
    return L;
}
inline size_t den_text_cache_floats(int B2, int n_steps, int ntxt = 1) { return den_text_cache_layout(nullptr, B2, n_steps, ntxt).total; }
inline const float* den_cache_tkv(const float* cache, int B2, int ntxt) {
    return den_text_cache_layout(const_cast<float*>(cache), B2, 0, ntxt).tkv;
}
inline const float* den_cache_ctab(const float* cache, int B2, int ntxt) {
    const DenTextCache L = den_text_cache_layout(const_cast<float*>(cache), B2, 0, ntxt);
    return ntxt > 1 ? L.catt : L.ctab;
}
inline void den_loop_io(float* ws, int rows, float** x, float** xs) {
    const DenForwardWs L = den_forward_layout(ws, (size_t)rows);
    *x = L.P[0]; *xs = L.Ps[0];
}

struct LcaWs { float *tn, *key, *val, *catt, *xn, *q, *semb, *mod; size_t total; };
inline LcaWs lca_layout(float* ws, int B, int T, int N) {
    LcaWs L;
    Carver c(ws);
    const size_t R = (size_t)B * N, M = (size_t)B * T;
    L.tn = c.take(R * D); L.key = c.take(R * D); L.val = c.take(R * D);
    L.catt = c.take((size_t)B * H * DH * DH);
    L.xn = c.take(M * D); L.q = c.take(M * D);
    L.semb = c.take((size_t)B * D); L.mod = c.take((size_t)B * 2 * D);
    L.total = c.off;
    return L;
}
inline size_t linear_cross_attention_ws_floats(int B, int T, int N) { return lca_layout(nullptr, B, T, N).total; }

inline size_t dec_cross_ws_floats(int B, int T) { return (size_t)B * H * T * (2 * D + 1); }

struct DecWs : XfmrWs {
    float *kv, *guws;
    int32_t* row_out;
    float *pex, *pexs, *qkv0;
    size_t kv_layer, gu_layer, total;
};
inline DecWs dec_layout(float* ws, int B, size_t M, int T) {
    DecWs L;
    Carver c(ws);
    carve_xfmr(c, M, L);
    L.kv_layer = (size_t)T * B * 2 * D; L.gu_layer = dec_cross_ws_floats(B, T);
    L.kv = c.take(NL * L.kv_layer);
    L.guws = c.take(NL * L.gu_layer);
    L.row_out = reinterpret_cast<int32_t*>(c.take((M + 63) / 64 * 64));
    L.pex = c.take((size_t)LADIFF_MAX_FRAMES * D);
    L.pexs = c.take((size_t)LADIFF_MAX_FRAMES * D);
    L.qkv0 = c.take((size_t)LADIFF_MAX_FRAMES * 3 * D);
    L.total = c.off;
    return L;
}
inline size_t dec_ws_floats(int B, size_t rows, int T) { return dec_layout(nullptr, B, rows, T).total; }

struct EncWs : XfmrWs { float *featp, *wskel, *emb; uint32_t* keybits; size_t total; };
inline EncWs enc_layout(float* ws, int B, int F, int T, int C) {
    EncWs L;
    Carver c(ws);
    const size_t Cp = pad32(C);
    carve_xfmr(c, (size_t)B * (2 * T + F), L);
    L.featp = c.take((size_t)B * F * Cp);
    L.wskel = c.take((size_t)D * Cp);
    L.emb = c.take((size_t)B * F * D);
    L.keybits = reinterpret_cast<uint32_t*>(c.take((size_t)B * 8 + 64));
    L.total = c.off;
    return L;
}
inline size_t enc_ws_floats(int B, int F, int T, int C) { return enc_layout(nullptr, B, F, T, C).total; }

constexpr int VAE_LOSS_MAX_BLOCKS = 512;
struct VaeLossWs { double* part; int blocks; size_t total; };
inline VaeLossWs vae_losses_layout(float* ws, int B, int F, int C, int J, int T) {
    VaeLossWs L;
    Carver c(ws);
    size_t n = (size_t)B * F * C;
    for (size_t m : {(size_t)B * F * J * 3, (size_t)T * B * D})
        if (m > n) n = m;
    const size_t blocks = ((n + 3) / 4 + 255) / 256;
    L.blocks = blocks < 1 ? 1 : (blocks > VAE_LOSS_MAX_BLOCKS ? VAE_LOSS_MAX_BLOCKS : (int)blocks);
    L.part = reinterpret_cast<double*>(c.take((size_t)L.blocks * 3 * 2));
    L.total = c.off;
    return L;
}
inline size_t vae_losses_ws_floats(int B, int F, int C, int J, int T) { return vae_losses_layout(nullptr, B, F, C, J, T).total; }

struct DenPerSampleWs { float *sinus, *tables, *cache, *dctab, *u, *tws, *xws, *fwd; size_t tws_floats, xws_floats, fwd_floats, total; };
inline DenPerSampleWs den_per_sample_layout(float* ws, int B2, int T) {
    DenPerSampleWs L;
    Carver c(ws, 64);
    L.sinus = c.take((size_t)B2 * TEXT_DIM);
    L.tables = c.take(den_tables_floats(B2));
    L.cache = c.take(den_text_cache_floats(B2, 0, 1));
    L.dctab = c.take((size_t)NL * B2 * 2 * D);
    L.u = c.take((size_t)NL * B2 * 2 * D);
    L.tws_floats = den_time_layout(nullptr, B2).total;
    L.tws = c.take(L.tws_floats);
    L.xws_floats = den_text_ws_floats(B2, 0, 1);
    L.xws = c.take(L.xws_floats);
    L.fwd_floats = den_forward_ws_floats(B2, T);
    L.fwd = c.take(L.fwd_floats);
    L.total = c.off;
    return L;
}
inline size_t den_per_sample_ws_floats(int B2, int T) { return den_per_sample_layout(nullptr, B2, T).total; }

constexpr int DIFF_LOSS_MAX_BLOCKS = 512;
struct DiffLossWs { double* part; int blocks; size_t total; };
inline DiffLossWs diffusion_losses_layout(float* ws, size_t n) {
    DiffLossWs L;
    Carver c(ws);
    const size_t blocks = ((n + 3) / 4 + 255) / 256;
    L.blocks = blocks < 1 ? 1 : (blocks > DIFF_LOSS_MAX_BLOCKS ? DIFF_LOSS_MAX_BLOCKS : (int)blocks);
    L.part = reinterpret_cast<double*>(c.take((size_t)L.blocks * 2));
    L.total = c.off;
    return L;
}

constexpr int CLIP_W = LADIFF_TEXT_DIM;
constexpr int CLIP_FF = 4 * CLIP_W;
constexpr int CLIP_SMALL_ROWS = 256;
constexpr int CLIP_PLANE_COLS = 12 * CLIP_W;
constexpr int CLIP_FC2_KPARTS = 4;
constexpr int CLIP_FC2_KPARTS_MAX_ROWS = 8192;
inline size_t clip_plane_floats(int M) {
    const size_t small_rows = (size_t)(M < CLIP_SMALL_ROWS ? M : CLIP_SMALL_ROWS) * CLIP_PLANE_COLS;
    const size_t kparts = M > CLIP_SMALL_ROWS ? (size_t)(M < CLIP_FC2_KPARTS_MAX_ROWS ? M : CLIP_FC2_KPARTS_MAX_ROWS) * CLIP_FC2_KPARTS * CLIP_W : 0;
    return small_rows > kparts ? small_rows : kparts;
}
struct ClipWs { float *x, *x2, *h, *qkv, *att, *mlp, *planes, *pooled; int32_t* eos; size_t total; };
inline ClipWs clip_layout(float* ws, int B, int M) {
    ClipWs L;
    Carver c(ws);
    const size_t MW = (size_t)M * CLIP_W;
    L.x = c.take(MW); L.x2 = c.take(MW); L.h = c.take(MW);
    L.qkv = c.take(3 * MW);
    L.att = c.take(MW);
    L.mlp = c.take((size_t)M * CLIP_FF);
    L.planes = c.take(clip_plane_floats(M));
    L.pooled = c.take((size_t)B * CLIP_W);
    L.eos = reinterpret_cast<int32_t*>(c.take((size_t)B + 64));
    L.total = c.off;
    return L;
}
inline size_t clip_ws_floats_rows(int B, int total_rows) { return clip_layout(nullptr, B, total_rows).total; }
inline size_t clip_ws_floats(int B, int L) { return clip_ws_floats_rows(B, B * L); }

constexpr int T2M_MOVE_H = 512, T2M_MOTION_H = 1024, T2M_TEXT_H = 512, T2M_WORD = 300, T2M_POS = 15;

struct GruHeadWs { float *gi, *gh, *h, *cat, *hid, *hidn; size_t total; };
inline GruHeadWs gru_head_layout(float* ws, int B, int T, int Hs) {
    GruHeadWs L;
    Carver c(ws);
    L.gi = c.take((size_t)2 * B * T * 3 * Hs);
    L.gh = c.take((size_t)2 * B * 3 * Hs);
    L.h = c.take((size_t)2 * B * Hs);
    L.cat = c.take((size_t)B * 2 * Hs);
    L.hid = c.take((size_t)B * Hs);
    L.hidn = c.take((size_t)B * Hs);
    c.take(64);
    L.total = c.off;
    return L;
}
inline size_t gru_head_floats(int B, int T, int Hs) { return gru_head_layout(nullptr, B, T, Hs).total; }

struct T2mMoveWs { float *a1, *w1, *y1, *a2, *y2; size_t total; };
inline T2mMoveWs t2m_move_layout(float* ws, int B, int F, int Cin) {
    T2mMoveWs L;
    Carver c(ws);
    const int T1 = F / 2, T2 = T1 / 2, K1 = pad32(4 * Cin);
    L.a1 = c.take((size_t)B * T1 * K1);
    L.w1 = c.take((size_t)T2M_MOVE_H * K1);
    L.y1 = c.take((size_t)B * T1 * T2M_MOVE_H);
    L.a2 = c.take((size_t)B * T2 * 4 * T2M_MOVE_H);
    L.y2 = c.take((size_t)B * T2 * T2M_MOVE_H);
    c.take(64);
    L.total = c.off;
    return L;
}
inline size_t t2m_move_ws_floats(int B, int F, int Cin) { return t2m_move_layout(nullptr, B, F, Cin).total; }

struct T2mMotionWs { float *emb, *gru; size_t total; };
inline T2mMotionWs t2m_motion_layout(float* ws, int B, int T) {
    T2mMotionWs L;
    Carver c(ws);
    L.emb = c.take((size_t)B * T * T2M_MOTION_H);
    L.gru = c.take(gru_head_floats(B, T, T2M_MOTION_H));
    L.total = c.off;
    return L;
}
inline size_t t2m_motion_ws_floats(int B, int T) { return t2m_motion_layout(nullptr, B, T).total; }

struct T2mTextWs { float *posp, *wpos, *wordp, *winp, *inp, *emb, *gru; size_t total; };
inline T2mTextWs t2m_text_layout(float* ws, int B, int L_) {
    T2mTextWs L;
    Carver c(ws);
    const size_t M = (size_t)B * L_, Kp = pad32(T2M_POS), Kw = pad32(T2M_WORD);
    L.posp = c.take(M * Kp);
    L.wpos = c.take(T2M_WORD * Kp);
    L.wordp = c.take(M * Kw);
    L.winp = c.take(T2M_TEXT_H * Kw);
    L.inp = c.take(M * Kw);
    L.emb = c.take(M * T2M_TEXT_H);
    L.gru = c.take(gru_head_floats(B, L_, T2M_TEXT_H));
    L.total = c.off;
    return L;
}
inline size_t t2m_text_ws_floats(int B, int L) { return t2m_text_layout(nullptr, B, L).total; }

constexpr int REVERSE_WINDOW_MAX = 64;
inline int reverse_window(int n) {
    if (n <= REVERSE_WINDOW_MAX) return n;
    for (int w = REVERSE_WINDOW_MAX; w >= 10; --w)
        if (n % w == 0 && w % 10 == 0) return w;
    for (int w = REVERSE_WINDOW_MAX; w > 1; --w)
        if (n % w == 0) return w;
    return 1;
}
struct ReverseWs {
    float *tables, *cache, *latents, *eps, *fwd, *sys, *cws;
    int32_t* d_step;
    size_t fwd_floats, cws_floats, total_bytes, sys_off;
    int window;
};
inline ReverseWs carve_reverse(void* ws, int B, int T, int n, int ntxt = 1) {
    ReverseWs r;
    const int B2 = 2 * B;
    Carver c(static_cast<float*>(ws), 64);
    r.d_step = reinterpret_cast<int32_t*>(c.take(64));
    r.tables = c.take(den_tables_floats(n));
    r.window = reverse_window(n);
    const int wcap = n < REVERSE_WINDOW_MAX ? n : REVERSE_WINDOW_MAX;
    r.cache = c.take(den_text_cache_floats(B2, wcap, ntxt));
    r.latents = c.take((size_t)B * T * D);
    r.eps = c.take((size_t)B2 * T * D);
    r.fwd_floats = den_forward_ws_floats(B2, T);
    for (size_t pre : {den_time_layout(nullptr, n).total, den_text_ws_floats(B2, 1, ntxt)})
        if (pre > r.fwd_floats) r.fwd_floats = pre;
    r.fwd = c.take(r.fwd_floats);
    r.sys_off = c.off;
    r.sys = c.take(sys_ws_floats(B, T));
    r.cws_floats = den_text_layout(nullptr, B2, wcap, 1).u_floats;
    r.cws = c.take(r.cws_floats);
    r.total_bytes = c.off * sizeof(float);
    return r;
}

}
```

Before: 11320 motions/s.

## Dedup shared-qkv decoder attention, write final layer directly, fuse ctab input prep

```diff
diff --git a/ladiff_amd/csrc/api.hip b/ladiff_amd/csrc/api.hip
--- a/ladiff_amd/csrc/api.hip
+++ b/ladiff_amd/csrc/api.hip
@@ -257,8 +257,9 @@
 }
 
 int ladiff_debug_set_handoff(int tagged) {
-    LADIFF_CHECK_ARG(tagged == 0 || tagged == 1);
-    g_handoff = tagged;
+    LADIFF_CHECK_ARG(tagged >= 0 && tagged <= 3);
+    g_handoff = tagged & 1;
+    g_ctab_fused = (tagged & 2) ? 0 : 1;
     return 0;
 }
 
@@ -273,7 +274,9 @@
 }
 
 int ladiff_debug_set_decoder_fusion(int on) {
-    LADIFF_CHECK_ARG(on >= 0 && on <= 126 && (on & 3) != 3 && (on & 48) != 48);
+    LADIFF_CHECK_ARG(on >= 0 && on <= 510 && (on & 3) != 3 && (on & 48) != 48);
+    g_dec_att_dedup = (on & 128) ? 0 : 1;
+    g_dec_final_direct = (on & 256) ? 0 : 1;
     g_dec_out_cross = (on & 64) ? 0 : 1;
     g_dec_fused_mlp = on & 3;
     g_dec_small_rows_path = (on & 4) ? 0 : 1;
@@ -741,7 +744,8 @@
     if (ws_bytes < ladiff_decoder_workspace_bytes(B, F, T, C)) return LADIFF_ERR_WORKSPACE;
     hipStream_t s = S(stream);
     const GraphKey key = decode_key(w, w_split, DEC_NPARAMS, weights_generation, z, lengths, counts, row_off, total_rows, B, F, T, C, feats, ws,
-                                    stream, g_dec_fused_mlp, g_dec_small_rows_path, g_dec_final_split, g_mlp_variant, g_dec_fused_attn);
+                                    stream, g_dec_fused_mlp, g_dec_small_rows_path, g_dec_final_split + 2 * g_dec_final_direct, g_mlp_variant,
+                                    g_dec_fused_attn + 4 * g_dec_att_dedup);
     if (!(dg->exec && dg->slot.key == key && dg->slot.newest())) {
         if (dg->exec) { LADIFF_HIP(hipStreamSynchronize(s)); (void)hipGraphExecDestroy(dg->exec); dg->exec = nullptr; }
         LADIFF_TRY(dec_mlp_prepare());
diff --git a/ladiff_amd/csrc/attention.hip b/ladiff_amd/csrc/attention.hip
--- a/ladiff_amd/csrc/attention.hip
+++ b/ladiff_amd/csrc/attention.hip
@@ -152,7 +152,8 @@
 __global__ __launch_bounds__(NT, NT == 64 ? 2 : 1) void self_attn_split_kernel(const float* __restrict__ qkv, const int32_t* __restrict__ lengths,
                                                                const uint32_t* __restrict__ keybits, float* __restrict__ out,
                                                                int B, int F, int split_out, const AttnGeom g,
-                                                               const int32_t* __restrict__ row_off, int shared_qkv) {
+                                                               const int32_t* __restrict__ row_off, int shared_qkv,
+                                                               int32_t* __restrict__ att_rep) {
     constexpr int NKT = FM / 32, IT = FM * 16 / NT, VLD = FM + 8;
     static_assert(FM % 32 == 0 && (FM * 16) % NT == 0 && NT % 64 == 0 && (FM / 4) % (NT / 64) == 0 && NT / 64 >= FM / 32, "a wave per query tile");
     __shared__ __attribute__((aligned(16))) s16 Kp[2 * FM * DH];
@@ -162,6 +163,17 @@
     float* const Vtmp = reinterpret_cast<float*>(Kp);
     const int tid = threadIdx.x, lane = tid & 63, wave = tid >> 6;
     const int b = blockIdx.x / g.nheads, h = blockIdx.x % g.nheads;
+    if (att_rep != nullptr) {
+        const int mine = lengths[b], rows = row_off != nullptr ? row_off[b + 1] - row_off[b] : 0;
+        int rep = b;
+        for (int j0 = 0; j0 < b; j0 += 64) {
+            const int j = j0 + lane;
+            const unsigned long long eq = __ballot(j < b && lengths[j] == mine && (row_off == nullptr || row_off[j + 1] - row_off[j] == rows));
+            if (eq != 0) { rep = j0 + __builtin_ctzll(eq); break; }
+        }
+        if (h == 0 && tid == 0) att_rep[b] = rep;
+        if (rep != b) return;
+    }
     int len = F;
     uint32_t kb[NKT + 1];
     if (keybits != nullptr) {
@@ -347,13 +359,14 @@
 }
 
 int launch_self_attention_split(const float* qkv, const int32_t* lengths, const uint32_t* keybits, float* out, int B, int F,
-                                 int nheads, int causal, int split_out, hipStream_t s, const int32_t* row_off, int shared_qkv) {
+                                 int nheads, int causal, int split_out, hipStream_t s, const int32_t* row_off, int shared_qkv, int32_t* att_rep) {
     if (F > SA_FMAX || F < 1 || nheads < 1) return LADIFF_ERR_SHAPE;
+    if (att_rep != nullptr && (!shared_qkv || lengths == nullptr || keybits != nullptr)) return LADIFF_ERR_ARG;
     if (B == 0) return 0;
     const int W = nheads * DH;
     const AttnGeom g{nheads, 3 * W, W, 2 * W, W, causal};
-    if (F <= 32) hipLaunchKernelGGL((self_attn_split_kernel<32, 64>), dim3(B * nheads), dim3(64), 0, s, qkv, lengths, keybits, out, B, F, split_out, g, row_off, shared_qkv);
-    else hipLaunchKernelGGL((self_attn_split_kernel<SA_FMAX, 512>), dim3(B * nheads), dim3(512), 0, s, qkv, lengths, keybits, out, B, F, split_out, g, row_off, shared_qkv);
+    if (F <= 32) hipLaunchKernelGGL((self_attn_split_kernel<32, 64>), dim3(B * nheads), dim3(64), 0, s, qkv, lengths, keybits, out, B, F, split_out, g, row_off, shared_qkv, att_rep);
+    else hipLaunchKernelGGL((self_attn_split_kernel<SA_FMAX, 512>), dim3(B * nheads), dim3(512), 0, s, qkv, lengths, keybits, out, B, F, split_out, g, row_off, shared_qkv, att_rep);
     LADIFF_LAUNCH_CHECK();
     return 0;
 }
diff --git a/ladiff_amd/csrc/dec_cross.hip b/ladiff_amd/csrc/dec_cross.hip
--- a/ladiff_amd/csrc/dec_cross.hip
+++ b/ladiff_amd/csrc/dec_cross.hip
@@ -213,6 +213,7 @@
     const float* gu; const float* cc;
     const float* bo_c; const float* g2; const float* b2;
     const int32_t* counts; const int32_t* row_off;
+    const int32_t* att_rep;
     float* y; float* ys;
     int F, rows_per_wg;
     unsigned long long* stamps;
@@ -305,6 +306,8 @@
     int F = p.F;
     size_t row0 = (size_t)b * F;
     if (p.row_off != nullptr) { row0 = p.row_off[b]; F = p.row_off[b + 1] - p.row_off[b]; }
+    size_t arow0 = row0;
+    if (p.att_rep != nullptr) { const int rb = p.att_rep[b]; arow0 = p.row_off != nullptr ? (size_t)p.row_off[rb] : (size_t)rb * F; }
     const int f0 = blockIdx.y * p.rows_per_wg;
     const int f1 = f0 + p.rows_per_wg < F ? f0 + p.rows_per_wg : F;
     if (f0 >= f1) return;
@@ -317,7 +320,7 @@
             const int r = wave + 8 * i, f = fb + r < f1 ? fb + r : f1 - 1;
             unsigned vo = ((lane & 48) << 4) + ((((lane & 15) ^ r) & 15) << 4);
             asm volatile("" : "+v"(vo));
-            const char* src = reinterpret_cast<const char*>(p.att) + ((row0 + f) << 10) + vo;
+            const char* src = reinterpret_cast<const char*>(p.att) + ((arow0 + f) << 10) + vo;
             __builtin_amdgcn_global_load_lds(reinterpret_cast<const float*>(src), (__attribute__((address_space(3))) void*)(tile + r * 1024), 16, 0, 0);
         }
     };
@@ -555,7 +558,7 @@
 
 int launch_decoder_out_cross(const float* att_s, const float* x0, const float* wo_s, const float* bo, const float* g1, const float* b1,
                              const float* bo_c, const float* g2, const float* b2, const int32_t* counts, int B, int F, int T,
-                             const float* gu_ws, float* y, float* ys, hipStream_t s, const int32_t* row_off) {
+                             const float* gu_ws, float* y, float* ys, hipStream_t s, const int32_t* row_off, const int32_t* att_rep) {
     if (B == 0 || F == 0) return 0;
     if (T < 1 || T > TM) return LADIFF_ERR_SHAPE;
     int chunks = (256 + B - 1) / B;
@@ -564,7 +567,7 @@
     const int rows_per_wg = ((F + chunks - 1) / chunks + OC_ROWS - 1) / OC_ROWS * OC_ROWS;
     chunks = (F + rows_per_wg - 1) / rows_per_wg;
     LADIFF_TRY(dec_cross_prepare());
-    OutCrossArgs a{att_s, x0, wo_s, bo, g1, b1, gu_ws, gu_ws + (size_t)B * H * T * 2 * D, bo_c, g2, b2, counts, row_off, y, ys, F, rows_per_wg, nullptr};
+    OutCrossArgs a{att_s, x0, wo_s, bo, g1, b1, gu_ws, gu_ws + (size_t)B * H * T * 2 * D, bo_c, g2, b2, counts, row_off, att_rep, y, ys, F, rows_per_wg, nullptr};
 #ifdef LADIFF_STAMPS
     a.stamps = g_sys_stamps;
 #endif
diff --git a/ladiff_amd/csrc/decoder.hip b/ladiff_amd/csrc/decoder.hip
--- a/ladiff_amd/csrc/decoder.hip
+++ b/ladiff_amd/csrc/decoder.hip
@@ -12,6 +12,8 @@
 #endif
 
 constexpr int DEC_SMALL_ROWS = 4096;
+std::atomic<int> g_dec_final_direct{1};
+std::atomic<int> g_dec_att_dedup{1};
 std::atomic<int> g_dec_out_cross{1};
 std::atomic<int> g_dec_fused_attn{1};
 std::atomic<int> g_dec_final_split{1};
@@ -62,6 +64,7 @@
 
     const bool small = sp && M < DEC_SMALL_ROWS && g_dec_small_rows_path;
     const bool fused_attn = sp && g_dec_fused_attn && (M >= DEC_SMALL_ROWS || g_dec_fused_attn == 2);
+    int32_t* const rep = sp && !small && g_dec_out_cross && g_dec_att_dedup && lengths != nullptr && (size_t)B <= a.att_rep_slots ? a.att_rep : nullptr;
     auto krs = [&](const float* A, int K, const float* W, const float* bias, float* Y, float* Ys, int ldy, int N, int act,
                    const float* res, int rows) -> int {
         KrArgs g;
@@ -128,12 +131,12 @@
         }
         const float* qkv_l = shared ? qkv0 : qkv;
         if (fused_attn && !shared) { LADIFF_TRY(launch_dec_qkv_attn(curs, Ls.self_attn.in_w, L.self_attn.in_b, lengths, row_off, att, B, F, 1, s)); DEC_CUT(); }
-        else if (sp) { LADIFF_TRY(launch_self_attention_split(qkv_l, lengths, nullptr, att, B, F, H, 0, 1, s, row_off, shared)); DEC_CUT(); }
+        else if (sp) { LADIFF_TRY(launch_self_attention_split(qkv_l, lengths, nullptr, att, B, F, H, 0, 1, s, row_off, shared, shared ? rep : nullptr)); DEC_CUT(); }
         else { LADIFF_TRY(launch_decoder_self_attention(qkv_l, lengths, nullptr, att, B, F, 0, s, row_off, shared)); DEC_CUT(); }
         const NormW* n1_late = nullptr;
         if (sp && !small && g_dec_out_cross) {
             LADIFF_TRY(launch_decoder_out_cross(att, cur, Ls.self_attn.out_w, L.self_attn.out_b, L.norm1.g, L.norm1.b, L.cross_attn.out_b,
-                                                L.norm2.g, L.norm2.b, counts, B, F, T, guws + l * gu_l, P[2], Ps[2], s, row_off)); DEC_CUT();
+                                                L.norm2.g, L.norm2.b, counts, B, F, T, guws + l * gu_l, P[2], Ps[2], s, row_off, shared ? rep : nullptr)); DEC_CUT();
         } else {
         if (sp) {
             if (small) { LADIFF_TRY(krs(att, D, Ls.self_attn.out_w, L.self_attn.out_b, P[1], nullptr, D, D, ACT_NONE, cur, M)); DEC_CUT(); }
@@ -175,6 +178,13 @@
         if ((size_t)M * Np > a.hid_floats || (size_t)Np * (D + 1) > a.qkv_floats) return LADIFF_ERR_SHAPE;
         float* wpad = qkv; float* bpad = qkv + (size_t)Np * D;
         LADIFF_TRY(launch_pad_rows(wsp->final_layer.w, w.final_layer.b, wpad, bpad, C, Np, s)); DEC_CUT();
+        if (g_dec_final_direct) {
+            GemmArgs g = lin(curs, D, wpad, bpad, feats, C, M, Np, D);
+            g.split = 1; g.ncols = C;
+            if (ragged) g.row_map = row_out;
+            else { g.row_len = lengths; g.rows_per_item = F; }
+            return launch_gemm(g, s);
+        }
         GemmArgs g = lin(curs, D, wpad, bpad, hid, Np, M, Np, D);
         g.split = 1;
         LADIFF_TRY(launch_gemm(g, s)); DEC_CUT();
diff --git a/ladiff_amd/csrc/denoiser.hip b/ladiff_amd/csrc/denoiser.hip
--- a/ladiff_amd/csrc/denoiser.hip
+++ b/ladiff_amd/csrc/denoiser.hip
@@ -132,6 +132,8 @@
     LADIFF_TRY(launch_layernorm_batch(ln, NL, B2, s));
     return launch_gemm_batch(val, NL, s);
 }
+
+std::atomic<int> g_ctab_fused{1};
 
 int denoiser_ctab(const DenoiserW& w, const float* tables_lo, int n, float* cache, int B2, float* u, size_t u_floats, hipStream_t s,
                   const DenoiserW* wsp) {
@@ -151,6 +153,15 @@
             rb.b[l] = tables_lo + (size_t)l * DEN_LAYER_STRIDE + DEN_OFF_CA_MOD; rb.y[l] = ul;
             g[l] = lin(ul, D, L.ca_proj.out, ctab + (size_t)l * n * R * D, D, n * R, D, D);
             if (wsp != nullptr) { g[l].W = wsp->layer[l].ca_proj.out.w; g[l].split = 1; }
+        }
+        if (wsp != nullptr && g_ctab_fused) {
+            GemmBatch gb;
+            for (int l = 0; l < NL; ++l) {
+                GemmArgs& a = gb.a[l];
+                a = g[l];
+                a.A = rb.a[l]; a.lda = D; a.A2 = rb.g[l]; a.K1 = a.K; a.mod = rb.b[l]; a.mod_stride = DEN_STEP_STRIDE; a.rows_per_item = R;
+            }
+            return launch_gemm_big_ctab(gb, NL, s);
         }
         LADIFF_TRY(launch_ca_table_input_batch(rb, NL, DEN_STEP_STRIDE, n, B2, s, wsp != nullptr ? 1 : 0));
         return launch_gemm_batch(g, NL, s);
diff --git a/ladiff_amd/csrc/gemm.h b/ladiff_amd/csrc/gemm.h
--- a/ladiff_amd/csrc/gemm.h
+++ b/ladiff_amd/csrc/gemm.h
@@ -23,6 +23,7 @@
     const int32_t* row_len = nullptr; int rows_per_item = 0;
     const int32_t* row_map = nullptr;
     int ksplit = 1; size_t plane = 0;
+    int ncols = 0;
 };
 
 int launch_gemm(const GemmArgs& a, hipStream_t stream);
@@ -32,5 +33,6 @@
 int launch_gemm_big_batch(const GemmBatch& b, int n, hipStream_t stream);
 bool gemm_big_supported(const GemmArgs& a);
 int launch_gemm_big(const GemmArgs& a, hipStream_t stream);
+int launch_gemm_big_ctab(const GemmBatch& b, int n, hipStream_t stream);
 
 }
diff --git a/ladiff_amd/csrc/gemm_big.hip b/ladiff_amd/csrc/gemm_big.hip
--- a/ladiff_amd/csrc/gemm_big.hip
+++ b/ladiff_amd/csrc/gemm_big.hip
@@ -159,7 +159,7 @@
     });
 }
 
-template <int BM, int BN>
+template <int BM, int BN, bool FRAMES = false, bool CTAB = false>
 __device__ __forceinline__ void gemm_big_split_body(const GemmArgs& p) {
     constexpr int NW = 4, WM = 2, WN = 2;
     constexpr int TMW = BM / WM, TNW = BN / WN, RM = TMW / 16, RN = TNW / 16;
@@ -197,7 +197,7 @@
         const float* abase; int ald;
         if (k0 < argK1) { abase = p.A + k0; ald = p.lda; } else { abase = p.A2 + (k0 - argK1); ald = p.lda2; }
 #pragma unroll
-        for (int g = 0; g < GT; ++g) {
+        for (int g = CTAB ? GA : 0; g < GT; ++g) {
             const float* src;
             if (g < GA) {
                 int gr = row0 + GRP * g + rl; gr = gr < argM ? gr : argM - 1;
@@ -208,6 +208,43 @@
             dma16(src, lbase + buf * STAGE + GRP * g * 32);
         }
     };
+    constexpr int AQ = CTAB ? BM / 32 : 1;
+    const int ar = tid >> 3, aj = tid & 7;
+    int amod[AQ], aval[AQ];
+    f32x4 av[AQ], asc[AQ], ash[AQ];
+    if constexpr (CTAB) {
+        const int R1 = pin_s(p.rows_per_item);
+#pragma unroll
+        for (int q = 0; q < AQ; ++q) {
+            int gr = row0 + 32 * q + ar; gr = gr < argM ? gr : argM - 1;
+            const int step = gr / R1, b = gr - step * R1;
+            amod[q] = step * p.mod_stride;
+            aval[q] = b < R1 - 1 ? b * p.lda : -1;
+        }
+    }
+    auto load_a = [&](int ktl) __attribute__((always_inline)) {
+        const int kb = (kt0 + ktl) * 32 + 4 * aj;
+#pragma unroll
+        for (int q = 0; q < AQ; ++q) {
+            const float* m = p.mod + amod[q] + kb;
+            asc[q] = ld4(m); ash[q] = ld4(m + 256);
+            av[q] = ld4((aval[q] >= 0 ? p.A + aval[q] : p.A2) + kb);
+        }
+    };
+    auto build_a = [&](int buf) __attribute__((always_inline)) {
+#pragma unroll
+        for (int q = 0; q < AQ; ++q) {
+            f32x4 v = av[q];
+#pragma unroll
+            for (int i = 0; i < 4; ++i) v[i] = silu(v[i] * (1.f + asc[q][i]) + ash[q][i]);
+            s16x4 hi, lo;
+            split4(v, hi, lo);
+            const int r = 32 * q + ar, sw = (r >> 1) & 7;
+            char* const rowp = reinterpret_cast<char*>(lds + buf * STAGE + r * 32);
+            *reinterpret_cast<s16x4*>(rowp + (((aj >> 1) ^ sw) << 4) + ((aj & 1) << 3)) = hi;
+            *reinterpret_cast<s16x4*>(rowp + (((4 + (aj >> 1)) ^ sw) << 4) + ((aj & 1) << 3)) = lo;
+        }
+    };
 
     f32x4 acc[RM][RN];
 #pragma unroll
@@ -253,16 +290,40 @@
 #pragma unroll
     for (int e = 0; e < EI; ++e) rv[e] = f32x4{0.f, 0.f, 0.f, 0.f};
     f32x4 bv = {0.f, 0.f, 0.f, 0.f};
+    constexpr int FR = BM / NW, FH = BN / 64;
+    int fdst = -1, fvalid = 0;
+    float fb[FH];
+#pragma unroll
+    for (int h = 0; h < FH; ++h) fb[h] = 0.f;
 
     issue(0, 0);
+    if constexpr (CTAB) { load_a(0); build_a(0); if (nk > 1) load_a(1); }
     for (int kt = 0; kt < nk; ++kt) {
         const int buf = kt & 1;
-        wait_vm<0>();
+        if constexpr (CTAB) asm volatile("s_waitcnt vmcnt(0) lgkmcnt(0)" ::: "memory");
+        else wait_vm<0>();
         __builtin_amdgcn_s_barrier();
         if (kt + 1 < nk) issue(kt + 1, buf ^ 1);
+        if constexpr (CTAB) {
+            if (kt + 1 < nk) build_a(buf ^ 1);
+            if (kt + 2 < nk) load_a(kt + 2);
+        }
+        if constexpr (FRAMES) {
+            if (kt == nk - 1) {
+                if (p.bias != nullptr) {
+#pragma unroll
+                    for (int h = 0; h < FH; ++h) fb[h] = p.bias[col0 + 64 * h + lane];
+                }
+                const int gr = row0 + wave * FR + lane;
+                if (lane < FR && gr < argM) {
+                    fdst = p.row_map != nullptr ? p.row_map[gr] : gr;
+                    fvalid = p.row_len == nullptr || (gr % p.rows_per_item) < p.row_len[gr / p.rows_per_item];
+                }
+            }
+        } else
         if (kt == nk - 1 && ksplit == 1) {
             if (p.bias != nullptr) bv = ld4(p.bias + col0 + ec);
-            if (p.res != nullptr) {
+            if (!CTAB && p.res != nullptr) {
 #pragma unroll
                 for (int e = 0; e < EI; ++e) {
                     const int gr = row0 + er + e * RPI;
@@ -288,6 +349,24 @@
 #pragma unroll
     for (int e = 0; e < EI; ++e) reg_touch(rv[e]);
 
+    if constexpr (FRAMES) {
+        const int ncols = pin_s(p.ncols);
+#pragma unroll
+        for (int i = 0; i < FR; ++i) {
+            const int dst = __builtin_amdgcn_readlane(fdst, i);
+            const int valid = __builtin_amdgcn_readlane(fvalid, i);
+            if (dst < 0) continue;
+            float* const yr = argY + (size_t)dst * ncols;
+            const float* const cr = ct + (wave * FR + i) * CLD;
+#pragma unroll
+            for (int h = 0; h < FH; ++h) {
+                const int c = 64 * h + lane;
+                const float v = valid ? (cr[c] + fb[h]) + 0.f : 0.f;
+                if (col0 + c < ncols) yr[col0 + c] = v;
+            }
+        }
+        return;
+    }
     if (ksplit > 1) {
         float* const Yz = argY + (size_t)kz * p.plane;
 #pragma unroll
@@ -317,7 +396,12 @@
 template <int BM, int BN>
 __global__ __launch_bounds__(256, 2) void gemm_big_split_kernel(const GemmArgs p) { gemm_big_split_body<BM, BN>(p); }
 template <int BM, int BN>
+__global__ __launch_bounds__(256, 2) void gemm_big_split_frames_kernel(const GemmArgs p) { gemm_big_split_body<BM, BN, true>(p); }
+template <int BM, int BN>
 __global__ __launch_bounds__(256, 2) void gemm_big_split_batch_kernel(const GemmBatch b) { gemm_big_split_body<BM, BN>(b.a[blockIdx.y]); }
+
+template <int BM, int BN>
+__global__ __launch_bounds__(256, 2) void gemm_big_split_ctab_batch_kernel(const GemmBatch b) { gemm_big_split_body<BM, BN, false, true>(b.a[blockIdx.y]); }
 
 template <int BM, int BN, int WM, int WN, bool LN>
 __global__ __launch_bounds__(256) void gemm_big_kernel(const GemmArgs p) { gemm_big_body<BM, BN, WM, WN, LN>(p); }
@@ -344,6 +428,10 @@
 }
 
 bool gemm_big_supported(const GemmArgs& a) {
+    if (a.split && a.ncols > 0)
+        return a.M > 0 && a.K % 64 == 0 && a.K1 == a.K && a.N % 128 == 0 && a.ncols <= a.N && a.N - a.ncols < 128 && a.lda % 4 == 0 && a.ldw % 4 == 0 &&
+               a.ldy == a.ncols && a.Y && !a.Ys && !a.res && a.act == ACT_NONE && a.ksplit <= 1 && !a.ln_g && !a.mod && a.post_act == ACT_NONE &&
+               (!a.row_len || a.rows_per_item > 0);
     if (a.split) return a.M > 0 && a.K % 64 == 0 && a.K1 % 64 == 0 && a.N % 128 == 0 && a.lda % 4 == 0 && a.ldw % 4 == 0 && (!a.A2 || a.lda2 % 4 == 0) &&
                         a.ldy % 64 == 0 && !a.ln_g && !a.mod && !a.row_len && !a.row_map && a.post_act == ACT_NONE && (a.Y || a.Ys);
     if (a.M < 4096 || a.K % BKB || a.K1 % BKB || (a.lda % 4) || (a.ldw % 4) || (a.A2 && (a.lda2 % 4))) return false;
@@ -357,7 +445,10 @@
         const int nbm = (a.M + 127) / 128, nbn = a.N / 128;
         const int ks = a.ksplit > 1 ? a.ksplit : 1;
         if (ks > 1 && ((a.K / 32) % ks != 0 || a.Y == nullptr || a.Ys != nullptr || a.plane == 0)) return LADIFF_ERR_ARG;
-        if (nbm * nbn <= 256 && a.M > 64) {
+        if (a.ncols > 0) {
+            if (nbm * nbn <= 256 && a.M > 64) hipLaunchKernelGGL((gemm_big_split_frames_kernel<64, 128>), dim3((((a.M + 63) / 64 + 7) / 8) * 8 * nbn), dim3(256), 0, s, a);
+            else hipLaunchKernelGGL((gemm_big_split_frames_kernel<128, 128>), dim3(((nbm + 7) / 8) * 8 * nbn), dim3(256), 0, s, a);
+        } else if (nbm * nbn <= 256 && a.M > 64) {
             const int nbm64 = (a.M + 63) / 64;
             hipLaunchKernelGGL((gemm_big_split_kernel<64, 128>), dim3(((nbm64 + 7) / 8) * 8 * nbn, ks), dim3(256), 0, s, a);
         } else {
@@ -369,6 +460,21 @@
     if (a.ksplit > 1) return LADIFF_ERR_ARG;
     if (a.ln_g != nullptr) return launch_big<64, 256, 2, 2, true>(a, s);
     return launch_big<128, 128, 2, 2, false>(a, s);
+}
+
+int launch_gemm_big_ctab(const GemmBatch& b, int n, hipStream_t s) {
+    const GemmArgs& a = b.a[0];
+    if (n < 1 || n > GEMM_BATCH_MAX) return LADIFF_ERR_ARG;
+    for (int i = 0; i < n; ++i) {
+        const GemmArgs& g = b.a[i];
+        if (!g.split || !g.A || !g.A2 || !g.mod || !g.W || !g.Y || g.Ys || g.res || g.ksplit > 1 || g.rows_per_item < 1 || g.lda % 4 || g.mod_stride % 4) return LADIFF_ERR_ARG;
+        if (g.M != a.M || g.N != a.N || g.K != 256 || g.K1 != g.K || g.N % 128 || g.ldw % 4 || g.ldy % 64 || g.M % g.rows_per_item) return LADIFF_ERR_SHAPE;
+    }
+    if (a.M == 0) return 0;
+    const int nbm = (a.M + 127) / 128, nbn = a.N / 128;
+    hipLaunchKernelGGL((gemm_big_split_ctab_batch_kernel<128, 128>), dim3(((nbm + 7) / 8) * 8 * nbn, n), dim3(256), 0, s, b);
+    LADIFF_LAUNCH_CHECK();
+    return 0;
 }
 
 int launch_gemm_big_batch(const GemmBatch& b, int n, hipStream_t s) {
diff --git a/ladiff_amd/csrc/kernels.h b/ladiff_amd/csrc/kernels.h
--- a/ladiff_amd/csrc/kernels.h
+++ b/ladiff_amd/csrc/kernels.h
@@ -78,7 +78,7 @@
 int launch_decoder_cross_prep(const DecCrossPrepBatch& pb, int n, int B, int T, hipStream_t s);
 int launch_decoder_out_cross(const float* att_s, const float* x0, const float* wo_s, const float* bo, const float* g1, const float* b1,
                              const float* bo_c, const float* g2, const float* b2, const int32_t* counts, int B, int F, int T,
-                             const float* gu_ws, float* y, float* ys, hipStream_t s, const int32_t* row_off);
+                             const float* gu_ws, float* y, float* ys, hipStream_t s, const int32_t* row_off, const int32_t* att_rep = nullptr);
 int launch_decoder_cross_apply(const float* x, const float* bo, const float* g2, const float* b2, const int32_t* counts, int B, int F,
                                int T, const float* gu_ws, float* y, float* ys, hipStream_t s, const int32_t* row_off = nullptr,
                                const float* g1 = nullptr, const float* b1 = nullptr);
@@ -102,7 +102,8 @@
 int launch_self_attention(const float* qkv, const int32_t* lengths, const uint32_t* keybits, float* out, int B, int F, int nheads,
                           int causal, int split_out, hipStream_t s, const int32_t* row_off = nullptr);
 int launch_self_attention_split(const float* qkv, const int32_t* lengths, const uint32_t* keybits, float* out, int B, int F,
-                                 int nheads, int causal, int split_out, hipStream_t s, const int32_t* row_off = nullptr, int shared_qkv = 0);
+                                 int nheads, int causal, int split_out, hipStream_t s, const int32_t* row_off = nullptr, int shared_qkv = 0,
+                                 int32_t* att_rep = nullptr);
 int launch_decoder_cross_attention(const float* q, const float* kv, const int32_t* counts, float* out, int B, int F,
                                    int T, int split_out, hipStream_t s);
 
diff --git a/ladiff_amd/csrc/model.h b/ladiff_amd/csrc/model.h
--- a/ladiff_amd/csrc/model.h
+++ b/ladiff_amd/csrc/model.h
@@ -48,6 +48,8 @@
 extern std::atomic<int> g_dec_small_rows_path;
 extern std::atomic<int> g_dec_final_split;
 extern std::atomic<int> g_dec_out_cross;
+extern std::atomic<int> g_dec_att_dedup, g_dec_final_direct;
+extern std::atomic<int> g_ctab_fused;
 extern std::atomic<int> g_stage_plan;
 extern std::atomic<int> g_poll_pause;
 extern std::atomic<int> g_stage_delay;
diff --git a/ladiff_amd/csrc/workspace.h b/ladiff_amd/csrc/workspace.h
--- a/ladiff_amd/csrc/workspace.h
+++ b/ladiff_amd/csrc/workspace.h
@@ -129,6 +129,8 @@
     float *kv, *guws;
     int32_t* row_out;
     float *pex, *pexs, *qkv0;
+    int32_t* att_rep;
+    size_t att_rep_slots;
     size_t kv_layer, gu_layer, total;
 };
 inline DecWs dec_layout(float* ws, int B, size_t M, int T) {
@@ -142,6 +144,7 @@
     L.pex = c.take((size_t)LADIFF_MAX_FRAMES * D);
     L.pexs = c.take((size_t)LADIFF_MAX_FRAMES * D);
     L.qkv0 = c.take((size_t)LADIFF_MAX_FRAMES * 3 * D);
+    L.att_rep = reinterpret_cast<int32_t*>(L.qkv); L.att_rep_slots = L.qkv_floats;
     L.total = c.off;
     return L;
 }
```

After: 11390 motions/s, median of 6. No clear change (+0.7%).
